# meyer-lab/cmtf-pls

Hardware: AMD Instinct MI355X
Metric: nipals_iters_per_sec (higher is better)
Workload: dtype f32

## Files before the change

cmtf_pls_amd/_lib.py:

```python
from __future__ import annotations

import ctypes
import os
from ctypes import c_char_p, c_double, c_int, c_int64, c_size_t, c_uint32, c_uint64, c_void_p

_HERE = os.path.dirname(os.path.abspath(__file__))
LIB_PATH = os.environ.get("CMTFPLS_LIB") or os.path.join(_HERE, "lib", "libcmtfpls.so")

_P = c_void_p

class XcovBlock(ctypes.Structure):
    _fields_ = [("S", _P), ("S2", _P), ("colcnt", _P), ("n_samples", c_double), ("order", c_int), ("A", c_int), ("B", c_int),
                ("n_squarings", c_int), ("Z", _P), ("wA", _P), ("wB", _P), ("info", _P)]


class KfoldState(ctypes.Structure):
    _fields_ = [("I", c_int), ("A", c_int), ("B", c_int), ("M", c_int), ("K", c_int), ("R", c_int)] + [
        (name, _P) for name in ("fold_of", "S", "mean", "Yk", "Gy", "WA", "WB", "Q", "Wa", "Wb", "T", "Gt", "coef", "Rm", "tm",
                                "Tout", "vec", "n_iter", "status", "part")]


class CvCoupledBlock(ctypes.Structure):
    _fields_ = [("X", _P), ("order", c_int), ("A", c_int), ("B", c_int)]


class LooCoupledBlock(ctypes.Structure):
    _fields_ = [("X", _P), ("colsum", _P), ("order", c_int), ("A", c_int), ("B", c_int)]


SIGNATURES = {
    "cmtfpls_xcov_iterate_blocks_f64": (c_int, [ctypes.POINTER(XcovBlock), c_int, c_int, _P, _P, _P, _P, _P, c_int, _P, c_size_t, _P]),
    "cmtfpls_abi_version": (c_int, []),
    "cmtfpls_last_error": (c_char_p, []),
    "cmtfpls_clear_error": (c_int, []),
    "cmtfpls_status_to_host": (c_int, [_P, _P, c_size_t, _P, _P]),
    "cmtfpls_colstats_workspace_bytes": (c_size_t, [c_int64, c_int64]),
    "cmtfpls_colstats_f32": (c_int, [_P, c_int64, c_int64, _P, _P, _P, c_size_t, _P]),
    "cmtfpls_colstats_f64": (c_int, [_P, c_int64, c_int64, _P, _P, _P, c_size_t, _P]),
    "cmtfpls_sweep_partials": (c_int, []),
    "cmtfpls_center_f32": (c_int, [_P, c_int64, c_int64, _P, _P, _P, _P]),
    "cmtfpls_center_f64": (c_int, [_P, c_int64, c_int64, _P, _P, _P, _P]),
    "cmtfpls_mode0_contract_workspace_bytes": (c_size_t, [c_int64, c_int64]),
    "cmtfpls_mode0_contract_f32": (c_int, [_P, c_int64, c_int64, _P, _P, c_int, _P, c_size_t, _P]),
    "cmtfpls_mode0_contract_f64": (c_int, [_P, c_int64, c_int64, _P, _P, c_int, _P, c_size_t, _P]),
    "cmtfpls_mode0_contract_yq_f32": (c_int, [_P, c_int64, c_int64, _P, c_int, c_int, _P, _P, c_int, _P, c_size_t, _P]),
    "cmtfpls_mode0_contract_yq_f64": (c_int, [_P, c_int64, c_int64, _P, c_int, c_int, _P, _P, c_int, _P, c_size_t, _P]),
    "cmtfpls_colscale_f64": (c_int, [_P, c_int64, _P, c_double, _P]),
    "cmtfpls_rank1_workspace_bytes": (c_size_t, [c_int, c_int]),
    "cmtfpls_rank1_score_f64": (c_int, [_P, c_int, c_int, _P, _P, _P, c_int, _P, c_int, _P, _P, c_size_t, _P]),
    "cmtfpls_rank1_f64": (c_int, [_P, c_int, c_int, _P, _P, _P, _P, c_int, _P, c_size_t, _P]),
    "cmtfpls_rank1_launches_f64": (c_int, [_P, c_int, c_int, _P, _P, _P, _P, c_int, _P, c_size_t, _P]),
    "cmtfpls_rank1_chain_enable": (None, [c_int]),
    "cmtfpls_rank1_chain_enabled": (c_int, []),
    "cmtfpls_normalize_f64": (c_int, [_P, c_int64, _P, _P]),
    "cmtfpls_rank1_tensor_workspace_bytes": (c_size_t, [_P, c_int]),
    "cmtfpls_rank1_tensor_f64": (c_int, [_P, _P, c_int, c_double, _P, c_int, _P, c_int, _P, c_size_t, _P]),
    "cmtfpls_kron_f64": (c_int, [_P, c_int, _P, c_int, _P, _P]),
    "cmtfpls_xcov_workspace_bytes": (c_size_t, [c_int64, c_int64, c_int]),
    "cmtfpls_xcov_f32": (c_int, [_P, c_int64, c_int64, _P, c_int, c_int, _P, c_int, _P, c_size_t, _P]),
    "cmtfpls_xcov_f64": (c_int, [_P, c_int64, c_int64, _P, c_int, c_int, _P, c_int, _P, c_size_t, _P]),
    "cmtfpls_xcov_bf16": (c_int, [_P, c_int64, c_int64, _P, c_int, c_int, _P, c_int, _P, c_size_t, _P]),
    "cmtfpls_xcov_f16": (c_int, [_P, c_int64, c_int64, _P, c_int, c_int, _P, c_int, _P, c_size_t, _P]),
    "cmtfpls_quadform_f64": (c_int, [_P, c_int, _P, _P, _P, _P]),
    "cmtfpls_xcov_iterate_f64": (c_int, [_P, c_int, c_int, c_int, _P, _P, _P, _P, _P, c_int, _P, _P, _P, c_int, _P, c_size_t, _P, c_size_t, _P]),
    "cmtfpls_s_downdate_f64": (c_int, [_P, c_int, c_int, c_int, _P, _P, _P, _P, _P, _P]),
    "cmtfpls_project_rows_f32": (c_int, [_P, c_int64, c_int, c_int, c_int, _P, _P, _P, _P, c_int, _P]),
    "cmtfpls_project_rows_f64": (c_int, [_P, c_int64, c_int, c_int, c_int, _P, _P, _P, _P, c_int, _P]),
    "cmtfpls_project_rows2_f32": (c_int, [_P, c_int, c_int, _P, _P, _P, _P, c_int, c_int, _P, _P, _P, c_int64, c_int, _P, c_int, _P]),
    "cmtfpls_project_rows2_f64": (c_int, [_P, c_int, c_int, _P, _P, _P, _P, c_int, c_int, _P, _P, _P, c_int64, c_int, _P, c_int, _P]),
    "cmtfpls_project_rows_idx_f32": (c_int, [_P, _P, c_int64, c_int, c_int, c_int, _P, _P, _P, _P, c_int, _P]),
    "cmtfpls_project_rows_idx_f64": (c_int, [_P, _P, c_int64, c_int, c_int, c_int, _P, _P, _P, _P, c_int, _P]),
    "cmtfpls_project_rows2_idx_f32": (c_int, [_P, c_int, c_int, _P, _P, _P, _P, c_int, c_int, _P, _P, _P, _P, c_int64, c_int, _P, c_int, _P]),
    "cmtfpls_project_rows2_idx_f64": (c_int, [_P, c_int, c_int, _P, _P, _P, _P, c_int, c_int, _P, _P, _P, _P, c_int64, c_int, _P, c_int, _P]),
    "cmtfpls_allreduce_sum_f64": (c_int, [_P, _P, c_size_t, _P]),
    "cmtfpls_allreduce_sum_f32": (c_int, [_P, _P, c_size_t, _P]),
    "cmtfpls_axpy_scalar_f64": (c_int, [_P, c_int64, _P, _P, _P]),
    "cmtfpls_xcov_deflate_f32": (c_int, [_P, c_int64, c_int, c_int, _P, c_int, c_int, _P, _P, _P, _P, _P, _P, c_size_t, _P]),
    "cmtfpls_xcov_deflate_f64": (c_int, [_P, c_int64, c_int, c_int, _P, c_int, c_int, _P, _P, _P, _P, _P, _P, c_size_t, _P]),
    "cmtfpls_xcov_stats_workspace_bytes": (c_size_t, [c_int64, c_int64, c_int]),
    "cmtfpls_xcov_stats_f32": (c_int, [_P, c_int64, c_int64, _P, c_int, c_int, _P, _P, _P, c_size_t, _P]),
    "cmtfpls_xcov_stats_f64": (c_int, [_P, c_int64, c_int64, _P, c_int, c_int, _P, _P, _P, c_size_t, _P]),
    "cmtfpls_xcov_stats_bf16": (c_int, [_P, c_int64, c_int64, _P, c_int, c_int, _P, _P, _P, c_size_t, _P]),
    "cmtfpls_xcov_stats_f16": (c_int, [_P, c_int64, c_int64, _P, c_int, c_int, _P, _P, _P, c_size_t, _P]),
    "cmtfpls_xcov_ssq_workspace_bytes": (c_size_t, [c_int64, c_int64, c_int]),
    "cmtfpls_xcov_ssq_f32": (c_int, [_P, c_int64, c_int64, _P, c_int, c_int, _P, _P, _P, _P, c_size_t, _P]),
    "cmtfpls_xcov_ssq_f64": (c_int, [_P, c_int64, c_int64, _P, c_int, c_int, _P, _P, _P, _P, c_size_t, _P]),
    "cmtfpls_score_contract_workspace_bytes": (c_size_t, [c_int64, c_int64]),
    "cmtfpls_score_contract_f32": (c_int, [_P, c_int64, c_int, c_int, _P, _P, _P, _P, _P, c_double, _P, _P, _P, _P, c_size_t, _P]),
    "cmtfpls_score_contract_f64": (c_int, [_P, c_int64, c_int, c_int, _P, _P, _P, _P, _P, c_double, _P, _P, _P, _P, c_size_t, _P]),
    "cmtfpls_score_contract_bf16": (c_int, [_P, c_int64, c_int, c_int, _P, _P, _P, _P, _P, c_double, _P, _P, _P, _P, c_size_t, _P]),
    "cmtfpls_score_contract_f16": (c_int, [_P, c_int64, c_int, c_int, _P, _P, _P, _P, _P, c_double, _P, _P, _P, _P, c_size_t, _P]),
    "cmtfpls_kr_axpy_f64": (c_int, [_P, c_int, c_int, _P, _P, c_int, c_int, _P, _P]),
    "cmtfpls_xcov_f32_mixed": (c_int, [_P, c_int64, c_int64, _P, c_int, c_int, _P, c_int, _P, c_size_t, _P]),
    "cmtfpls_mttkrp_f32_mixed": (c_int, [_P, c_int64, c_int, c_int, _P, _P, c_int, _P, c_int, _P]),
    "cmtfpls_mttkrp_f32": (c_int, [_P, c_int64, c_int, c_int, _P, _P, c_int, _P, c_int, _P]),
    "cmtfpls_mttkrp_f64": (c_int, [_P, c_int64, c_int, c_int, _P, _P, c_int, _P, c_int, _P]),
    "cmtfpls_mttkrp_bf16": (c_int, [_P, c_int64, c_int, c_int, _P, _P, c_int, _P, c_int, _P]),
    "cmtfpls_mttkrp_f16": (c_int, [_P, c_int64, c_int, c_int, _P, _P, c_int, _P, c_int, _P]),
    "cmtfpls_score_f32": (c_int, [_P, c_int64, c_int, c_int, _P, _P, _P, _P, _P]),
    "cmtfpls_score_f64": (c_int, [_P, c_int64, c_int, c_int, _P, _P, _P, _P, _P]),
    "cmtfpls_score_s_f64": (c_int, [_P, c_int, c_int, c_int, _P, _P, _P, _P]),
    "cmtfpls_deflate_contract_workspace_bytes": (c_size_t, [c_int64, c_int64]),
    "cmtfpls_deflate_contract_yq_f32": (c_int, [_P, c_int64, c_int, c_int, _P, _P, _P, _P, c_int, c_int, _P, _P, c_int, _P, _P, c_size_t, _P]),
    "cmtfpls_deflate_contract_yq_f64": (c_int, [_P, c_int64, c_int, c_int, _P, _P, _P, _P, c_int, c_int, _P, _P, c_int, _P, _P, c_size_t, _P]),
    "cmtfpls_score_gram_f32": (c_int, [_P, c_int64, c_int, c_int, _P, _P, _P, _P, _P, c_int, c_int, _P, _P]),
    "cmtfpls_score_gram_f64": (c_int, [_P, c_int64, c_int, c_int, _P, _P, _P, _P, _P, c_int, c_int, _P, _P]),
    "cmtfpls_q_update_f64": (c_int, [_P, c_int, c_int, _P, c_int, _P, _P, _P, _P]),
    "cmtfpls_deflate_f32": (c_int, [_P, c_int64, c_int, c_int, _P, _P, _P, _P, _P]),
    "cmtfpls_deflate_f64": (c_int, [_P, c_int64, c_int, c_int, _P, _P, _P, _P, _P]),
    "cmtfpls_score_deflate_f32": (c_int, [_P, c_int64, c_int, c_int, _P, _P, _P, _P, _P, _P]),
    "cmtfpls_score_deflate_f64": (c_int, [_P, c_int64, c_int, c_int, _P, _P, _P, _P, _P, _P]),
    "cmtfpls_sweep_form": (c_int, [c_char_p, c_int, c_int64, c_int, c_int, c_int, c_int, c_int, c_char_p, c_size_t]),
    "cmtfpls_sweep_form_list": (c_int, [c_char_p, c_int, c_char_p, c_size_t]),
    "cmtfpls_small_workspace_bytes": (c_size_t, []),
    "cmtfpls_gram_tn_f64": (c_int, [_P, c_int, c_int, _P, c_int, c_int, c_int64, _P, _P, c_size_t, _P]),
    "cmtfpls_rowdot_f64": (c_int, [_P, c_int, c_int, c_int64, _P, _P, _P, _P, _P, c_size_t, _P]),
    "cmtfpls_scores_mean_f64": (c_int, [_P, c_int, c_int64, _P, _P]),
    "cmtfpls_y_deflate_f64": (c_int, [_P, c_int, c_int, c_int64, _P, c_int, c_int, _P, _P, _P, _P, c_size_t, _P]),
# ... 159 lines not shown
```

cmtf_pls_amd/backend.py:

```python
from __future__ import annotations

import ctypes
from typing import Optional, Tuple

import torch

from . import _lib
from .storage import HALF_DTYPES, HALF_ENTRIES, SUFFIX, entry_name

_HALF_ENTRIES = tuple(dict.fromkeys(e for group in HALF_ENTRIES.values() for e in group))


def _ptr(t: Optional[torch.Tensor]):
    return None if t is None else t.data_ptr()


def _int_pairs(pairs):
    flat = [int(v) for p in pairs for v in p]
    return (ctypes.c_int * len(flat))(*flat)


def _scratch(nbytes: int, device) -> torch.Tensor:
    return torch.empty(max(int(nbytes), 256), dtype=torch.uint8, device=device)


def chunk_size(n: int, per: int, budget: int, cap: Optional[int] = None) -> int:
    chunk = max(1, min(int(n), int(budget) // max(int(per), 1)))
    return chunk if cap is None else min(chunk, int(cap))


class HipBackend:
    name = "hip"

    def __init__(self, device: Optional[torch.device] = None):
        self.lib = _lib.load()
        if not torch.cuda.is_available():
            raise _lib.CmtfplsError("cmtf_pls_amd needs a ROCm GPU (torch.cuda.is_available() is False); there is no CPU fallback")
        self.device = torch.device(device) if device is not None else torch.device("cuda", torch.cuda.current_device())
        self.n_partials = int(self.lib.cmtfpls_sweep_partials())
        self._ws = {}
        self._status_slots = {}
        self.rank1_squarings = 30
        self.rank1_chain_side = 256 if self.lib.cmtfpls_rank1_chain_enabled() else 0

    def _stream(self):
        return torch.cuda.current_stream(self.device).cuda_stream

    def _workspace(self, key: str, nbytes: int) -> torch.Tensor:
        buf = self._ws.get(key)
        if buf is None or buf.numel() < nbytes:
            buf = self._ws[key] = _scratch(nbytes, self.device)
        return buf

    @staticmethod
    def _form(rc: int, name: str, value=True):
        if rc == 4:
            return None
        _lib.check(rc, name)
        return value

    def _chunked_launch(self, name: str, call, n: int, per_fn, budget: int, cap: Optional[int] = None, extra: int = 0,
                        ws_key: Optional[str] = None) -> Optional[int]:
        if call(0, 1, None, 0) == 4:
            return None
        per = int(per_fn())
        chunk = chunk_size(n, per + extra, budget, cap)
        ws = self._workspace(ws_key, per * chunk) if ws_key else _scratch(per * chunk, self.device)
        launches = 0
        for i0 in range(0, n, chunk):
            if self._form(call(i0, min(chunk, n - i0), _ptr(ws), ws.numel()), name) is None:
                return None
            launches += 1
        return launches

    def _ws_budget(self, max_ws_bytes: Optional[int], third_of_free: bool = False) -> int:
        if max_ws_bytes is not None:
            return int(max_ws_bytes)
        return max(4 << 30, torch.cuda.mem_get_info(self.device)[0] // 3) if third_of_free else 4 << 30

    def clear_error(self) -> bool:
        return bool(self.lib.cmtfpls_clear_error())

    def empty(self, *shape, dtype=torch.float64) -> torch.Tensor:
        return torch.empty(*shape, dtype=dtype, device=self.device)

    def zeros(self, *shape, dtype=torch.float64) -> torch.Tensor:
        return torch.zeros(*shape, dtype=dtype, device=self.device)

    def has_half(self, base: str) -> bool:
        return base in _HALF_ENTRIES and all(hasattr(self.lib, entry_name(base, d)) for d in HALF_DTYPES)

    def _read_fn(self, base: str, X: torch.Tensor, mixed: bool = False):
        if X.dtype not in SUFFIX:
            raise TypeError(f"X must be float32 or float64 on device, got {X.dtype}")
        if X.dtype in HALF_DTYPES and (mixed or not self.has_half(base)):
            return None
        if mixed and X.dtype == torch.float32:
            return getattr(self.lib, f"cmtfpls_{base}_f32_mixed")
        assert X.is_contiguous() and X.device == self.device
        return getattr(self.lib, entry_name(base, X.dtype))

    def _fn(self, base: str, X: torch.Tensor):
        fn = self._read_fn(base, X)
        if fn is None:
            raise TypeError(f"{base} has no form for {X.dtype} storage (16-bit X is only read by {', '.join(_HALF_ENTRIES)}); "
                            "use a float32 copy")
        return fn

    def _close_partials(self, part: torch.Tensor) -> torch.Tensor:
        out = self.empty(1)
        _lib.check(self.lib.cmtfpls_sum_f64(_ptr(part), part.numel(), _ptr(out), self._stream()), "sum")
        return out

    @staticmethod
    def sweep_form(op: str, dtype, I: int, A: int, B: int, masked: bool = False, M: int = 0, aligned16: bool = True) -> str:
        buf = ctypes.create_string_buffer(256)
        elem = 4 if dtype in (torch.float32, "f32", "float32") else 8
        _lib.check(_lib.load().cmtfpls_sweep_form(op.encode(), elem, int(I), int(A), int(B), int(bool(masked)), int(M), int(bool(aligned16)),
                                                  buf, len(buf)), "sweep_form")
        return buf.value.decode()

    @staticmethod
    def sweep_form_list(op: str, dtype) -> list:
        buf = ctypes.create_string_buffer(1 << 14)
# ... 65 lines not shown
        ws = self._workspace("rank1t", self.lib.cmtfpls_rank1_tensor_workspace_bytes(arr, len(dims)))
        _lib.check(self.lib.cmtfpls_rank1_tensor_f64(_ptr(Z), arr, len(dims), float(tol), _ptr(factors), factors.stride(0), _ptr(info),
                                                     int(n_squarings or self.rank1_squarings), _ptr(ws), ws.numel(), self._stream()),
                   "rank1_tensor")

    def kron(self, a: torch.Tensor, b: torch.Tensor, out: torch.Tensor) -> torch.Tensor:
        _lib.check(self.lib.cmtfpls_kron_f64(_ptr(a), a.numel(), _ptr(b), b.numel(), _ptr(out), self._stream()), "kron")
        return out

    def normalize(self, v: torch.Tensor) -> None:
        _lib.check(self.lib.cmtfpls_normalize_f64(_ptr(v), v.numel(), None, self._stream()), "normalize")

    def xcov(self, X2: torch.Tensor, Y: torch.Tensor, masked: bool, out: Optional[torch.Tensor] = None,
             mixed: bool = False) -> Optional[torch.Tensor]:
        I, P = X2.shape
        M = Y.shape[1]
        fn = self._read_fn("xcov", X2, mixed)
        if fn is None:
            return None
        ws = self._workspace("contract", self.lib.cmtfpls_xcov_workspace_bytes(I, P, M))
        S = out if out is not None else self.empty(M, P)
        _lib.check(fn(_ptr(X2), I, P, _ptr(Y), Y.stride(0), M, _ptr(S), int(masked), _ptr(ws), ws.numel(), self._stream()), "xcov")
        return S

    def xcov_deflate(self, X2: torch.Tensor, A: int, B: int, Y: torch.Tensor, t: torch.Tensor, wA: torch.Tensor, wB: torch.Tensor,
                     out: torch.Tensor) -> Optional[torch.Tensor]:
        I, P = X2.shape
        M = Y.shape[1]
        if M > 64 or P % 4 != 0 or P != A * B:
            return None
        ws = self._workspace("contract", self.lib.cmtfpls_xcov_ssq_workspace_bytes(I, P, M))
        ssq = self.empty(1)
        rc = self._fn("xcov_deflate", X2)(_ptr(X2), I, A, B, _ptr(Y), Y.stride(0), M, _ptr(t), _ptr(wA), _ptr(wB), _ptr(out), _ptr(ssq),
                                          _ptr(ws), ws.numel(), self._stream())
        return self._form(rc, "xcov_deflate", ssq)

    def rank1_score(self, Z: torch.Tensor, A: int, B: int, wA: torch.Tensor, wB: torch.Tensor, S: torch.Tensor, tq: torch.Tensor,
                    info: Optional[torch.Tensor] = None, n_squarings: Optional[int] = None) -> torch.Tensor:
        M = S.shape[0]
        assert S.is_contiguous() and S.shape[1] == A * B and tq.numel() >= M
        ws = self._workspace("rank1", self.lib.cmtfpls_rank1_workspace_bytes(A, B))
        _lib.check(self.lib.cmtfpls_rank1_score_f64(_ptr(Z), A, B, _ptr(wA), _ptr(wB), _ptr(info),
                                                    int(n_squarings if n_squarings is not None else self.rank1_squarings),
                                                    _ptr(S), M, _ptr(tq), _ptr(ws), ws.numel(), self._stream()), "rank1_score")
        return tq

    def xcov_ssq(self, X2: torch.Tensor, Y: torch.Tensor, mean: torch.Tensor, out: torch.Tensor):
        I, P = X2.shape
        M = Y.shape[1]
        ws = self._workspace("contract", self.lib.cmtfpls_xcov_ssq_workspace_bytes(I, P, M))
        ssq = self.empty(1)
        assert mean.is_contiguous() and mean.numel() == P and mean.dtype == torch.float64
        _lib.check(self._fn("xcov_ssq", X2)(_ptr(X2), I, P, _ptr(Y), Y.stride(0), M, _ptr(out), _ptr(mean), _ptr(ssq), _ptr(ws), ws.numel(),
                                            self._stream()), "xcov_ssq")
        return out, ssq

    def xcov_stats(self, X2: torch.Tensor, Y: torch.Tensor, out: torch.Tensor):
        I, P = X2.shape
        M = Y.shape[1]
        fn = self._read_fn("xcov_stats", X2) if M <= 64 and X2.is_contiguous() else None
        if fn is None:
            return None
        ws = self._workspace("contract", self.lib.cmtfpls_xcov_stats_workspace_bytes(I, P, M))
        stats = self.empty(2 * P)
        rc = fn(_ptr(X2), I, P, _ptr(Y), Y.stride(0), M, _ptr(out), _ptr(stats), _ptr(ws), ws.numel(), self._stream())
        return self._form(rc, "xcov_stats", (out, stats))

    def status_snapshot(self, status: torch.Tensor, slot: int, slots: Optional[dict] = None):
        slots = self._status_slots if slots is None else slots
        ent = slots.get((slot, status.numel()))
        if ent is None:
            host, ev = torch.empty(status.numel(), dtype=torch.float64, pin_memory=True), torch.cuda.Event()
            ev.record(torch.cuda.current_stream(self.device))
            ent = slots[(slot, status.numel())] = (host, ev, host.numpy(), host.data_ptr(), ev.cuda_event, status.numel() * 8)
        rc = self.lib.cmtfpls_status_to_host(status.data_ptr(), ent[3], ent[5], ent[4], self._stream())
        if rc:
            _lib.check(rc, "status_to_host")
        return ent

    def status_wait(self, token) -> "np.ndarray":
        token[1].synchronize()
        return token[2]

    def xcov_iterate_plan(self, S: torch.Tensor, A: int, B: int, q_cur: torch.Tensor, Z: torch.Tensor, wA: torch.Tensor,
                          wB: torch.Tensor, status: torch.Tensor, q_new: torch.Tensor, G: torch.Tensor):
        M, P = S.shape
        wc = self._workspace("contract", self.lib.cmtfpls_mode0_contract_workspace_bytes(M, P))
        wr = self._workspace("rank1", self.lib.cmtfpls_rank1_workspace_bytes(A, B))
        keep = (S, q_cur, Z, wA, wB, status, q_new, G, wc, wr)
        fn = self.lib.cmtfpls_xcov_iterate_f64
        head = (_ptr(S), M, A, B, _ptr(q_cur), _ptr(Z), _ptr(wA), _ptr(wB), status[1:3].data_ptr())
        tail = (_ptr(wc), wc.numel(), _ptr(wr), wr.numel())
        qn, Gp, du2 = _ptr(q_new), _ptr(G), status[0:1].data_ptr()
        stream = self._stream

        def enqueue(n_squarings: int, first: bool, _keep=keep) -> None:
            rc = fn(*head, n_squarings, qn, Gp, du2, 1 if first else 0, *tail, stream())
            if rc:
                _lib.check(rc, "xcov_iterate")
        return enqueue

    def xcov_iterate(self, S: torch.Tensor, A: int, B: int, q_cur: torch.Tensor, Z: torch.Tensor, wA: torch.Tensor,
                     wB: torch.Tensor, info: torch.Tensor, n_squarings: int, q_new: torch.Tensor, G: torch.Tensor,
                     du2: torch.Tensor, first: bool) -> None:
        M, P = S.shape
        wc = self._workspace("contract", self.lib.cmtfpls_mode0_contract_workspace_bytes(M, P))
        wr = self._workspace("rank1", self.lib.cmtfpls_rank1_workspace_bytes(A, B))
        _lib.check(self.lib.cmtfpls_xcov_iterate_f64(_ptr(S), M, A, B, _ptr(q_cur), _ptr(Z), _ptr(wA), _ptr(wB), _ptr(info),
                                                     int(n_squarings), _ptr(q_new), _ptr(G), _ptr(du2), int(first),
                                                     _ptr(wc), wc.numel(), _ptr(wr), wr.numel(), self._stream()), "xcov_iterate")

    def xcov_blocks_plan(self, blocks, M: int, q_cur: torch.Tensor, tq: torch.Tensor, q_new: torch.Tensor, G: torch.Tensor,
                         status: torch.Tensor):
        nb = len(blocks)
        if M > 64 or any(b["order"] not in (2, 3) for b in blocks) or tq.numel() != nb * M or not tq.is_contiguous():
            return None
        arr = (_lib.XcovBlock * nb)()
        need = 256
        for i, b in enumerate(blocks):
            for name in ("S", "S2", "colcnt", "Z", "wA", "wB"):
                t = b.get(name)
                assert t is None or (t.is_contiguous() and t.dtype == torch.float64 and t.device == self.device), name
                setattr(arr[i], name, _ptr(t))
            arr[i].n_samples, arr[i].order, arr[i].A, arr[i].B = float(b["n_samples"]), int(b["order"]), int(b["A"]), int(b["B"])
            arr[i].info = status[1 + 2 * i: 3 + 2 * i].data_ptr()
            if b["order"] == 3:
                need = max(need, self.lib.cmtfpls_rank1_workspace_bytes(b["A"], b["B"]))
        wr = self._workspace("rank1", need)
        keep = (blocks, q_cur, tq, q_new, G, status, wr, arr)
        fn, stream = self.lib.cmtfpls_xcov_iterate_blocks_f64, self._stream
        args = (nb, M, _ptr(q_cur), _ptr(tq), _ptr(q_new), _ptr(G), status[0:1].data_ptr())
        tail = (_ptr(wr), wr.numel())

        def enqueue(n_squarings, first: bool, _keep=keep) -> None:
            for i in range(nb):
                arr[i].n_squarings = int(n_squarings[i])
            rc = fn(arr, *args, 1 if first else 0, *tail, stream())
            if rc:
                _lib.check(rc, "xcov_iterate_blocks")
        return enqueue

    def s_downdate(self, S: torch.Tensor, A: int, B: int, ya: torch.Tensor, wA: torch.Tensor, wB: torch.Tensor,
                   q: torch.Tensor, v: torch.Tensor) -> None:
        assert S.is_contiguous() and S.shape[1] == A * B
        _lib.check(self.lib.cmtfpls_s_downdate_f64(_ptr(S), S.shape[0], A, B, _ptr(ya), _ptr(wA), _ptr(wB), _ptr(q), _ptr(v),
                                                   self._stream()), "s_downdate")

    def kr_axpy(self, v: torch.Tensor, A: int, B: int, WA: torch.Tensor, WB: torch.Tensor, k: int, coef: torch.Tensor) -> torch.Tensor:
        assert WA.is_contiguous() and WB.is_contiguous() and WA.shape[1] == WB.shape[1] and coef.numel() >= k
        _lib.check(self.lib.cmtfpls_kr_axpy_f64(_ptr(v), A, B, _ptr(WA), _ptr(WB), WA.shape[1], int(k), _ptr(coef), self._stream()), "kr_axpy")
        return v

    def axpy_scalar(self, y: torch.Tensor, a: torch.Tensor, x: Optional[torch.Tensor] = None) -> torch.Tensor:
        assert y.is_contiguous() and y.dtype == torch.float64 and a.numel() >= 1 and (x is None or (x.is_contiguous() and x.numel() == y.numel()))
        _lib.check(self.lib.cmtfpls_axpy_scalar_f64(_ptr(y), y.numel(), _ptr(a), _ptr(x), self._stream()), "axpy_scalar")
        return y

    def total(self, v: torch.Tensor) -> torch.Tensor:
        assert v.is_contiguous() and v.dtype == torch.float64
        return self._close_partials(v)

    def quadform(self, G: torch.Tensor, q: torch.Tensor, q_old: torch.Tensor, out: torch.Tensor) -> torch.Tensor:
        _lib.check(self.lib.cmtfpls_quadform_f64(_ptr(G), G.shape[0], _ptr(q), _ptr(q_old), _ptr(out), self._stream()), "quadform")
        return out

    def mttkrp(self, X2: torch.Tensor, A: int, B: int, WA: torch.Tensor, WB: torch.Tensor, out: torch.Tensor,
               mixed: bool = False) -> Optional[torch.Tensor]:
        R = WA.shape[1]
        assert WA.is_contiguous() and WB.is_contiguous() and out.stride(1) == 1
        fn = self._read_fn("mttkrp", X2, mixed)
        if fn is None:
            return None
        rc = fn(_ptr(X2), X2.shape[0], A, B, _ptr(WA), _ptr(WB), R, _ptr(out), out.stride(0), self._stream())
        return self._form(rc, "mttkrp", out)

    def score(self, X2, A, B, wA, wB, rowcnt, out) -> torch.Tensor:
        _lib.check(self._fn("score", X2)(_ptr(X2), X2.shape[0], A, B, _ptr(wA), _ptr(wB), _ptr(rowcnt), _ptr(out), self._stream()), "score")
        return out

    def score_s(self, S, A, B, wA, wB, out) -> torch.Tensor:
        assert S.dtype == torch.float64 and S.is_contiguous()
        _lib.check(self.lib.cmtfpls_score_s_f64(_ptr(S), S.shape[0], A, B, _ptr(wA), _ptr(wB), _ptr(out), self._stream()), "score_s")
        return out

    def score_contract(self, X2, A, B, wA, wB, shift, t, Z, sub_own=None, add_other=None, alpha: float = 1.0,
                       csum: Optional[torch.Tensor] = None) -> Optional[torch.Tensor]:
        I, P = X2.shape
        fn = self._read_fn("score_contract", X2) if X2.is_contiguous() and P == A * B else None
        if fn is None:
            return None
        for v in (sub_own, add_other):
            assert v is None or (v.is_contiguous() and v.numel() == I and v.dtype == torch.float64)
        nbytes = self.lib.cmtfpls_score_contract_workspace_bytes(I, P)
        ws = self._workspace("score_contract", max(nbytes, 256))
        rc = fn(_ptr(X2), I, A, B, _ptr(wA), _ptr(wB), _ptr(shift), _ptr(sub_own), _ptr(add_other), float(alpha),
                                            _ptr(t), _ptr(Z), _ptr(csum), _ptr(ws), ws.numel(), self._stream())
        return self._form(rc, "score_contract", Z)

    def score_gram(self, X2, A, B, wA, wB, rowcnt, out, Y: torch.Tensor, qpart: torch.Tensor) -> Optional[torch.Tensor]:
        assert qpart.numel() >= self.n_partials * Y.shape[1] and qpart.is_contiguous()
        rc = self._fn("score_gram", X2)(_ptr(X2), X2.shape[0], A, B, _ptr(wA), _ptr(wB), _ptr(rowcnt), _ptr(out),
                                        _ptr(Y), Y.stride(0), Y.shape[1], _ptr(qpart), self._stream())
        return self._form(rc, "score_gram", out)

    def q_update(self, q: torch.Tensor, qpart: Optional[torch.Tensor] = None, normalize: bool = True,
                 G: Optional[torch.Tensor] = None, q_prev: Optional[torch.Tensor] = None,
                 du2: Optional[torch.Tensor] = None, nparts: Optional[int] = None) -> None:
        M = q.numel()
        nrows = (nparts or self.n_partials) if qpart is not None else 0
        assert qpart is None or (qpart.is_contiguous() and qpart.numel() >= nrows * M)
        _lib.check(self.lib.cmtfpls_q_update_f64(_ptr(qpart), nrows, M, _ptr(q), int(normalize),
                                                 _ptr(G), _ptr(q_prev), _ptr(du2), self._stream()), "q_update")

    def deflate(self, X2, A, B, t, wA, wB) -> torch.Tensor:
        part = self.empty(self.n_partials)
        _lib.check(self._fn("deflate", X2)(_ptr(X2), X2.shape[0], A, B, _ptr(t), _ptr(wA), _ptr(wB), _ptr(part), self._stream()), "deflate")
        return self._close_partials(part)

    def deflate_contract_yq(self, X2, A, B, t, wA, wB, Y: torch.Tensor, q: torch.Tensor, masked: bool,
                            out: torch.Tensor) -> Optional[torch.Tensor]:
        I, P = X2.shape
        ws = self._workspace("deflate_contract", self.lib.cmtfpls_deflate_contract_workspace_bytes(I, P))
        ssq = self.empty(1)
        rc = self._fn("deflate_contract_yq", X2)(_ptr(X2), I, A, B, _ptr(t), _ptr(wA), _ptr(wB), _ptr(Y), Y.stride(0), Y.shape[1],
                                                 _ptr(q), _ptr(out), int(masked), _ptr(ssq), _ptr(ws), ws.numel(), self._stream())
        return self._form(rc, "deflate_contract_yq", ssq)

    def score_deflate(self, X2, A, B, wA, wB, rowcnt, out) -> Optional[torch.Tensor]:
        part = self.empty(self.n_partials)
        rc = self._fn("score_deflate", X2)(_ptr(X2), X2.shape[0], A, B, _ptr(wA), _ptr(wB), _ptr(rowcnt), _ptr(out), _ptr(part), self._stream())
        if self._form(rc, "score_deflate") is None:
            return None
        return self._close_partials(part)

    def gram_tn(self, A: torch.Tensor, B: torch.Tensor, out: Optional[torch.Tensor] = None) -> torch.Tensor:
        if A.dim() == 1:
            A = A.unsqueeze(1)
        if B.dim() == 1:
            B = B.unsqueeze(1)
        assert A.stride(1) == 1 and B.stride(1) == 1 and A.shape[0] == B.shape[0]
        a, b = A.shape[1], B.shape[1]
        ws = self._workspace("small", self.lib.cmtfpls_small_workspace_bytes())
        C = out if out is not None else self.empty(a, b)
        assert C.numel() == a * b and C.is_contiguous()
        _lib.check(self.lib.cmtfpls_gram_tn_f64(_ptr(A), A.stride(0), a, _ptr(B), B.stride(0), b, A.shape[0], _ptr(C),
                                                _ptr(ws), ws.numel(), self._stream()), "gram_tn")
        return C

    def rowdot(self, Y: torch.Tensor, q: torch.Tensor, u_out: torch.Tensor, u_old: Optional[torch.Tensor],
               du2: Optional[torch.Tensor] = None) -> Optional[torch.Tensor]:
        ws = self._workspace("small", self.lib.cmtfpls_small_workspace_bytes())
        if u_old is not None and du2 is None:
            du2 = self.empty(1)
        _lib.check(self.lib.cmtfpls_rowdot_f64(_ptr(Y), Y.stride(0), Y.shape[1], Y.shape[0], _ptr(q), _ptr(u_out), _ptr(u_old),
                                               _ptr(du2) if u_old is not None else None,
                                               _ptr(ws), ws.numel(), self._stream()), "rowdot")
        return du2 if u_old is not None else None

    def normal_solve(self, G: torch.Tensor, g: torch.Tensor, out: Optional[torch.Tensor] = None) -> torch.Tensor:
        k = G.shape[0]
        assert G.is_contiguous() and G.shape == (k, k) and g.numel() == k
        b = out if out is not None else self.empty(k)
        if k <= 64:
            _lib.check(self.lib.cmtfpls_normal_solve_f64(_ptr(G), _ptr(g), k, _ptr(b), 1, self._stream()), "normal_solve")
        else:
            ws = self._workspace("normal_solve", self.lib.cmtfpls_normal_solve_workspace_bytes(k))
            _lib.check(self.lib.cmtfpls_normal_solve_ws_f64(_ptr(G), _ptr(g), k, _ptr(b), 1, _ptr(ws), ws.numel(), self._stream()),
                       "normal_solve")
        return b

    def unit_upper_solve_rows(self, M: torch.Tensor, U: torch.Tensor, shift: Optional[torch.Tensor] = None,
                              nan_flag: Optional[torch.Tensor] = None) -> torch.Tensor:
        I, R = M.shape
        assert M.stride(1) == 1 and U.is_contiguous() and U.shape == (R, R)
        assert shift is None or (shift.is_contiguous() and shift.numel() == R and shift.dtype == torch.float64)
        assert nan_flag is None or nan_flag.dtype == torch.int32
        _lib.check(self.lib.cmtfpls_unit_upper_solve_rows_f64(_ptr(M), I, M.stride(0), R, _ptr(U), _ptr(shift), _ptr(nan_flag),
                                                              self._stream()), "unit_upper_solve_rows")
        return M

    def kr_gram_row(self, L: torch.Tensor, a: int, g: torch.Tensor, first: bool) -> torch.Tensor:
        assert L.is_contiguous() and g.is_contiguous() and g.numel() >= a
        _lib.check(self.lib.cmtfpls_kr_gram_row_f64(_ptr(L), L.shape[0], L.shape[1], int(a), _ptr(g), int(first), self._stream()), "kr_gram_row")
        return g

    def kr_gram(self, L: torch.Tensor, G: torch.Tensor, first: bool) -> torch.Tensor:
        n, R = L.shape
        assert L.is_contiguous() and G.is_contiguous() and G.numel() == R * R
        _lib.check(self.lib.cmtfpls_kr_gram_f64(_ptr(L), n, R, _ptr(G), int(first), 1.0, self._stream()), "kr_gram")
        return G

    def khatri_rao(self, Am: torch.Tensor, Bm: torch.Tensor) -> torch.Tensor:
        na, R = Am.shape
# ... 489 lines not shown
```

cmtf_pls_amd/csrc/common.hpp:

```cpp
#pragma once
#include <hip/hip_runtime.h>
#include <stdint.h>
#include <stdio.h>

#include "../../include/cmtfpls.h"

namespace cmtfpls {

constexpr int kWave = 64;
#ifndef CMTFPLS_SWEEP_BLOCKS
#define CMTFPLS_SWEEP_BLOCKS 512
#endif
#ifndef CMTFPLS_UNROLL
#define CMTFPLS_UNROLL 4
#endif
#ifndef CMTFPLS_ROW_UNROLL
#define CMTFPLS_ROW_UNROLL 8
#endif
#ifndef CMTFPLS_CONTRACT_BLOCKS
#define CMTFPLS_CONTRACT_BLOCKS 1024
#endif
#ifndef CMTFPLS_NT_LOAD
#define CMTFPLS_NT_LOAD 1
#endif
// ... 57 lines not shown
__device__ __forceinline__ VT ld_stream(const VT* p) {
#if CMTFPLS_NT_LOAD
  using R = typename NtRaw<sizeof(VT)>::type;
  const R r = __builtin_nontemporal_load(reinterpret_cast<const R*>(p));
  VT v;
  __builtin_memcpy(&v, &r, sizeof(VT));
  return v;
#else
  return *p;
#endif
}
template <typename VT>
__device__ __forceinline__ void st_stream(VT* p, const VT& v) {
#if CMTFPLS_NT_STORE
  using R = typename NtRaw<sizeof(VT)>::type;
  R r;
  __builtin_memcpy(&r, &v, sizeof(VT));
  __builtin_nontemporal_store(r, reinterpret_cast<R*>(p));
#else
  *p = v;
#endif
}

__device__ __forceinline__ double wave_sum(double v) {
#pragma unroll
  for (int m = 32; m > 0; m >>= 1) v += __shfl_xor(v, m, kWave);
  return v;
}

__device__ __forceinline__ double block_sum(double v, double* slot) {
  const int lane = threadIdx.x & 63, wv = threadIdx.x >> 6, nw = (blockDim.x + 63) >> 6;
  v = wave_sum(v);
  if (lane == 0) slot[wv] = v;
  __syncthreads();
  double s = 0.0;
  for (int w = 0; w < nw; ++w) s += slot[w];
  return s;
}

struct KronWalk {
  int j, k, dj, dk, B;
  __device__ __forceinline__ KronWalk(int64_t c0, int64_t stride, int B_) : B(B_) {
    j = (int)(c0 / B_);
    k = (int)(c0 % B_);
    dj = (int)(stride / B_);
    dk = (int)(stride % B_);
  }
  __device__ __forceinline__ void next() {
    k += dk;
    j += dj;
    if (k >= B) { k -= B; ++j; }
  }
};


struct TileId { int ct, rb; };
__device__ __forceinline__ TileId xcd_tile() {
  const unsigned CT = gridDim.x, RB = gridDim.y;
  const unsigned lin = blockIdx.x + CT * blockIdx.y;
  const unsigned G = CT * 8u, groups = RB / 8u;
  const unsigned grp = lin / G;
  TileId id;
  if (grp < groups) {
    const unsigned within = lin - grp * G;
    id.ct = (int)(within >> 3);
    id.rb = (int)(grp * 8u + (within & 7u));
  } else {
    const unsigned rest = lin - groups * G;
    id.ct = (int)(rest % CT);
    id.rb = (int)(groups * 8u + rest / CT);
  }
  return id;
}

struct XcovPlan {
  int col_tiles, row_blocks, rows_per_block;
};
XcovPlan plan_xcov(int64_t I, int64_t P);
constexpr int kXcovMaxResponses = 64;

void set_error(const char* msg);
int check_launch(const char* what);

}
```

cmtf_pls_amd/csrc/rank1.hip:

```cpp
#include "common.hpp"
#include <atomic>

namespace cmtfpls {

constexpr int kTile = 16;
constexpr int kMaxTiles = 256;
constexpr int kMaxSteps = 48;

struct Rank1Ctl {
  int done;
  int final_buf;
  int steps_used;
  int last_step;
  double pad[6];
};
__host__ __device__ __forceinline__ size_t rank1_ctl_bytes(int nt) {
  return sizeof(Rank1Ctl) + ((size_t)(kMaxSteps + 2) * nt + 2 * (size_t)nt * nt) * sizeof(double);
}
__device__ __forceinline__ double* ctl_trace(Rank1Ctl* c, int nt, int step) { return reinterpret_cast<double*>(c + 1) + (size_t)step * nt; }
__device__ __forceinline__ double* ctl_fro(Rank1Ctl* c, int nt, int which) {
  return reinterpret_cast<double*>(c + 1) + (size_t)(kMaxSteps + 2) * nt + (size_t)which * nt * nt;
}

__device__ __forceinline__ double pow2_scale_from_trace(const double* parts, int nt, double* tr_out) {
// ... 49 lines not shown
    if (tid >= nt * nt) f = 0.0;
    for (int i = tid + kTile * kTile; i < nt * nt; i += kTile * kTile) f += fp[i];
    f = wave_sum(f);
    if ((tid & 63) == 0) fsum[tid >> 6] = f;
    if (tid == 0) s_done = done_in;
    __syncthreads();
    fro_in = ((fsum[0] + fsum[1]) + fsum[2]) + fsum[3];
  }
  if (tid == 0) {
    int done = 0;
    double scale = 1.0;
    if (step == 0) {
      if (blockIdx.x == 0 && blockIdx.y == 0) { ctl->done = 0; ctl->final_buf = -1; ctl->steps_used = 0; ctl->last_step = -1; }
    } else {
      done = s_done;
      if (!done) {
        double tr1;
        scale = pow2_scale_from_trace(tr_s, nt, &tr1);
        const double rho = fro_in / (tr1 * tr1);
        const bool rank_one_in = !(tr1 > 0.0) || rho >= 1.0 - 1e-13;
        const bool rank_one_out = rho >= 1.0 - 1e-7;
        if (blockIdx.x == 0 && blockIdx.y == 0) {
          if (rank_one_in) { ctl->done = 1; ctl->final_buf = out_buf ^ 1; }
          else {
            ctl->steps_used = step;
            if (rank_one_out) { ctl->last_step = step; ctl->final_buf = out_buf; }
          }
        }
        if (rank_one_in) done = 1;
      }
    }
    s_scale = scale;
    s_done = done;
  }
  __syncthreads();
  if (s_done) return;
  const double scale = s_scale;

  d4r_t acc = d4r_t{0.0, 0.0, 0.0, 0.0};
  for (int kk = 0; kk < k; kk += KC) {
    if (kk > 0) {
#pragma unroll
      for (int s2 = 0; s2 < KW; ++s2) {
        const int c = kk + cl + s2;
        const int cc = (c < k) ? c : 0;
        a[s2] = rowa[cc];
        b[s2] = rowb[cc];
      }
    }
#pragma unroll
    for (int s2 = 0; s2 < KW; ++s2) {
      const bool cok = (kk + cl + s2) < k;
      const double av = (ra && cok) ? a[s2] : 0.0;
      const double bv = (rb && cok) ? b[s2] : 0.0;
      acc = __builtin_amdgcn_mfma_f64_16x16x4f64(av, bv, acc, 0, 0, 0);
    }
  }
#pragma unroll
  for (int e = 0; e < 4; ++e) red[wv][(kq + 4 * e) * kTile + ri] = acc[e];
  __syncthreads();
  double cacc = ((red[0][tid] + red[1][tid]) + red[2][tid]) + red[3][tid];
  cacc *= scale * scale;
  const bool inside = (i0 + ty < n && j0 + tx < n);
  if (inside) C[(int64_t)(i0 + ty) * n + (j0 + tx)] = cacc;
  if (inside && C_keep) C_keep[(int64_t)(i0 + ty) * n + (j0 + tx)] = cacc;
  {
    double sq = inside ? cacc * cacc : 0.0;
    sq = wave_sum(sq);
    if ((tid & 63) == 0) fsum[tid >> 6] = sq;
    __syncthreads();
    if (tid == 0) ctl_fro(ctl, nt, step & 1)[blockIdx.y * nt + blockIdx.x] = ((fsum[0] + fsum[1]) + fsum[2]) + fsum[3];
  }
  if (blockIdx.x == blockIdx.y) {
    if (tx == ty) diag[tx] = (i0 + ty < n) ? cacc : 0.0;
    __syncthreads();
    if (tid == 0) {
      double t = 0.0;
      for (int l = 0; l < kTile; ++l) t += diag[l];
      ctl_trace(ctl, nt, step)[blockIdx.x] = t;
    }
  }
}

constexpr unsigned long long kChainEmpty = ~0ull;
constexpr int kChainMaxSteps = 31;
constexpr int kChainSpin = 1 << 15;

__device__ __forceinline__ double chain_ld(const double* p) {
  return __longlong_as_double((long long)__hip_atomic_load(reinterpret_cast<const unsigned long long*>(p), __ATOMIC_RELAXED, __HIP_MEMORY_SCOPE_AGENT));
}
__device__ __forceinline__ void chain_st(double* p, double v) {
  unsigned long long b = (unsigned long long)__double_as_longlong(v);
  if (b == kChainEmpty) b = 0x7FF8000000000000ull;
  __hip_atomic_store(reinterpret_cast<unsigned long long*>(p), b, __ATOMIC_RELAXED, __HIP_MEMORY_SCOPE_AGENT);
}
__device__ __forceinline__ bool chain_empty(double v) { return (unsigned long long)__double_as_longlong(v) == kChainEmpty; }

__global__ __launch_bounds__(256) void chain_preset_kernel(unsigned long long* __restrict__ p, int64_t n) {
  for (int64_t i = (int64_t)blockIdx.x * 256 + threadIdx.x; i < n; i += (int64_t)gridDim.x * 256) p[i] = kChainEmpty;
}

#ifdef CMTFPLS_CHAIN_PROFILE
__device__ unsigned long long g_chain_prof[1024];
#define CHAIN_STAMP(slot) do { if (first_wg && tid == 0 && step < 32) g_chain_prof[step * 8 + (slot)] = __builtin_amdgcn_s_memrealtime(); } while (0)
#define CHAIN_COUNT(slot, v) do { if (first_wg && tid == 0 && step < 32) g_chain_prof[step * 8 + (slot)] = (unsigned long long)(v); } while (0)
#else
#define CHAIN_STAMP(slot) do { } while (0)
#define CHAIN_COUNT(slot, v) do { } while (0)
#endif

__global__ __launch_bounds__(kTile* kTile) void syrk_chain_kernel(const double* __restrict__ M0, int n, int k0,
                                                                 double* gbufs, double* trs, double* fros, double* gave_up,
                                                                 Rank1Ctl* __restrict__ ctl, int n_squarings) {
  constexpr int KC = 128, KW = 8, LDP = KC + 2;
  __shared__ __attribute__((aligned(16))) double pan[2][kTile][LDP];
  __shared__ double red[2][4][kTile * kTile];
  __shared__ double diag[2][kTile];
  __shared__ double fsum[2][4];
  __shared__ double cfro[2][4];
  __shared__ double ctr[2][kTile];
  __shared__ int cdead[2];
  const int tx = threadIdx.x, ty = threadIdx.y, tid = ty * kTile + tx;
  const int lane = tid & 63, wv = tid >> 6, ri = lane & 15, kq = lane >> 4;
  const int nt = (n + kTile - 1) / kTile, nt2 = nt * nt;
  const int i0 = blockIdx.y * kTile, j0 = blockIdx.x * kTile;
  const bool first_wg = blockIdx.x == 0 && blockIdx.y == 0;
  const bool ra = (i0 + ri) < n, rb = (j0 + ri) < n;
  const int cl = 32 * wv + KW * kq;
  const int64_t nn = (int64_t)n * n;
  const double qnan = __longlong_as_double(0x7FF8000000000000ll);
  bool dead = false;
  if (first_wg && tid == 0) { ctl->done = 0; ctl->final_buf = -1; ctl->steps_used = 0; ctl->last_step = -1; }
  if (tid < 2) cdead[tid] = 0;
  int last_step = -1;
  for (int step = 0; step <= n_squarings; ++step) {
    if (last_step >= 0) break;
    const int par = step & 1;
    const double* __restrict__ M = step == 0 ? M0 : gbufs + (int64_t)(step - 1) * nn;
    const int k = step == 0 ? k0 : n, ld = k;
    double* C = gbufs + (int64_t)step * nn;
    double a[KW], b[KW];
    double scale = 1.0;
    bool input_is_result = false;
    d4r_t acc = d4r_t{0.0, 0.0, 0.0, 0.0};
    CHAIN_STAMP(0);
    for (int kk = 0; kk < k; kk += KC) {
      if (step == 0) {
        const double* __restrict__ rowa = M + (int64_t)(ra ? i0 + ri : 0) * ld;
        const double* __restrict__ rowb = M + (int64_t)(rb ? j0 + ri : 0) * ld;
#pragma unroll
        for (int s2 = 0; s2 < KW; ++s2) {
          const int c = kk + cl + s2;
          const int cc = (c < k) ? c : 0;
          a[s2] = rowa[cc];
          b[s2] = rowb[cc];
        }
      } else {
        double va[8], vb[8], trv = 0.0, f = 0.0;
        const bool first_chunk = kk == 0;
        const double* tp = trs + (int64_t)(step - 1) * nt;
        const double* fp = fros + (int64_t)(step - 1) * nt2;
        unsigned offa[8], offb[8];
#pragma unroll
        for (int i = 0; i < 8; ++i) {
          const int e = tid + 256 * i, r = e >> 7, c = kk + (e & 127);
          const int cc = (c < k) ? c : 0;
          const int rra = (i0 + r < n) ? i0 + r : 0, rrb = (j0 + r < n) ? j0 + r : 0;
// ... 275 lines not shown
    if (bestv[w] > bv || (bestv[w] == bv && besti[w] < bi)) { bv = bestv[w]; bi = besti[w]; }
  const bool gv = gave && !chain_empty(chain_ld(gave));
  const double sgn = gv ? __longlong_as_double(0x7FF8000000000000ll) : ((vb[bi] < 0.0) ? -1.0 : 1.0);
  double* lx = x_is_A ? sA : sB;
  double* ly = x_is_A ? sB : sA;
  double* ox = x_is_A ? wA : wB;
  double* oy = x_is_A ? wB : wA;
  const bool store = blockIdx.x == 0;
  for (int i = threadIdx.x; i < n; i += 1024) {
    const double v = sgn * (x[i] / nx);
    lx[i] = v;
    if (store) ox[i] = v;
  }
  for (int i = threadIdx.x; i < k; i += 1024) {
    const double v = sgn * (y[i] / ny);
    ly[i] = v;
    if (store) oy[i] = v;
  }
  if (store && threadIdx.x == 0) rank1_write_info(info, ctl, gave);
  __syncthreads();
  using VT = Pack<double, 2>;
  const int64_t P = (int64_t)A * B;
  const int64_t step = (int64_t)1024 * 2;
  const double* __restrict__ xr = S + (int64_t)blockIdx.x * P;
  KronWalk w((int64_t)threadIdx.x * 2, step, B);
  double acc = 0.0;
  int64_t c = (int64_t)threadIdx.x * 2;
  constexpr int UN = 4;
  for (; c + (UN - 1) * step < P; c += UN * step) {
    VT xs[UN];
#pragma unroll
    for (int u = 0; u < UN; ++u) xs[u] = ld_stream(reinterpret_cast<const VT*>(xr + c + u * step));
#pragma unroll
    for (int u = 0; u < UN; ++u) {
      double d = 0.0;
      d = fma(xs[u].e[0], sB[w.k], d);
      d = fma(xs[u].e[1], sB[w.k + 1], d);
      acc = fma(sA[w.j], d, acc);
      w.next();
    }
  }
  for (; c < P; c += step) {
    const VT xv = ld_stream(reinterpret_cast<const VT*>(xr + c));
    double d = 0.0;
    d = fma(xv.e[0], sB[w.k], d);
    d = fma(xv.e[1], sB[w.k + 1], d);
    acc = fma(sA[w.j], d, acc);
    w.next();
  }
  acc = block_sum(acc, red[0]);
  if (threadIdx.x == 0) t[blockIdx.x] = acc;
}

static inline size_t align_up(size_t x, size_t a) { return (x + a - 1) / a * a; }

static std::atomic<int> g_chain_on{1};

static int chain_slots() {
  static int slots = 0;
  if (slots == 0) {
    int dev = 0, cus = 0;
    if (hipGetDevice(&dev) != hipSuccess || hipDeviceGetAttribute(&cus, hipDeviceAttributeMultiprocessorCount, dev) != hipSuccess || cus <= 0) cus = 256;
    slots = 2 * cus;
  }
  return slots;
}

}

using namespace cmtfpls;

extern "C" {

size_t cmtfpls_rank1_workspace_bytes(int A, int B) {
  if (A <= 0 || B <= 0) return 0;
  const size_t n = (size_t)(A < B ? A : B), k = (size_t)(A < B ? B : A);
  const size_t nt = (n + kTile - 1) / kTile;
  const size_t chain = nt * nt <= 256 ? align_up(((size_t)(kChainMaxSteps + 1) * (n * n + nt + nt * nt) + 1) * sizeof(double), 256) : 0;
  return align_up(rank1_ctl_bytes((int)nt), 256) + 3 * align_up(n * n * sizeof(double), 256) +
         align_up((size_t)A * B * sizeof(double), 256) + align_up(n * sizeof(double), 256) + align_up(k * sizeof(double), 256) + chain;
}

static int rank1_run(const double* Z, int A, int B, double* wA, double* wB, double* sigma, double* info,
                     int n_squarings, void* ws, size_t ws_bytes, void* stream, const double* S, int M, double* tq, bool allow_chain = true);

int cmtfpls_rank1_f64(const double* Z, int A, int B, double* wA, double* wB, double* sigma, double* info,
                      int n_squarings, void* ws, size_t ws_bytes, void* stream) {
  return rank1_run(Z, A, B, wA, wB, sigma, info, n_squarings, ws, ws_bytes, stream, nullptr, 0, nullptr);
}

#ifdef CMTFPLS_CHAIN_PROFILE
int cmtfpls_debug_chain_prof(unsigned long long* out) { return (int)hipMemcpyFromSymbol(out, HIP_SYMBOL(g_chain_prof), sizeof(unsigned long long) * 1024); }
#endif
void cmtfpls_rank1_chain_enable(int on) { g_chain_on.store((on == 1 || on == 2) ? on : 0, std::memory_order_relaxed); }
int cmtfpls_rank1_chain_enabled(void) { return g_chain_on.load(std::memory_order_relaxed); }

int cmtfpls_rank1_launches_f64(const double* Z, int A, int B, double* wA, double* wB, double* sigma, double* info,
                               int n_squarings, void* ws, size_t ws_bytes, void* stream) {
  return rank1_run(Z, A, B, wA, wB, sigma, info, n_squarings, ws, ws_bytes, stream, nullptr, 0, nullptr, false);
}

int cmtfpls_rank1_score_f64(const double* Z, int A, int B, double* wA, double* wB, double* info, int n_squarings,
                            const double* S, int M, double* tq, void* ws, size_t ws_bytes, void* stream) {
  if (!S || !tq || M <= 0) { set_error("rank1_score: bad argument"); return CMTFPLS_EINVAL; }
  const int64_t P = (int64_t)A * B;
  if (M > 64 || P < 8192 || (B % 2) != 0 || ((size_t)(((A + 1) & ~1) + B) * sizeof(double)) > 60 * 1024 ||
      (reinterpret_cast<uintptr_t>(S) & 15) != 0) {
    int rc = cmtfpls_rank1_f64(Z, A, B, wA, wB, nullptr, info, n_squarings, ws, ws_bytes, stream);
    if (rc == CMTFPLS_OK) rc = cmtfpls_score_s_f64(S, M, A, B, wA, wB, tq, stream);
    return rc;
  }
  return rank1_run(Z, A, B, wA, wB, nullptr, info, n_squarings, ws, ws_bytes, stream, S, M, tq);
}

static int rank1_run(const double* Z, int A, int B, double* wA, double* wB, double* sigma, double* info,
                     int n_squarings, void* ws, size_t ws_bytes, void* stream, const double* S, int M, double* tq, bool allow_chain) {
  if (!Z || !wA || !wB || A <= 0 || B <= 0) { set_error("rank1: bad argument"); return CMTFPLS_EINVAL; }
  const int n = A < B ? A : B, k = A < B ? B : A;
  if (n > kTile * kMaxTiles) { set_error("rank1: min(A, B) > 4096 unsupported"); return CMTFPLS_EUNSUPPORTED; }
  if ((size_t)n * sizeof(double) > 64 * 1024) { set_error("rank1: seed exceeds the LDS"); return CMTFPLS_EUNSUPPORTED; }
  if (n_squarings < 1) n_squarings = 1;
  if (n_squarings > kMaxSteps) n_squarings = kMaxSteps;
  if (!ws || ws_bytes < cmtfpls_rank1_workspace_bytes(A, B)) { set_error("rank1: workspace too small"); return CMTFPLS_EWORKSPACE; }
  hipStream_t st = (hipStream_t)stream;
  char* p = static_cast<char*>(ws);
  Rank1Ctl* ctl = reinterpret_cast<Rank1Ctl*>(p);
  p += align_up(rank1_ctl_bytes((n + kTile - 1) / kTile), 256);
  double* buf0 = reinterpret_cast<double*>(p);
  p += align_up((size_t)n * n * sizeof(double), 256);
  double* buf1 = reinterpret_cast<double*>(p);
  p += align_up((size_t)n * n * sizeof(double), 256);
  double* g0keep = reinterpret_cast<double*>(p);
  p += align_up((size_t)n * n * sizeof(double), 256);
  double* Zt = reinterpret_cast<double*>(p);
  p += align_up((size_t)A * B * sizeof(double), 256);
  double* xv = reinterpret_cast<double*>(p);
  p += align_up((size_t)n * sizeof(double), 256);
  double* yv = reinterpret_cast<double*>(p);
  p += align_up((size_t)k * sizeof(double), 256);
  double* chain_region = reinterpret_cast<double*>(p);

  const double* M0 = Z;
  if (A > B) {
    const int64_t tot = (int64_t)A * B;
    hipLaunchKernelGGL(transpose_kernel, dim3((unsigned)((tot + 255) / 256)), dim3(256), 0, st, Z, A, B, Zt);
    M0 = Zt;
  }
  const int nt = (n + kTile - 1) / kTile;
  const dim3 grid(nt, nt), block(kTile, kTile);
  const int ny_blocks = (k + 31) / 32;
  const double* gave = nullptr;
  if (allow_chain && g_chain_on.load(std::memory_order_relaxed) && nt * nt <= 256 && nt * nt <= chain_slots() && n_squarings <= kChainMaxSteps) {
    const size_t nn = (size_t)n * n, steps = (size_t)n_squarings + 1;
    double* gbufs = chain_region;
    double* trs = gbufs + steps * nn;
    double* fros = trs + steps * nt;
    double* gave_up = fros + steps * (size_t)nt * nt;
    gave = gave_up;
    const int64_t words = (int64_t)(steps * (nn + nt + (size_t)nt * nt) + 1);
    hipLaunchKernelGGL(chain_preset_kernel, dim3((unsigned)((words + 2047) / 2048)), dim3(256), 0, st, reinterpret_cast<unsigned long long*>(chain_region), words);
    const dim3 cgrid(nt, (g_chain_on.load(std::memory_order_relaxed) == 2 && nt > 1) ? nt - 1 : nt);
    hipLaunchKernelGGL(syrk_chain_kernel, cgrid, block, 0, st, M0, n, k, gbufs, trs, fros, gave_up, ctl, n_squarings);
    hipLaunchKernelGGL(rank1_seed_xy_kernel, dim3(ny_blocks + (n + 3) / 4), dim3(256), (size_t)n * sizeof(double), st,
                       M0, n, k, gbufs, (int64_t)nn, gbufs, ctl, n_squarings, ny_blocks, yv, xv);
  } else {
    hipLaunchKernelGGL(syrk_step_kernel, grid, block, 0, st, M0, n, k, k, buf0, ctl, 0, 0, g0keep);
    for (int s = 1; s <= n_squarings; ++s) {
      const double* in = (s & 1) ? buf0 : buf1;
      double* out = (s & 1) ? buf1 : buf0;
      hipLaunchKernelGGL(syrk_step_kernel, grid, block, 0, st, in, n, n, n, out, ctl, s, s & 1, (double*)nullptr);
    }
    hipLaunchKernelGGL(rank1_seed_xy_kernel, dim3(ny_blocks + (n + 3) / 4), dim3(256), (size_t)n * sizeof(double), st,
                       M0, n, k, buf0, (int64_t)(buf1 - buf0), g0keep, ctl, n_squarings & 1, ny_blocks, yv, xv);
  }
  if (S) {
    const size_t lds = (size_t)(((A + 1) & ~1) + B) * sizeof(double);
    hipLaunchKernelGGL(rank1_final_score_kernel, dim3((unsigned)M), dim3(1024), lds, st, xv, yv, n, k, (A <= B) ? 1 : 0, ctl, wA, wB, info,
                       S, A, B, tq, gave);
    return check_launch("rank1_score");
  }
  hipLaunchKernelGGL(rank1_final_kernel, dim3(1), dim3(1024), 0, st, xv, yv, n, k, (A <= B) ? 1 : 0, ctl, wA, wB, sigma, info, gave);
  return check_launch("rank1");
}

}
```

cmtf_pls_amd/csrc/runtime.hip:

```cpp
#include <string.h>

#include "common.hpp"

namespace cmtfpls {

static thread_local char g_err[256] = "";

void set_error(const char* msg) {
  strncpy(g_err, msg, sizeof(g_err) - 1);
  g_err[sizeof(g_err) - 1] = 0;
}

int check_launch(const char* what) {
  const hipError_t e = hipGetLastError();
  if (e == hipSuccess) return CMTFPLS_OK;
  snprintf(g_err, sizeof(g_err), "%s: %s", what, hipGetErrorString(e));
  return CMTFPLS_EHIP;
}

}

extern "C" {
int cmtfpls_abi_version(void) { return 1; }
const char* cmtfpls_last_error(void) { return cmtfpls::g_err; }
int cmtfpls_clear_error(void) {
  const hipError_t e = hipGetLastError();
  cmtfpls::g_err[0] = 0;
  return e == hipSuccess ? 0 : 1;
}

int cmtfpls_status_to_host(const void* src, void* dst_host, size_t bytes, void* event, void* stream) {
  if (!src || !dst_host || bytes == 0) { cmtfpls::set_error("status_to_host: bad argument"); return CMTFPLS_EINVAL; }
  hipStream_t st = (hipStream_t)stream;
  hipError_t e = hipMemcpyAsync(dst_host, src, bytes, hipMemcpyDeviceToHost, st);
  if (e == hipSuccess && event) e = hipEventRecord((hipEvent_t)event, st);
  if (e != hipSuccess) { cmtfpls::set_error(hipGetErrorString(e)); return CMTFPLS_EHIP; }
  return CMTFPLS_OK;
}
}
```

cmtf_pls_amd/csrc/small.hip:

```cpp
#include "common.hpp"

namespace cmtfpls {

void launch_reduce_rows(const double* part, int nrows, int64_t P, double* out, hipStream_t st);

constexpr int kSmallBlocks = 128;
constexpr int kMaxGramDim = 64;
constexpr size_t kSmallWsBytes = (size_t)kSmallBlocks * kMaxGramDim * kMaxGramDim * sizeof(double);

__global__ __launch_bounds__(256) void gram_tn_kernel(const double* __restrict__ A, int lda, int a,
                                                     const double* __restrict__ B, int ldb, int b,
                                                     int64_t I, double* __restrict__ part, int TR) {
  extern __shared__ double lds[];
  double* As = lds;
  double* Bs = lds + TR * a;
  const int ab = a * b;
  const int64_t rows_per = (I + gridDim.x - 1) / gridDim.x;
  const int64_t r0 = (int64_t)blockIdx.x * rows_per;
  const int64_t r1 = (r0 + rows_per < I) ? r0 + rows_per : I;
  double acc[16];
#pragma unroll
  for (int s = 0; s < 16; ++s) acc[s] = 0.0;
  for (int64_t rb = r0; rb < r1; rb += TR) {
    const int nr = (int)((r1 - rb < TR) ? r1 - rb : TR);
    if (lda == a) {
      for (int idx = threadIdx.x; idx < nr * a; idx += 256) As[idx] = A[rb * a + idx];
    } else {
      for (int idx = threadIdx.x; idx < nr * a; idx += 256) As[idx] = A[(rb + idx / a) * lda + idx % a];
    }
    if (ldb == b) {
      for (int idx = threadIdx.x; idx < nr * b; idx += 256) Bs[idx] = B[rb * b + idx];
    } else {
      for (int idx = threadIdx.x; idx < nr * b; idx += 256) Bs[idx] = B[(rb + idx / b) * ldb + idx % b];
    }
    __syncthreads();
#pragma unroll
    for (int s = 0; s < 16; ++s) {
      const int o = threadIdx.x + s * 256;
      if (o < ab) {
        const int p = o / b, q = o % b;
        double v = acc[s];
        for (int r = 0; r < nr; ++r) v = fma(As[r * a + p], Bs[r * b + q], v);
        acc[s] = v;
      }
    }
    __syncthreads();
  }
#pragma unroll
  for (int s = 0; s < 16; ++s) {
    const int o = threadIdx.x + s * 256;
    if (o < ab) part[(int64_t)blockIdx.x * ab + o] = acc[s];
  }
}

__global__ __launch_bounds__(256) void reduce_block_kernel(const double* __restrict__ part, int nblk, int ac, int bc,
                                                          double* __restrict__ C, int ldc) {
  const int o = blockIdx.x * 4 + (threadIdx.x >> 6);
  const int lane = threadIdx.x & 63;
  if (o >= ac * bc) return;
  double s = 0.0;
  for (int r = lane; r < nblk; r += 64) s += part[(int64_t)r * ac * bc + o];
  s = wave_sum(s);
  if (lane == 0) C[(int64_t)(o / bc) * ldc + (o % bc)] = s;
}

__global__ __launch_bounds__(256) void gemv_t_kernel(const double* __restrict__ A, int lda, int a0, int ac,
                                                    const double* __restrict__ v, int ldv, int64_t I,
                                                    double* __restrict__ part, int a_total) {
  __shared__ double red[4][16];
  double acc[16];
#pragma unroll
  for (int e = 0; e < 16; ++e) acc[e] = 0.0;
  for (int64_t i = (int64_t)blockIdx.x * 256 + threadIdx.x; i < I; i += (int64_t)gridDim.x * 256) {
    const double vi = v[i * ldv];
    const double* ar = A + i * lda + a0;
#pragma unroll
    for (int e = 0; e < 16; ++e)
      if (e < ac) acc[e] = fma(ar[e], vi, acc[e]);
  }
  const int lane = threadIdx.x & 63, wv = threadIdx.x >> 6;
#pragma unroll
  for (int e = 0; e < 16; ++e) {
// ... 25 lines not shown
  }
}

__global__ __launch_bounds__(256) void y_deflate_kernel(double* __restrict__ Y, int ldy, int M, int64_t I,
                                                       const double* __restrict__ T, int ldt, int R,
                                                       const double* __restrict__ b, const double* __restrict__ q,
                                                       double* __restrict__ part) {
  __shared__ double red[16];
  double ssq = 0.0;
  for (int64_t i = (int64_t)blockIdx.x * 256 + threadIdx.x; i < I; i += (int64_t)gridDim.x * 256) {
    double s = 0.0;
    for (int r = 0; r < R; ++r) s = fma(T[i * ldt + r], b[r], s);
    double* yr = Y + i * ldy;
    for (int m = 0; m < M; ++m) {
      const double v = yr[m] - s * q[m];
      yr[m] = v;
      ssq = fma(v, v, ssq);
    }
  }
  const double s = block_sum(ssq, red);
  if (threadIdx.x == 0) part[blockIdx.x] = s;
}

__global__ __launch_bounds__(1024) void sum_kernel(const double* __restrict__ in, int64_t n, double* __restrict__ out) {
  __shared__ double red[16];
  double s = 0.0;
  for (int64_t i = threadIdx.x; i < n; i += 1024) s += in[i];
  s = block_sum(s, red);
  if (threadIdx.x == 0) out[0] = s;
}

__global__ __launch_bounds__(1024) void normalize_kernel(double* __restrict__ v, int64_t n, double* __restrict__ nrm) {
  __shared__ double red[16];
  double s = 0.0;
  for (int64_t i = threadIdx.x; i < n; i += 1024) s = fma(v[i], v[i], s);
  s = sqrt(block_sum(s, red));
  for (int64_t i = threadIdx.x; i < n; i += 1024) v[i] = v[i] / s;
  if (nrm && threadIdx.x == 0) nrm[0] = s;
}

__global__ __launch_bounds__(1024) void normalize_to_kernel(const double* __restrict__ in, double* __restrict__ out, int64_t n) {
  __shared__ double red[16];
  double s = 0.0;
  for (int64_t i = threadIdx.x; i < n; i += 1024) s = fma(in[i], in[i], s);
  s = sqrt(block_sum(s, red));
  for (int64_t i = threadIdx.x; i < n; i += 1024) out[i] = in[i] / s;
}

__global__ __launch_bounds__(1024) void s_vector_block_kernel(const double* __restrict__ S, const double* __restrict__ S2,
                                                            const double* __restrict__ colcnt, double n_samples, int M, int P,
                                                            const double* __restrict__ q, double* __restrict__ Z,
                                                            double* __restrict__ wB, double* __restrict__ tq) {
  extern __shared__ double wl[];
  __shared__ double red[16];
  const int lane = threadIdx.x & 63, wv = threadIdx.x >> 6;
  double ssq = 0.0;
  for (int c = threadIdx.x; c < P; c += 1024) {
    double z = 0.0;
#pragma unroll 8
    for (int m = 0; m < M; ++m) z = fma(q[m], S[(int64_t)m * P + c], z);
    if (colcnt) z = (colcnt[c] > 0.0) ? z / colcnt[c] * n_samples : 0.0;
    Z[c] = z;
    wl[c] = z;
    ssq = fma(z, z, ssq);
  }
  const double nrm = sqrt(block_sum(ssq, red));
  for (int c = threadIdx.x; c < P; c += 1024) {
    const double w = wl[c] / nrm;
    wl[c] = w;
    wB[c] = w;
  }
  __syncthreads();
  for (int m = wv; m < M; m += 16) {
    double acc = 0.0;
    for (int c = lane; c < P; c += 64) acc = fma(S2[(int64_t)m * P + c], wl[c], acc);
    acc = wave_sum(acc);
    if (lane == 0) tq[m] = acc;
  }
}

__global__ __launch_bounds__(1024) void q_update_kernel(const double* __restrict__ qpart, int nblk, int M,
                                                       double* __restrict__ q, int normalize,
                                                       const double* __restrict__ G, const double* __restrict__ q_prev,
                                                       double* __restrict__ du2) {
  __shared__ double part[64][17];
  __shared__ double qs[64];
  __shared__ double dq[64];
  __shared__ double red[16];
  const int tid = threadIdx.x, lane = tid & 63;
  const int Mp = (M <= 16) ? 16 : (M <= 32) ? 32 : 64;
  const int ngrp = 1024 / Mp;
  const int m = tid & (Mp - 1), grp = tid / Mp;
  double* pflat = &part[0][0];
  if (qpart) {
    double sacc = 0.0;
    const int msafe = (m < M) ? m : 0;
    for (int b0 = grp; b0 < nblk; b0 += 16 * ngrp) {
      double v[16];
#pragma unroll
      for (int k = 0; k < 16; ++k) {
        const int b = b0 + k * ngrp;
        v[k] = qpart[(int64_t)((b < nblk) ? b : nblk - 1) * M + msafe];
      }
#pragma unroll
      for (int k = 0; k < 16; ++k) sacc += (b0 + k * ngrp < nblk) ? v[k] : 0.0;
    }
    if (m >= M) sacc = 0.0;
    pflat[grp * (Mp + 1) + m] = sacc;
    __syncthreads();
    if (tid < M) {
      double tot = 0.0;
      for (int g = 0; g < ngrp; ++g) tot += pflat[g * (Mp + 1) + tid];
      qs[tid] = tot;
    }
  } else if (tid < M) {
    qs[tid] = q[tid];
  }
  __syncthreads();
  if (tid < 64) {
    double v = (lane < M) ? qs[lane] : 0.0;
    if (normalize) {
      const double nrm = sqrt(wave_sum(v * v));
      v = v / nrm;
    }
    if (lane < M) {
      q[lane] = v;
      if (G) dq[lane] = v - q_prev[lane];
    }
  }
  if (G) {
    __syncthreads();
    double sacc = 0.0;
    for (int idx = tid; idx < M * M; idx += 1024) {
      const int i = idx / M, j = idx - i * M;
      sacc = fma(dq[i] * G[idx], dq[j], sacc);
    }
    sacc = block_sum(sacc, red);
    if (tid == 0) du2[0] = sacc;
  }
}

__global__ __launch_bounds__(256) void s_downdate_kernel(double* __restrict__ S, int M, int64_t P, int B,
                                                        const double* __restrict__ ya, const double* __restrict__ wA,
                                                        const double* __restrict__ wB, const double* __restrict__ q,
                                                        const double* __restrict__ v) {
  const int64_t c = (int64_t)blockIdx.x * 256 + threadIdx.x;
  if (c >= P) return;
  const double w = wA[c / B] * wB[c % B];
  const double vc = v[c];
  for (int m = 0; m < M; ++m) {
    double sv = S[(int64_t)m * P + c];
    sv = fma(-ya[m], w, sv);
    sv = fma(-q[m], vc, sv);
    S[(int64_t)m * P + c] = sv;
  }
}

__global__ __launch_bounds__(256) void s_contract_kernel(const double* __restrict__ S, int M, int64_t P, const double* __restrict__ q,
                                                        double* __restrict__ Z) {
  const int64_t c = (int64_t)blockIdx.x * 256 + threadIdx.x;
  if (c >= P) return;
  double acc = 0.0;
#pragma unroll 8
  for (int m = 0; m < M; ++m) acc = fma(q[m], S[(int64_t)m * P + c], acc);
  Z[c] = acc;
}

__global__ __launch_bounds__(256) void axpy_scalar_kernel(double* __restrict__ y, int64_t n, const double* __restrict__ a,
                                                         const double* __restrict__ x) {
  const double av = a[0];
  for (int64_t i = (int64_t)blockIdx.x * 256 + threadIdx.x; i < n; i += (int64_t)gridDim.x * 256) y[i] = fma(-av, x ? x[i] : 1.0, y[i]);
}

__global__ __launch_bounds__(256) void kr_axpy_kernel(double* __restrict__ v, int64_t P, int B, const double* __restrict__ WA,
                                                     const double* __restrict__ WB, int ld, int k, const double* __restrict__ coef) {
  __shared__ double cs[64];
  for (int j = threadIdx.x; j < k; j += 256) cs[j] = coef[j];
  __syncthreads();
  const int64_t c = (int64_t)blockIdx.x * 256 + threadIdx.x;
  if (c >= P) return;
  const double* __restrict__ wa = WA + (c / B) * ld;
  const double* __restrict__ wb = WB + (c % B) * ld;
  double s = 0.0;
  for (int j = 0; j < k; ++j) s = fma(cs[j] * wa[j], wb[j], s);
  v[c] -= s;
}

__global__ __launch_bounds__(256) void colscale_kernel(double* __restrict__ Z, int64_t P, const double* __restrict__ cnt, double n_samples) {
  const int64_t c = (int64_t)blockIdx.x * 256 + threadIdx.x;
  if (c < P) Z[c] = (cnt[c] > 0.0) ? Z[c] / cnt[c] * n_samples : 0.0;
}

__global__ __launch_bounds__(256) void scores_mean_kernel(const double* __restrict__ Ts, int nb, int64_t I, double* __restrict__ out) {
  const int64_t i = (int64_t)blockIdx.x * 256 + threadIdx.x;
  if (i >= I) return;
  double s = Ts[i];
  for (int b = 1; b < nb; ++b) s += Ts[(int64_t)b * I + i];
  out[i] = s / (double)nb;
}

}

using namespace cmtfpls;

extern "C" {

size_t cmtfpls_small_workspace_bytes(void) { return kSmallWsBytes; }

int cmtfpls_gram_tn_f64(const double* A, int lda, int a, const double* B, int ldb, int b, int64_t I,
                        double* C, void* ws, size_t ws_bytes, void* stream) {
  if (!A || !B || !C || a <= 0 || b <= 0 || lda < a || ldb < b || I <= 0) {
    set_error("gram_tn: bad argument");
    return CMTFPLS_EINVAL;
  }
  if (!ws || ws_bytes < kSmallWsBytes) { set_error("gram_tn: workspace too small"); return CMTFPLS_EWORKSPACE; }
  hipStream_t st = (hipStream_t)stream;
  double* part = static_cast<double*>(ws);
  if (b == 1 && (size_t)kSmallBlocks * a * sizeof(double) <= kSmallWsBytes) {
    for (int a0 = 0; a0 < a; a0 += 16) {
      const int ac = (a - a0 < 16) ? a - a0 : 16;
      hipLaunchKernelGGL(gemv_t_kernel, dim3(kSmallBlocks), dim3(256), 0, st, A, lda, a0, ac, B, ldb, I, part, a);
    }
    hipLaunchKernelGGL(reduce_block_kernel, dim3((a + 3) / 4), dim3(256), 0, st, part, kSmallBlocks, a, 1, C, 1);
    return check_launch("gram_tn");
  }
  for (int a0 = 0; a0 < a; a0 += kMaxGramDim)
    for (int b0 = 0; b0 < b; b0 += kMaxGramDim) {
      const int ac = (a - a0 < kMaxGramDim) ? a - a0 : kMaxGramDim;
      const int bc = (b - b0 < kMaxGramDim) ? b - b0 : kMaxGramDim;
      const int tr = (ac + bc <= 32) ? 128 : (ac + bc <= 64) ? 64 : 32;
      const size_t lds = (size_t)tr * (ac + bc) * sizeof(double);
      hipLaunchKernelGGL(gram_tn_kernel, dim3(kSmallBlocks), dim3(256), lds, st, A + a0, lda, ac, B + b0, ldb, bc, I, part, tr);
      hipLaunchKernelGGL(reduce_block_kernel, dim3((ac * bc + 3) / 4), dim3(256), 0, st, part, kSmallBlocks, ac, bc,
                         C + (size_t)a0 * b + b0, b);
    }
  return check_launch("gram_tn");
}

int cmtfpls_rowdot_f64(const double* Y, int ldy, int M, int64_t I, const double* q, double* u,
                       const double* u_old, double* du2, void* ws, size_t ws_bytes, void* stream) {
  if (!Y || !q || !u || M <= 0 || ldy < M || I <= 0 || (u_old && !du2)) { set_error("rowdot: bad argument"); return CMTFPLS_EINVAL; }
  if (u_old && (!ws || ws_bytes < kSmallBlocks * sizeof(double))) { set_error("rowdot: workspace too small"); return CMTFPLS_EWORKSPACE; }
  hipStream_t st = (hipStream_t)stream;
  double* part = u_old ? static_cast<double*>(ws) : nullptr;
  hipLaunchKernelGGL(rowdot_kernel, dim3(kSmallBlocks), dim3(256), 0, st, Y, ldy, M, I, q, u, u_old, part);
  if (u_old) hipLaunchKernelGGL(sum_kernel, dim3(1), dim3(1024), 0, st, part, (int64_t)kSmallBlocks, du2);
  return check_launch("rowdot");
}

int cmtfpls_y_deflate_f64(double* Y, int ldy, int M, int64_t I, const double* T, int ldt, int R,
                          const double* b, const double* q, double* ssq, void* ws, size_t ws_bytes, void* stream) {
  if (!Y || !T || !b || !q || !ssq || M <= 0 || ldy < M || R <= 0 || ldt < R || I <= 0) { set_error("y_deflate: bad argument"); return CMTFPLS_EINVAL; }
  if (!ws || ws_bytes < kSmallBlocks * sizeof(double)) { set_error("y_deflate: workspace too small"); return CMTFPLS_EWORKSPACE; }
  hipStream_t st = (hipStream_t)stream;
  double* part = static_cast<double*>(ws);
  hipLaunchKernelGGL(y_deflate_kernel, dim3(kSmallBlocks), dim3(256), 0, st, Y, ldy, M, I, T, ldt, R, b, q, part);
  hipLaunchKernelGGL(sum_kernel, dim3(1), dim3(1024), 0, st, part, (int64_t)kSmallBlocks, ssq);
  return check_launch("y_deflate");
}

int cmtfpls_sum_f64(const double* in, int64_t n, double* out, void* stream) {
  if (!in || !out || n <= 0) { set_error("sum: bad argument"); return CMTFPLS_EINVAL; }
  hipLaunchKernelGGL(sum_kernel, dim3(1), dim3(1024), 0, (hipStream_t)stream, in, n, out);
  return check_launch("sum");
}

int cmtfpls_normalize_f64(double* v, int64_t n, double* nrm, void* stream) {
  if (!v || n <= 0) { set_error("normalize: bad argument"); return CMTFPLS_EINVAL; }
  hipLaunchKernelGGL(normalize_kernel, dim3(1), dim3(1024), 0, (hipStream_t)stream, v, n, nrm);
  return check_launch("normalize");
}

int cmtfpls_q_update_f64(const double* qpart, int nblk, int M, double* q, int normalize, const double* G, const double* q_prev,
                         double* du2, void* stream) {
  if (!q || M <= 0 || (qpart && nblk <= 0) || (G && (!q_prev || !du2))) { set_error("q_update: bad argument"); return CMTFPLS_EINVAL; }
  if (M > 64) { set_error("q_update: more than 64 responses; use gram_tn + normalize + rowdot"); return CMTFPLS_EUNSUPPORTED; }
  hipLaunchKernelGGL(q_update_kernel, dim3(1), dim3(1024), 0, (hipStream_t)stream, qpart, nblk, M, q, normalize, G, q_prev, du2);
  return check_launch("q_update");
}

int cmtfpls_s_downdate_f64(double* S, int M, int A, int B, const double* ya, const double* wA, const double* wB,
                           const double* q, const double* v, void* stream) {
  if (!S || !ya || !wA || !wB || !q || !v || M <= 0 || A <= 0 || B <= 0) { set_error("s_downdate: bad argument"); return CMTFPLS_EINVAL; }
  const int64_t P = (int64_t)A * B;
  hipLaunchKernelGGL(s_downdate_kernel, dim3((unsigned)((P + 255) / 256)), dim3(256), 0, (hipStream_t)stream, S, M, P, B, ya, wA, wB, q, v);
  return check_launch("s_downdate");
}

int cmtfpls_axpy_scalar_f64(double* y, int64_t n, const double* a, const double* x, void* stream) {
  if (!y || !a || n <= 0) { set_error("axpy_scalar: bad argument"); return CMTFPLS_EINVAL; }
  int64_t blocks = (n + 255) / 256;
  if (blocks > 1024) blocks = 1024;
  hipLaunchKernelGGL(axpy_scalar_kernel, dim3((unsigned)blocks), dim3(256), 0, (hipStream_t)stream, y, n, a, x);
  return check_launch("axpy_scalar");
}

int cmtfpls_kr_axpy_f64(double* v, int A, int B, const double* WA, const double* WB, int ld, int k, const double* coef, void* stream) {
  if (!v || !WA || !WB || !coef || A <= 0 || B <= 0 || k < 0 || ld < k) { set_error("kr_axpy: bad argument"); return CMTFPLS_EINVAL; }
  if (k > 64) { set_error("kr_axpy: more than 64 terms"); return CMTFPLS_EUNSUPPORTED; }
  if (k == 0) return CMTFPLS_OK;
  const int64_t P = (int64_t)A * B;
  hipLaunchKernelGGL(kr_axpy_kernel, dim3((unsigned)((P + 255) / 256)), dim3(256), 0, (hipStream_t)stream, v, P, B, WA, WB, ld, k, coef);
  return check_launch("kr_axpy");
}

int cmtfpls_xcov_iterate_f64(const double* S, int M, int A, int B, const double* q_cur, double* Z, double* wA, double* wB,
                             double* info, int n_squarings, double* q_new, const double* G, double* du2, int first,
                             void* ws_contract, size_t ws_contract_bytes, void* ws_rank1, size_t ws_rank1_bytes, void* stream) {
  if (!S || !q_cur || !Z || !wA || !wB || !q_new || !G || !du2 || M <= 0 || A <= 0 || B <= 0) {
    set_error("xcov_iterate: bad argument");
    return CMTFPLS_EINVAL;
  }
  if (M > 64) { set_error("xcov_iterate: more than 64 responses"); return CMTFPLS_EUNSUPPORTED; }
  const int64_t P = (int64_t)A * B;
  int rc = CMTFPLS_OK;
  if (first) {
    hipLaunchKernelGGL(s_contract_kernel, dim3((unsigned)((P + 255) / 256)), dim3(256), 0, (hipStream_t)stream, S, M, P, q_cur, Z);
    rc = check_launch("xcov_iterate: s_contract");
  }
  if (rc == CMTFPLS_OK) rc = cmtfpls_rank1_score_f64(Z, A, B, wA, wB, info, n_squarings, S, M, q_new, ws_rank1, ws_rank1_bytes, stream);
  if (rc == CMTFPLS_OK) rc = cmtfpls_q_update_f64(nullptr, 0, M, q_new, 1, G, q_cur, du2, stream);
  return rc;
}

int cmtfpls_xcov_iterate_blocks_f64(const cmtfpls_xcov_block* blocks, int nb, int M, const double* q_cur, double* tq, double* q_new,
                                    const double* G, double* du2, int first, void* ws_rank1, size_t ws_rank1_bytes, void* stream) {
  if (!blocks || nb <= 0 || !q_cur || !tq || !q_new || !G || !du2 || M <= 0) { set_error("xcov_iterate_blocks: bad argument"); return CMTFPLS_EINVAL; }
  if (M > 64) { set_error("xcov_iterate_blocks: more than 64 responses"); return CMTFPLS_EUNSUPPORTED; }
  hipStream_t st = (hipStream_t)stream;
  int rc = CMTFPLS_OK;
  for (int b = 0; b < nb && rc == CMTFPLS_OK; ++b) {
    const cmtfpls_xcov_block& k = blocks[b];
    if (!k.S || !k.Z || !k.wA || !k.wB || k.A <= 0 || k.B <= 0 || (k.order != 2 && k.order != 3) || (k.order == 2 && k.A != 1) ||
        (k.order == 3 && !k.info)) {
      set_error("xcov_iterate_blocks: bad block");
      return CMTFPLS_EINVAL;
    }
    const int64_t P = (int64_t)k.A * k.B;
    if (k.order == 2 && P <= 8192) {
      hipLaunchKernelGGL(s_vector_block_kernel, dim3(1), dim3(1024), (size_t)P * sizeof(double), st, k.S, k.S2 ? k.S2 : k.S, k.colcnt,
                         k.n_samples, M, (int)P, q_cur, k.Z, k.wB, tq + (int64_t)b * M);
      rc = check_launch("xcov_iterate_blocks: s_vector_block");
      continue;
    }
    if (first) {
      hipLaunchKernelGGL(s_contract_kernel, dim3((unsigned)((P + 255) / 256)), dim3(256), 0, st, k.S, M, P, q_cur, k.Z);
      rc = check_launch("xcov_iterate_blocks: s_contract");
      if (rc == CMTFPLS_OK && k.colcnt) rc = cmtfpls_colscale_f64(k.Z, P, k.colcnt, k.n_samples, stream);
    }
    if (rc != CMTFPLS_OK) break;
    if (k.order == 3) {
      rc = cmtfpls_rank1_score_f64(k.Z, k.A, k.B, k.wA, k.wB, k.info, k.n_squarings, k.S2 ? k.S2 : k.S, M, tq + (int64_t)b * M, ws_rank1,
                                   ws_rank1_bytes, stream);
      continue;
    } else {
      hipLaunchKernelGGL(normalize_to_kernel, dim3(1), dim3(1024), 0, st, k.Z, k.wB, P);
      rc = check_launch("xcov_iterate_blocks: normalize_to");
    }
    if (rc == CMTFPLS_OK) rc = cmtfpls_score_s_f64(k.S2 ? k.S2 : k.S, M, k.A, k.B, k.wA, k.wB, tq + (int64_t)b * M, stream);
  }
  if (rc == CMTFPLS_OK) rc = cmtfpls_q_update_f64(tq, nb, M, q_new, 1, G, q_cur, du2, stream);
  return rc;
}

int cmtfpls_colscale_f64(double* Z, int64_t P, const double* colcnt, double n_samples, void* stream) {
  if (!Z || !colcnt || P <= 0) { set_error("colscale: bad argument"); return CMTFPLS_EINVAL; }
  hipLaunchKernelGGL(colscale_kernel, dim3((unsigned)((P + 255) / 256)), dim3(256), 0, (hipStream_t)stream, Z, P, colcnt, n_samples);
  return check_launch("colscale");
}

int cmtfpls_scores_mean_f64(const double* Ts, int nb, int64_t I, double* out, void* stream) {
  if (!Ts || !out || nb <= 0 || I <= 0) { set_error("scores_mean: bad argument"); return CMTFPLS_EINVAL; }
  hipLaunchKernelGGL(scores_mean_kernel, dim3((unsigned)((I + 255) / 256)), dim3(256), 0, (hipStream_t)stream, Ts, nb, I, out);
  return check_launch("scores_mean");
}

}
```

cmtf_pls_amd/fitrun.py:

```python
from __future__ import annotations

import math
from typing import Dict, List, Optional

import numpy as np
import torch

from .fitrun_xcov import XcovMixin
from .state import BlockState, FitState, split_trailing, validate_limits
from .storage import HALF_DTYPES, HALF_ENTRIES, dtype_name, fallback_text, half_route


class FitRun(XcovMixin):

    def __init__(self, eng: NipalsEngine, Xs: List[torch.Tensor], Y: torch.Tensor, n_components: int, coupled: bool,
                 algorithm: str = "direct", owned: Optional[List[bool]] = None, allow_raw: bool = True):
        be, comm = eng.be, eng.comm
        Xs = list(Xs)
        owned = [True] * len(Xs) if owned is None else list(owned)
        if algorithm not in ("direct", "xcov"):
            raise ValueError("algorithm must be 'direct' or 'xcov'")
        self.algorithm_requested = self.algorithm = algorithm
        self.notes: List[str] = []
        validate_limits([tuple(X.shape) for X in Xs], n_components)
# ... 19 lines not shown
            self.half_fallback = fallback_text([dtype_name(d) for d in self.half_storage if d is not None], why)
            self.notes.append(self.half_fallback)

        if any(d is not None for d in self.half_storage):
            why = self._half_declined(want_raw, allow_raw, [tuple(X.shape) for X in Xs], M)
            if why is not None:
                upcast(why)
        if not want_raw:
            for b in range(len(Xs)):
                if not owned[b]:
                    Xs[b] = Xs[b].clone()
        ysum, ycnt = be.colstats(Y)
        comm.allreduce(ysum)
        comm.allreduce(ycnt)
        self.y_mean = ysum / ycnt
        _, ssqy0 = be.center(Y, self.y_mean, False)
        comm.allreduce(ssqy0)
        self.ssqy0 = float(ssqy0.item())
        self._ssq_with_s = (want_raw and hasattr(be, "xcov_ssq") and eng.opt.xcov_ssq_with_s)
        self._ssq0_dev = {}
        self._s_prebuilt = {}
        self.blocks = None
        self._stats_with_s = False
        if (want_raw and self._ssq_with_s and eng.opt.xcov_stats_with_s and hasattr(be, "xcov_stats") and M <= 64
                and eng._probe_plain(Xs)):
            self.blocks = self._blocks_from_one_read(Xs)
            self._stats_with_s = self.blocks is not None
            if self.blocks is None:
                self._s_prebuilt, self._ssq0_dev = {}, {}
                self.notes.append("column statistics from the read that builds S declined: a column sum came out non-finite")
        if self.blocks is None and any(X.dtype in HALF_DTYPES for X in Xs):
            upcast("missing or non-finite values in X (the statistics read shows them; the masked forms write X)")
        if self.blocks is None:
            self.blocks = [eng._prepare_block(X, self.n_total, defer_centring=want_raw) for X in Xs]
        self.raw = want_raw and not any(blk.has_miss for blk in self.blocks)
        raw_declined = None
        if self.raw:
            ratio = eng._offset_ratio(self.blocks, Xs)
            if not ratio <= eng.opt.xcov_raw_max_offset:
                self.raw = False
                raw_declined = f"uncentred xcov form declined: max|column mean| / spread = {ratio:.3g} > {eng.opt.xcov_raw_max_offset:g}"
                self.notes.append(raw_declined)
        if self.raw and not self._ssq_with_s:
            self.raw = all(eng._ssq_uncentred(blk, X) for blk, X in zip(self.blocks, Xs))
        if not self.raw and any(X.dtype in HALF_DTYPES for X in Xs):
            upcast(raw_declined or "the uncentred cross-covariance form declined: no read-only norm of the block")
        for blk, d in zip(self.blocks, self.half_storage):
            if d is not None:
                blk.dtype = d
        if want_raw and not self.raw:
            for b, blk in enumerate(self.blocks):
                if not owned[b]:
                    Xs[b] = Xs[b].clone()
                eng._centre_block(blk, Xs[b])
        if want_raw and not self.raw:
            self._s_prebuilt, self._ssq0_dev, self._stats_with_s = {}, {}, False
        self.X2 = [X.view(I, -1) for X in Xs]
        self.T = be.zeros(I, R)
        self.U = be.zeros(I, R)
        self.Q = be.zeros(M, R)
        self.coef = np.zeros((R, R))
        self.coef_dev = be.zeros(R, R)
        self.b_dev = be.empty(R)
        self.ssq_log = be.zeros(R, len(self.blocks) + 1)
        self.r2y = np.zeros(R)
        for blk in self.blocks:
            blk.loadings = [be.zeros(d, R) for d in blk.shape[1:]]
            blk.r2x = np.zeros(R)
        self.wA = [be.empty(blk.A) for blk in self.blocks]
        for b, blk in enumerate(self.blocks):
            if len(blk.shape) == 2:
                self.wA[b].fill_(1.0)
        self.wB = [be.empty(blk.B) for blk in self.blocks]
        self.Zs = [be.empty(blk.A * blk.B) for blk in self.blocks]
        self.fac = [be.zeros(len(blk.shape) - 1, max(blk.shape[1:])) if len(blk.shape) > 3 else None for blk in self.blocks]
        self.tol = 1e-8
        self.Ts = be.empty(len(self.blocks), I)
        self.t = self.Ts[0] if (len(self.blocks) == 1 and not coupled) else be.empty(I)
        self.status = be.zeros(1 + 2 * len(self.blocks))
        self.status[1::2] = 1.0
        self.status_host = None
        if self.status.is_cuda:
            self.status_host = torch.empty(self.status.shape, dtype=torch.float64, pin_memory=True)
        self.sq_max = int(getattr(be, "rank1_squarings", 30))
        self.sq_budget = [self.sq_max] * len(self.blocks)
        side = int(getattr(be, "rank1_chain_side", 0))
        self.sq_spare = [3 if (len(blk.shape) == 3 and min(blk.A, blk.B) <= side) else 1 for blk in self.blocks]
        self.u = be.empty(I)
        self.u_new = be.empty(I)
        self.q = be.empty(M)
        self.n_iter: List[int] = []
        self.pipeline_stats = {"iterations": 0, "ahead": 0, "unused": 0, "waited": 0, "redone": 0}
        self._executed = 0
        self._parity = 0
        self.mixed = False
        self.use_graphs = False
        self._graphs = {}
        self._graph_error = None
        self._collectives_captured = None
        self._z_ready = False
        self._fused = (algorithm == "direct" and M <= 64
                       and all(hasattr(be, f) for f in ("mode0_contract_yq", "score_gram", "q_update")))
        if self._fused:
            self.Gy = be.empty(M, M)
            self.qbuf = [be.zeros(M), be.zeros(M)]
            self.qpart = be.empty(len(self.blocks), int(be.n_partials) * M)
        elif algorithm == "direct" and comm.sharded:
            self.Gy = be.empty(M, M)
            self.q_prev = be.zeros(M)
        if algorithm == "xcov":
            nb = len(self.blocks)
            self._s_pair = 2 * M <= 64 and eng.opt.xcov_pair_build
            self.S, self.S2, self.S12 = [], [], []
            for blk in self.blocks:
                if blk.has_miss and self._s_pair:
                    both = be.empty(2 * M, blk.A * blk.B)
                    self.S12.append(both)
                    self.S.append(both[:M])
                    self.S2.append(both[M:])
                else:
                    self.S12.append(None)
                    pre = self._s_prebuilt.get(len(self.S))
                    self.S.append(pre if pre is not None else be.empty(M, blk.A * blk.B))
                    self.S2.append(be.empty(M, blk.A * blk.B) if blk.has_miss else None)
            self.rowscale = [(float(blk.A * blk.B) / blk.rowcnt) if blk.has_miss else None for blk in self.blocks]
            any_miss = any(blk.has_miss for blk in self.blocks)
            self.Yw = be.empty(I, 2 * M if self._s_pair else M) if any_miss else None
            self.Gy = be.empty(M, M)
            self.Tq = be.empty(nb, M)
            self.qx = [be.zeros(M), be.zeros(M)]
            self.qc = self.qx[0]
            self.qn = self.Tq[0] if (nb == 1 and not coupled) else be.empty(M)
            self._s_carry = (not any(blk.has_miss for blk in self.blocks)
                             and all(hasattr(be, f) for f in ("s_downdate", "deflate_contract_yq")))
            self._s_ready = False
            self._nowrite = False
            if self.raw:
                self.zM = be.zeros(M)
                self.zA = [be.zeros(blk.A) for blk in self.blocks]
                self.zB = [be.zeros(blk.B) for blk in self.blocks]
            if self._s_carry:
                self.yhat = be.empty(I, 1)
                self.one = be.empty(1)
                self.one.fill_(1.0)
                self.vs = [be.empty(blk.A * blk.B) for blk in self.blocks]
                self._nowrite = eng.opt.xcov_nowrite and hasattr(be, "kr_axpy") and R <= 64
                if self._nowrite:
                    self.dot_log = be.zeros(R, 1 + len(self.blocks))
                    self.Gw = be.empty(R * R)
                    self._G_last = None
                    self._one_read = R > 1 and eng.opt.xcov_one_read and hasattr(be, "score_contract")
                    if self._one_read:
                        self._fused_b = max(range(len(self.blocks)), key=lambda b: self.blocks[b].A * self.blocks[b].B)
                        P0 = self.blocks[self._fused_b].A * self.blocks[self._fused_b].B
                        self.ps = be.empty(P0)
                        self.Rm = be.zeros(P0, R)
                        self.corr = be.empty(I)
                        self.csum = be.empty(1)
            assert self._nowrite or not self.raw, "an uncentred X needs the form of the loop that never writes it"

    def _half_declined(self, want_raw: bool, allow_raw: bool, shapes, M: int) -> Optional[str]:
        eng, be = self.eng, self.eng.be
        if self.algorithm != "xcov":
            return 'algorithm="direct" centres and deflates X in place'
        if not half_route(eng, None, HALF_ENTRIES["fit"])[0]:
            return "the backend has no 16-bit entries"
# ... 58 lines not shown
                comm.allreduce(self.Gy)
            return
        for b, blk in enumerate(self.blocks):
            if self._s_ready:
                break
            if self.S12[b] is not None:
                self.Yw[:, :self.M].copy_(self.Y)
                torch.mul(self.Y, self.rowscale[b][:, None], out=self.Yw[:, self.M:])
                be.xcov(self.X2[b], self.Yw, True, out=self.S12[b], mixed=self.mixed)
                comm.allreduce(self.S12[b])
                continue
            if b in self._s_prebuilt:
                del self._s_prebuilt[b]
            elif self.raw and self._ssq_with_s and b not in self._ssq0_dev:
                _, ssq = be.xcov_ssq(self.X2[b], self.Y, blk.mean, out=self.S[b])
                self._ssq0_dev[b] = comm.allreduce(ssq)
            else:
                be.xcov(self.X2[b], self.Y, blk.has_miss, out=self.S[b], mixed=self.mixed)
            comm.allreduce(self.S[b])
            if self.raw:
                ysum, _ = be.colstats(self.Y)
                comm.allreduce(ysum)
                be.s_downdate(self.S[b], blk.A, blk.B, self.zM, self.zA[b], self.zB[b], ysum, blk.mean)
            if blk.has_miss:
                torch.mul(self.Y, self.rowscale[b][:, None], out=self.Yw)
                be.xcov(self.X2[b], self.Yw, True, out=self.S2[b], mixed=self.mixed)
                comm.allreduce(self.S2[b])
        self._s_ready = False
        be.gram_tn(self.Y, self.Y, out=self.Gy)
        comm.allreduce(self.Gy)
        self._parity = 0
        self.qc = self.qx[0]
        self.qc.zero_()
        self.qc[0] = 1.0

    def inner_loop(self, a: int, max_iter: int, tol: float, verbose: int = 0) -> None:
        if max_iter > 0 and self._pipeline_ok():
            self._pipelined = True
            self._inner_loop_xcov_pipelined(a, max_iter, tol, verbose)
            return
        for it in range(max_iter):
            du = self.iterate(it)
            if du is not None and du < tol:
                if verbose:
                    print("Comp {}: converged after {} iterations".format(a, it))
                break

    def _update_budgets(self, host) -> bool:
        retry = False
        for b in range(len(self.blocks)):
            conv, used = host[1 + 2 * b] > 0.5, int(host[2 + 2 * b])
            if used < 0:
                self._chain_gave_up()
                retry = True
                continue
            if not conv and self.sq_budget[b] < self.sq_max:
                self.sq_budget[b] = self.sq_max
                retry = True
            elif conv and len(self.blocks[b].shape) == 3:
                if not self.use_graphs or used + 1 > self.sq_budget[b] or used + 3 < self.sq_budget[b]:
                    self.sq_budget[b] = min(self.sq_max, used + (1 if self.use_graphs else self.sq_spare[b]))
        return retry

    def _peer_failed(self, host, first_attempt: bool) -> bool:
        if not self.eng.comm.sharded:
            return False
        if first_attempt:
            self._nan_tails = 0
        if np.isfinite(float(host[0])) or self._nan_tails > int(getattr(self.eng.comm, "world", 1)):
            return False
        self._nan_tails += 1
        return True

    def _chain_gave_up(self) -> None:
        be = self.eng.be
        if hasattr(be, "rank1_chain_gave_up"):
            be.rank1_chain_gave_up()
        self._graphs.clear()
        self.sq_spare = [1] * len(self.blocks)
        note = "rank-1 chain of squarings in one launch switched off: a workgroup never became resident (GPU shared with another process)"
        if note not in self.notes:
            self.notes.append(note)

    def _read_status(self) -> np.ndarray:
        if self.status_host is None:
            return self.status.cpu().numpy()
        self.status_host.copy_(self.status, non_blocking=True)
        torch.cuda.current_stream(self.status.device).synchronize()
        return self.status_host.numpy()

    def _run(self, key, fn) -> None:
        if not self.use_graphs:
            fn()
            return
        g = self._graphs.get(key)
        if g is not None:
            g.replay()
            return
        fn()
        try:
            g = torch.cuda.CUDAGraph()
            with torch.cuda.graph(g, capture_error_mode="thread_local"):
                fn()
            self._graphs[key] = g
        except Exception as e:
            self.use_graphs = False
            self._graph_error = repr(e)
            self._after_failed_capture()

    def _run_with_collectives(self, key, fn) -> bool:
        if not (self.use_graphs and self.eng.opt.capture_collectives and self._collectives_captured is not False):
            return False
        if not getattr(self.eng.comm, "capturable", False):
            self._collectives_captured = False
            self.notes.append(f"all-reduces not captured into the iteration's graph: the {getattr(self.eng.comm, 'backend', None)} "
                              "backend stages through the host (only RCCL collectives are stream-ordered kernels)")
            return False
        g = self._graphs.get(key)
        if g is not None:
            g.replay()
            return True
        fn()
        try:
            torch.cuda.current_stream().synchronize()
            g = torch.cuda.CUDAGraph()
            with torch.cuda.graph(g, capture_error_mode="thread_local"):
                fn()
            self._graphs[key] = g
            self._collectives_captured = True
        except Exception as e:
            self._collectives_captured = False
            self.notes.append("all-reduces not captured into the iteration's graph: " + repr(e)[:200])
            self._after_failed_capture()
        return True

    def _after_failed_capture(self) -> None:
        try:
            torch.cuda.synchronize()
        except Exception:
            pass
        if hasattr(self.eng.be, "clear_error"):
            self.eng.be.clear_error()

    def iterate(self, it: int) -> Optional[float]:
        if self.algorithm == "xcov":
            return self._iterate_xcov(it)
        be, comm = self.eng.be, self.eng.comm
        if self._fused:
            return self._iterate_fused(it)
        self._executed += 1
        sharded = comm.sharded
        par = self._parity
        u, u_new = (self.u, self.u_new) if par == 0 else (self.u_new, self.u)

        def seg_contract():
            for b, blk in enumerate(self.blocks):
                be.mode0_contract(self.X2[b], u, blk.has_miss, out=self.Zs[b])

        def seg_colscale():
            for b, blk in enumerate(self.blocks):
                if blk.has_miss:
                    be.colscale(self.Zs[b], blk.colcnt, self.n_total)

        def seg_loadings_scores():
            for b, blk in enumerate(self.blocks):
                self.eng._rank1(blk, self.Zs[b], self.wA[b], self.wB[b], info=self.status[1 + 2 * b: 3 + 2 * b],
                                n_squarings=self.sq_budget[b], fac=self.fac[b], tol=self.tol)
                be.score(self.X2[b], blk.A, blk.B, self.wA[b], self.wB[b],
                         blk.rowcnt if blk.has_miss else None, self.Ts[b])
            if self.t.data_ptr() != self.Ts.data_ptr():
                be.scores_mean(self.Ts, self.t)
            be.gram_tn(self.Y, self.t, out=self.q)

        def seg_y_update():
            be.normalize(self.q)
            if sharded:
                be.rowdot(self.Y, self.q, u_new, None)
                be.quadform(self.Gy, self.q, self.q_prev if it > 0 else self.q, self.status[0:1])
            else:
                be.rowdot(self.Y, self.q, u_new, u if it > 0 else None, du2=self.status[0:1])

        first = True
        while True:
            budgets = tuple(self.sq_budget)
            if not sharded:
                def whole():
                    if first:
                        seg_contract()
                        seg_colscale()
                    seg_loadings_scores()
                    seg_y_update()
                self._run(("iter", it > 0, par, budgets, first), whole)
            else:
                if first:
                    self._run(("contract", par), seg_contract)
                    for b in range(len(self.blocks)):
                        comm.allreduce(self.Zs[b])
                    seg_colscale()
                self._run(("loadings", budgets), seg_loadings_scores)
                comm.allreduce(self.q)
                self._run(("yupdate", it > 0, par), seg_y_update)
            host = self._read_status()
            local, peer = self._update_budgets(host), self._peer_failed(host, first)
            if not (local or peer):
                break
            first = False
        if sharded:
            self.q_prev.copy_(self.q)
        self._parity ^= 1
        return None if it == 0 else math.sqrt(max(float(host[0]), 0.0))

    def _iterate_fused(self, it: int) -> Optional[float]:
        be, comm = self.eng.be, self.eng.comm
        self._executed += 1
        sharded = comm.sharded
        par = self._parity
        q_cur, q_new = self.qbuf[par], self.qbuf[par ^ 1]
        nparts = len(self.blocks) * int(be.n_partials)

        def seg_contract():
            for b, blk in enumerate(self.blocks):
                if be.mode0_contract_yq(self.X2[b], self.Y, q_cur, blk.has_miss, out=self.Zs[b]) is None:
                    be.rowdot(self.Y, q_cur, self.u, None)
                    be.mode0_contract(self.X2[b], self.u, blk.has_miss, out=self.Zs[b])

        def seg_colscale():
            for b, blk in enumerate(self.blocks):
                if blk.has_miss:
                    be.colscale(self.Zs[b], blk.colcnt, self.n_total)

        def seg_loadings_scores():
            for b, blk in enumerate(self.blocks):
                self.eng._rank1(blk, self.Zs[b], self.wA[b], self.wB[b], info=self.status[1 + 2 * b: 3 + 2 * b],
                                n_squarings=self.sq_budget[b], fac=self.fac[b], tol=self.tol)
                if be.score_gram(self.X2[b], blk.A, blk.B, self.wA[b], self.wB[b], blk.rowcnt if blk.has_miss else None,
                                 self.Ts[b], self.Y, self.qpart[b]) is None:
                    raise RuntimeError("score_gram refused a shape the fused iteration was planned for")
            if sharded:
                be.q_update(q_new, self.qpart, normalize=False, nparts=nparts)

        def seg_y_update():
            if sharded:
                be.q_update(q_new, None, normalize=True, G=self.Gy, q_prev=q_cur, du2=self.status[0:1])
            else:
                be.q_update(q_new, self.qpart, normalize=True, G=self.Gy, q_prev=q_cur, du2=self.status[0:1], nparts=nparts)

        have_z = self._z_ready and it == 0
        self._z_ready = False
        first = True
        while True:
            budgets = tuple(self.sq_budget)
            if not sharded:
                def whole():
                    if first:
                        if not have_z:
                            seg_contract()
                        seg_colscale()
                    seg_loadings_scores()
                    seg_y_update()
                self._run(("fiter", par, budgets, first, have_z), whole)
            else:
                def whole_sharded():
                    if first:
                        if not have_z:
                            seg_contract()
                        for b in range(len(self.blocks)):
                            comm.allreduce(self.Zs[b])
                        seg_colscale()
                    seg_loadings_scores()
                    comm.allreduce(q_new)
                    seg_y_update()
                if not self._run_with_collectives(("fiter+ar", par, budgets, first, have_z), whole_sharded):
                    if first:
                        if not have_z:
                            self._run(("fcontract", par), seg_contract)
                        for b in range(len(self.blocks)):
                            comm.allreduce(self.Zs[b])
                        seg_colscale()
                    self._run(("floadings", par, budgets), seg_loadings_scores)
                    comm.allreduce(q_new)
                    self._run(("fyupdate", par), seg_y_update)
            host = self._read_status()
            local, peer = self._update_budgets(host), self._peer_failed(host, first)
            if not (local or peer):
                break
            first = False
        self._parity ^= 1
        self.q = q_new
        return None if it == 0 else math.sqrt(max(float(host[0]), 0.0))

    def finish_component(self, a: int) -> None:
        be, comm = self.eng.be, self.eng.comm
        self.n_iter.append(self._executed)
        ssqs = []
        if self.algorithm == "xcov" and self._s_carry:
            if self._nowrite:
                self._finish_xcov_nowrite(a)
            else:
                self._finish_xcov_carry(a)
            return
        if (self.algorithm == "xcov" and len(self.blocks) == 1 and self.blocks[0].has_miss and self.S12[0] is not None
                and a + 1 < self.R and hasattr(be, "xcov_deflate") and self.eng.opt.xcov_deflate_build
                and getattr(self, "_deflate_build_ok", True)):
            if self._finish_xcov_masked_fused(a):
                return
        if self.algorithm == "xcov":
            self.q = self.qc
            if len(self.blocks) == 1:
                blk = self.blocks[0]
                rc = blk.rowcnt if blk.has_miss else None
                s0 = be.score_deflate(self.X2[0], blk.A, blk.B, self.wA[0], self.wB[0], rc, self.t)
                if s0 is None:
                    be.score(self.X2[0], blk.A, blk.B, self.wA[0], self.wB[0], rc, self.t)
                    s0 = be.deflate(self.X2[0], blk.A, blk.B, self.t, self.wA[0], self.wB[0])
                ssqs.append(s0)
            else:
                for b, blk in enumerate(self.blocks):
                    be.score(self.X2[b], blk.A, blk.B, self.wA[b], self.wB[b], blk.rowcnt if blk.has_miss else None, self.Ts[b])
                be.scores_mean(self.Ts, self.t)
                for b, blk in enumerate(self.blocks):
                    ssqs.append(be.deflate(self.X2[b], blk.A, blk.B, self.t, self.wA[b], self.wB[b]))
            be.rowdot(self.Y, self.q, self.u, None)
        if self.algorithm == "direct" and self._fused:
            be.rowdot(self.Y, self.q, self.u, None)
            if self.t.data_ptr() != self.Ts.data_ptr():
                be.scores_mean(self.Ts, self.t)
        elif self.algorithm == "direct" and self._parity == 1:
            self.u.copy_(self.u_new)
            self._parity = 0
        self.T[:, a].copy_(self.t)
        self.U[:, a].copy_(self.u)
        self.Q[:, a].copy_(self.q)
        for b, blk in enumerate(self.blocks):
            if len(blk.shape) == 2:
                blk.loadings[0][:, a].copy_(self.wB[b])
            elif len(blk.shape) == 3:
                blk.loadings[0][:, a].copy_(self.wA[b])
                blk.loadings[1][:, a].copy_(self.wB[b])
            else:
                for m, d in enumerate(blk.shape[1:]):
                    blk.loadings[m][:, a].copy_(self.fac[b][m, :d])
            if self.algorithm == "direct" and not self._fused:
                ssqs.append(be.deflate(self.X2[b], blk.A, blk.B, self.t, self.wA[b], self.wB[b]))
        if self.algorithm == "direct" and self._fused:
            self._finish_fused(a)
            return
        b_dev, _ = self._inner_regression(a)
        for b in range(len(self.blocks)):
            self.ssq_log[a, b].copy_(ssqs[b].reshape(()))
        ssqy = be.y_deflate(self.Y, self.T, a + 1, b_dev, self.q)
        self.ssq_log[a, len(self.blocks)].copy_(ssqy.reshape(()))

    def _inner_regression(self, a: int, extra: Optional[torch.Tensor] = None):
        be, comm = self.eng.be, self.eng.comm
        k = a + 1
        Ta = self.T[:, :k]
        G = be.gram_tn(Ta, Ta)
        g = be.gram_tn(Ta, self.u)
        if comm.sharded:
            packed = torch.cat([G.reshape(-1), g.reshape(-1)] + ([extra.reshape(-1)] if extra is not None else []))
            comm.allreduce(packed)
            G, g = packed[: k * k].view(k, k), packed[k * k: k * k + k]
            extra = packed[k * k + k:] if extra is not None else None
        b_dev = be.normal_solve(G, g.reshape(-1), out=self.b_dev[:k])
        self.coef_dev[:k, a].copy_(b_dev)
        self._G_last = G
        return b_dev, extra

    def _finish_fused(self, a: int) -> None:
        be, comm = self.eng.be, self.eng.comm
        k = a + 1
        b_dev, _ = self._inner_regression(a)
        ssqy = be.y_deflate(self.Y, self.T, k, b_dev, self.q)
        ssqs = []
        self._z_ready = False
        if k < self.R:
            q0 = self.qbuf[0]
            q0.zero_()
            q0[0] = 1.0
            ready = True
            for b, blk in enumerate(self.blocks):
                s_b = be.deflate_contract_yq(self.X2[b], blk.A, blk.B, self.t, self.wA[b], self.wB[b], self.Y, q0,
                                             blk.has_miss, out=self.Zs[b])
                if s_b is None:
                    s_b = be.deflate(self.X2[b], blk.A, blk.B, self.t, self.wA[b], self.wB[b])
                    ready = False
                ssqs.append(s_b)
            self._z_ready = ready
        else:
            for b, blk in enumerate(self.blocks):
                ssqs.append(be.deflate(self.X2[b], blk.A, blk.B, self.t, self.wA[b], self.wB[b]))
        self._log_ssq(a, ssqs, ssqy)

    def _log_ssq(self, a: int, ssqs, ssqy) -> None:
        for b in range(len(self.blocks)):
            self.ssq_log[a, b].copy_(ssqs[b].reshape(()))
        self.ssq_log[a, len(self.blocks)].copy_(ssqy.reshape(()))

    def _store_component(self, a: int) -> None:
        self.T[:, a].copy_(self.t)
        self.U[:, a].copy_(self.u)
        self.Q[:, a].copy_(self.q)
        self._store_loadings(a)

    def _store_loadings(self, a: int) -> None:
        for b, blk in enumerate(self.blocks):
            if len(blk.shape) == 2:
                blk.loadings[0][:, a].copy_(self.wB[b])
            elif len(blk.shape) == 3:
                blk.loadings[0][:, a].copy_(self.wA[b])
                blk.loadings[1][:, a].copy_(self.wB[b])
            else:
                for m, d in enumerate(blk.shape[1:]):
                    blk.loadings[m][:, a].copy_(self.fac[b][m, :d])

    def result(self) -> FitState:
        if getattr(self, "_state", None) is not None:
            return self._state
        nb = len(self.blocks)
        nowrite = self.algorithm == "xcov" and getattr(self, "_nowrite", False)
        for b, ssq in getattr(self, "_ssq0_dev", {}).items():
            self.blocks[b].ssq0 = float(ssq.item())
        self.eng.comm.allreduce(self.ssq_log)
        parts = [self.coef_dev.reshape(-1), self.ssq_log.reshape(-1)]
        if nowrite:
            self.eng.comm.allreduce(self.dot_log)
            parts.append(self.dot_log.reshape(-1))
        host = torch.cat(parts).cpu().numpy()
        R = self.R
        self.coef[...] = host[: R * R].reshape(R, R)
        ssq = host[R * R: R * R + R * (nb + 1)].reshape(R, nb + 1).copy()
        if nowrite:
            dots = host[R * R + R * (nb + 1):].reshape(R, 1 + nb)
            for b, blk in enumerate(self.blocks):
                run = blk.ssq0
                for a in range(len(self.n_iter)):
                    run = run - 2.0 * dots[a, 1 + b] + dots[a, 0]
                    ssq[a, b] = run
        for a in range(len(self.n_iter)):
            for b, blk in enumerate(self.blocks):
                blk.r2x[a] = 1.0 - ssq[a, b] / blk.ssq0
            self.r2y[a] = 1.0 - ssq[a, nb] / self.ssqy0
        self._state = FitState(coupled=self.coupled, n_components=self.R, blocks=self.blocks, T=self.T, U=self.U, Q=self.Q,
                               coef=self.coef, r2y=self.r2y, y_mean=self.y_mean, n_iter=self.n_iter,
                               n_samples_total=self.n_total, report=self.build_report())
        return self._state

    def build_report(self) -> Dict[str, object]:
        eng, comm, nb = self.eng, self.eng.comm, len(self.blocks)
        rep: Dict[str, object] = {
            "form": "regular", "algorithm_requested": self.algorithm_requested, "algorithm": self.algorithm,
            "shapes": [tuple(b.shape) for b in self.blocks], "storage": [dtype_name(b.dtype) for b in self.blocks],
            "missing": [bool(b.has_miss) for b in self.blocks], "responses": self.M,
            "sharded": bool(comm.sharded), "world": int(comm.world),
            "graphs": bool(self.use_graphs and self._graphs), "graph_error": self._graph_error,
            "collectives_in_graph": self._collectives_captured is True,
            "backend": getattr(eng.be, "name", type(eng.be).__name__),
        }
        if self.algorithm == "direct":
            rep["y_side"] = "fused into the sweeps" if self._fused else "separate launches"
            if not self._fused and self.M > 64:
                self.notes.append("Y side not fused into the sweeps: more than 64 responses")
            rep["x_passes_per_iteration"] = "2 reads"
            rep["x_passes_per_component"] = ("1 read + write (deflation fused with the next contraction)" if self._fused
                                             else "1 read + write (deflation)")
            rep["x_copy"] = "centred private copy"
        else:
            nowrite = bool(getattr(self, "_nowrite", False))
            one_read = nowrite and bool(getattr(self, "_one_read", False))
            any_miss = any(b.has_miss for b in self.blocks)
            rep["x_copy"] = "none: the caller's uncentred tensor is read in place" if self.raw else "centred private copy"
            rep["raw"] = bool(self.raw)
            rep["x_written"] = not nowrite
            rep["s_carried"] = bool(self._s_carry)
            rep["s_build"] = ("per component (missing values)" if any_miss else "first component only") + \
                             (f", {(self.M + 63) // 64} response tiles of <= 64" if self.M > 64 else "") + \
                             (", [Y, Y * rowscale] in one pass" if any(x is not None for x in self.S12) else "")
            rep["one_read"] = one_read
            rep["stats_with_s"] = bool(getattr(self, "_stats_with_s", False))
            if nowrite:
                rep["x_passes_per_component"] = ("1 read (largest block); 2 reads (other blocks)" if one_read and nb > 1 else
                                                 "1 read" if one_read else "2 reads")
            elif any_miss and nb == 1 and getattr(self, "_deflate_build_ok", True) and self.S12[0] is not None and eng.opt.xcov_deflate_build:
                rep["x_passes_per_component"] = "1 read + 1 read + write (deflation inside the rebuild of S)"
            elif any_miss:
                rep["x_passes_per_component"] = "1 read + write (score + deflation) + S rebuild reads"
            else:
                rep["x_passes_per_component"] = "1 read + 1 read + write"
            rep["pipelined"] = bool(getattr(self, "_pipelined", False))
            if rep["pipelined"]:
                rep["pipeline"] = dict(self.pipeline_stats)
            if not rep["pipelined"] and eng.opt.xcov_pipeline:
                why = ("graph replay requested" if self.use_graphs else "more than 64 responses" if self.M > 64 else
                       "a block of order > 3 or a backend without the single-call iteration")
                self.notes.append("inner loop on S not pipelined: " + why)
            if self.algorithm_requested == "xcov" and not self.raw and eng.opt.xcov_raw and not any_miss and not any("uncentred" in n for n in self.notes):
                self.notes.append("uncentred xcov form declined: " + ("more than 64 components" if self.R > 64 else
                                                                      "f32 matrix precision or a backend without its kernels"))
            if nowrite and eng.opt.xcov_one_read and self.R > 1 and not one_read:
                self.notes.append("one read per component declined: the row does not fit the registers of 1..16 workgroups "
                                  "(rows of 2048..131072 f32 -- 262144 when the last mode divides 4096 -- / 1024..131072 f64 elements, "
                                  "last mode a multiple of 4 / 2)")
        if any(d is not None for d in self.half_storage):
            rep["half_storage"] = {
                "in_place": self.half_fallback is None,
                "fallback": self.half_fallback,
                "reads": [None if d is None or self.half_fallback is not None else self._half_reads_form(b)
                          for b, d in enumerate(self.half_storage)],
            }
        rep["rank1_one_launch_chain"] = bool(getattr(eng.be, "rank1_chain_side", 0)) and any(
            len(blk.shape) == 3 and min(blk.A, blk.B) <= int(getattr(eng.be, "rank1_chain_side", 0)) for blk in self.blocks)
        rep["declined"] = list(self.notes)
        return rep
```

cmtf_pls_amd/fitrun_xcov.py:

```python
from __future__ import annotations

import math
from typing import Optional

import torch

from .storage import HALF_DTYPES


class XcovMixin:
    def _score_x0(self, b: int, out: torch.Tensor) -> None:
        be, blk, X2 = self.eng.be, self.blocks[b], self.X2[b]
        if X2.dtype in HALF_DTYPES:
            self.half_reads.setdefault(b, set()).add("mttkrp")
            if be.mttkrp(X2, blk.A, blk.B, self.wA[b].view(-1, 1), self.wB[b].view(-1, 1), out.view(-1, 1)) is None:
                raise RuntimeError("mttkrp refused a shape the 16-bit fit was planned for")
        else:
            be.score(X2, blk.A, blk.B, self.wA[b], self.wB[b], None, out)

    def _contract_x0(self, b: int, v: torch.Tensor, out: torch.Tensor) -> None:
        be, X2 = self.eng.be, self.X2[b]
        if X2.dtype in HALF_DTYPES:
            self.half_reads.setdefault(b, set()).add("xcov")
            if be.xcov(X2, v.view(-1, 1), False, out=out.view(1, -1)) is None:
                raise RuntimeError("xcov refused a block the 16-bit fit was planned for")
        else:
            be.mode0_contract(X2, v, False, out=out)

    def _iterate_xcov(self, it: int) -> Optional[float]:
        be = self.eng.be
        self._executed += 1

        blk0 = self.blocks[0]
        composite = (len(self.blocks) == 1 and len(blk0.shape) == 3 and not blk0.has_miss and self.M <= 64
                     and self.qn.data_ptr() == self.Tq.data_ptr() and hasattr(be, "xcov_iterate"))

        par = self._parity
        q_cur, q_new = self.qx[par], self.qx[par ^ 1]

        def seg(first: bool):
            if composite:
                be.xcov_iterate(self.S[0], blk0.A, blk0.B, q_cur, self.Zs[0], self.wA[0], self.wB[0], self.status[1:3],
                                self.sq_budget[0], q_new, self.Gy, self.status[0:1], first)
                return
            if first:
                for b, blk in enumerate(self.blocks):
                    be.mode0_contract(self.S[b], self.qc, False, out=self.Zs[b])
                    if blk.has_miss:
                        be.colscale(self.Zs[b], blk.colcnt, self.n_total)
            for b, blk in enumerate(self.blocks):
                self.eng._rank1(blk, self.Zs[b], self.wA[b], self.wB[b], info=self.status[1 + 2 * b: 3 + 2 * b],
                                n_squarings=self.sq_budget[b], fac=self.fac[b], tol=self.tol)
                be.score_s(self.S2[b] if blk.has_miss else self.S[b], blk.A, blk.B, self.wA[b], self.wB[b], self.Tq[b])
            if self.qn.data_ptr() != self.Tq.data_ptr():
                be.scores_mean(self.Tq, self.qn)
            be.normalize(self.qn)
            if it > 0:
                be.quadform(self.Gy, self.qn, self.qc, self.status[0:1])

        first = True
        while True:
            self._run(("xcov", it > 0, tuple(self.sq_budget), first, par if composite else -1), lambda: seg(first))
            host = self._read_status()
            if not self._update_budgets(host):
                break
            first = False
        if composite:
            self._parity ^= 1
            self.qc = q_new
        else:
            self.qc.copy_(self.qn)
        return None if it == 0 else math.sqrt(max(float(host[0]), 0.0))

    def _single_composite(self) -> bool:
        blk0 = self.blocks[0]
        return (len(self.blocks) == 1 and len(blk0.shape) == 3 and not blk0.has_miss and self.M <= 64
                and self.qn.data_ptr() == self.Tq.data_ptr() and hasattr(self.eng.be, "xcov_iterate"))

    def _pipeline_ok(self) -> bool:
        be = self.eng.be
        if self.algorithm != "xcov" or self.use_graphs or not self.eng.opt.xcov_pipeline:
            return False
        if self.M > 64 or not all(hasattr(be, f) for f in ("status_snapshot", "status_wait")):
            return False
        return self._single_composite() or (hasattr(be, "xcov_blocks_plan") and all(len(blk.shape) in (2, 3) for blk in self.blocks))

    def _inner_loop_xcov_pipelined(self, a: int, max_iter: int, tol: float, verbose: int) -> None:
        be = self.eng.be
        nb = len(self.blocks)
        single = self._single_composite()
        pp = getattr(self, "_pipe", None)
        if pp is None:
            M = self.M
            second = {"Z": [], "wA": [], "wB": []}
            for b, blk in enumerate(self.blocks):
                second["Z"].append(be.empty(blk.A * blk.B))
                second["wA"].append(self.wA[b].clone())
                second["wB"].append(be.empty(blk.B))
            pp = self._pipe = {
                "q": [self.qx[0], self.qx[1], be.zeros(M)],
                "Z": [list(self.Zs), second["Z"]], "wA": [list(self.wA), second["wA"]], "wB": [list(self.wB), second["wB"]],
                "status": [be.zeros(1 + 2 * nb), be.zeros(1 + 2 * nb)],
                "plans": {}, "slots": {},
            }
            for st in pp["status"]:
                st[1::2] = 1.0
        plans = pp["plans"]

        def make_plan(it: int):
            s = it & 1
            st, q_cur, q_new = pp["status"][s], pp["q"][it % 3], pp["q"][(it + 1) % 3]
            if single:
                blk0 = self.blocks[0]
                if hasattr(be, "xcov_iterate_plan"):
                    one = be.xcov_iterate_plan(self.S[0], blk0.A, blk0.B, q_cur, pp["Z"][s][0], pp["wA"][s][0], pp["wB"][s][0], st,
                                               q_new, self.Gy)
                    return lambda nsq, first: one(nsq[0], first)
                return lambda nsq, first: be.xcov_iterate(self.S[0], blk0.A, blk0.B, q_cur, pp["Z"][s][0], pp["wA"][s][0],
                                                          pp["wB"][s][0], st[1:3], nsq[0], q_new, self.Gy, st[0:1], first)
            descr = [dict(S=self.S[b], S2=self.S2[b] if blk.has_miss else None, colcnt=blk.colcnt if blk.has_miss else None,
                          n_samples=self.n_total, order=len(blk.shape), A=blk.A, B=blk.B,
                          Z=pp["Z"][s][b], wA=pp["wA"][s][b], wB=pp["wB"][s][b]) for b, blk in enumerate(self.blocks)]
            return be.xcov_blocks_plan(descr, self.M, q_cur, self.Tq, q_new, self.Gy, st)

        def enqueue(it: int, first: bool = True):
            plan = plans.get(it % 6)
            if plan is None:
                plan = plans[it % 6] = make_plan(it)
            plan([n if it > 0 else min(self.sq_max, n + 4) for n in self.sq_budget], first)
            return be.status_snapshot(pp["status"][it & 1], it & 1, slots=pp["slots"])

        stats = self.pipeline_stats
        it, tok = 0, enqueue(0)
        du_prev = du = None
        while True:
            ahead = None
            if it + 1 < max_iter:
                predicted = None if (du is None or du_prev is None or du_prev <= 0.0) else du * (du / du_prev)
                if it == 0 or predicted is None or predicted >= tol:
                    ahead = enqueue(it + 1)
                    stats["ahead"] += 1
            host = be.status_wait(tok)
            short = [b for b in range(nb) if not host[1 + 2 * b] > 0.5 and self.sq_budget[b] < self.sq_max]
            if any(host[2 + 2 * b] < 0 for b in range(nb)):
                self._chain_gave_up()
                pp["plans"].clear()
                tok = enqueue(it, first=False)
                stats["redone"] += 1
                continue
            if short:
                for b in short:
                    self.sq_budget[b] = self.sq_max
                tok = enqueue(it, first=False)
                stats["redone"] += 1
                continue
            for b, blk in enumerate(self.blocks):
                if len(blk.shape) == 3 and host[1 + 2 * b] > 0.5:
                    self.sq_budget[b] = min(self.sq_max, int(host[2 + 2 * b]) + self.sq_spare[b])
            self._executed += 1
            stats["iterations"] += 1
            du_prev, du = du, (None if it == 0 else math.sqrt(max(float(host[0]), 0.0)))
            if (du is not None and du < tol) or it + 1 >= max_iter:
                if verbose and du is not None and du < tol:
                    print("Comp {}: converged after {} iterations".format(a, it))
                stats["unused"] += ahead is not None
                break
            it += 1
            stats["waited"] += ahead is None
            tok = ahead if ahead is not None else enqueue(it)
        if it & 1:
            for b in range(nb):
                self.wA[b].copy_(pp["wA"][1][b])
                self.wB[b].copy_(pp["wB"][1][b])
        self.qc = pp["q"][(it + 1) % 3]
        self._parity = 0

    def _finish_xcov_masked_fused(self, a: int) -> bool:
        be, comm = self.eng.be, self.eng.comm
        blk, M = self.blocks[0], self.M
        if blk.A * blk.B % 4 != 0:
            self._deflate_build_ok = False
            return False
        self.q = self.qc
        be.score(self.X2[0], blk.A, blk.B, self.wA[0], self.wB[0], blk.rowcnt, self.t)
        be.rowdot(self.Y, self.q, self.u, None)
        self._store_component(a)
        b_dev, _ = self._inner_regression(a)
        ssqy = be.y_deflate(self.Y, self.T, a + 1, b_dev, self.q)
        self.Yw[:, :M].copy_(self.Y)
        torch.mul(self.Y, self.rowscale[0][:, None], out=self.Yw[:, M:])
        ssq = be.xcov_deflate(self.X2[0], blk.A, blk.B, self.Yw, self.t, self.wA[0], self.wB[0], out=self.S12[0])
        if ssq is None:
            self._deflate_build_ok = False
            ssq = be.deflate(self.X2[0], blk.A, blk.B, self.t, self.wA[0], self.wB[0])
        else:
            comm.allreduce(self.S12[0])
            self._s_ready = True
        self._log_ssq(a, [ssq], ssqy)
        return True

    def _finish_xcov_carry(self, a: int) -> None:
        be, comm = self.eng.be, self.eng.comm
        self.q = self.qc
        for b, blk in enumerate(self.blocks):
            be.score(self.X2[b], blk.A, blk.B, self.wA[b], self.wB[b], None, self.Ts[b])
        if self.t.data_ptr() != self.Ts.data_ptr():
            be.scores_mean(self.Ts, self.t)
        be.rowdot(self.Y, self.q, self.u, None)
        self._store_component(a)
        k = a + 1
        Ta = self.T[:, :k]
        ya = be.gram_tn(self.Y, self.t).reshape(-1)
        b_dev, ya_g = self._inner_regression(a, extra=ya)
        ssqs = []
        if k < self.R:
            be.rowdot(Ta, b_dev, self.yhat.view(-1), None)
        ssqy = be.y_deflate(self.Y, self.T, k, b_dev, self.q)
        if k < self.R:
            carried = True
            for b, blk in enumerate(self.blocks):
                s_b = be.deflate_contract_yq(self.X2[b], blk.A, blk.B, self.t, self.wA[b], self.wB[b], self.yhat, self.one,
                                             False, out=self.vs[b])
                if s_b is None:
                    s_b = be.deflate(self.X2[b], blk.A, blk.B, self.t, self.wA[b], self.wB[b])
                    carried = False
# ... 95 lines not shown
```

cmtf_pls_amd/options.py:

```python
from __future__ import annotations

from dataclasses import dataclass, replace
from typing import Optional


@dataclass(frozen=True)
class EngineOptions:
    small_fit: bool = True
    small_fit_elements: int = 1 << 15
    xcov_nowrite: bool = True
    xcov_raw: bool = True
    xcov_raw_max_offset: float = 1e4
    project_raw_max_offset: float = 1e4
    xcov_one_read: bool = True
    xcov_pair_build: bool = True
    xcov_ssq_with_s: bool = True
    xcov_stats_with_s: bool = True
    xcov_deflate_build: bool = True
    xcov_pipeline: bool = True
    capture_collectives: bool = False
    project_split_rows: bool = True
    masked_folds: bool = False
    masked_folds_coupled: bool = False
    coupled_permutations: bool = False
    tensor_folds: bool = False
    tensor_folds_coupled: bool = False
    masked_tensor_folds: bool = False
    tensor_resamples_coupled: bool = False
    masked_tensor_folds_coupled: bool = False
    half_folds: bool = False
    half_diagnostics: bool = False

    def but(self, **changes) -> "EngineOptions":
        return replace(self, **changes)


_DEFAULT_OPTIONS = EngineOptions()


def default_options() -> EngineOptions:
    return _DEFAULT_OPTIONS


def set_default_options(options: Optional[EngineOptions]) -> EngineOptions:
    global _DEFAULT_OPTIONS
    old, _DEFAULT_OPTIONS = _DEFAULT_OPTIONS, (options if options is not None else EngineOptions())
    return old
```

include/cmtfpls.h:

```cpp
#ifndef CMTFPLS_H
#define CMTFPLS_H

#include <stddef.h>
#include <stdint.h>

#ifdef __cplusplus
extern "C" {
#endif

#define CMTFPLS_OK 0
#define CMTFPLS_EINVAL 1
#define CMTFPLS_EWORKSPACE 2
#define CMTFPLS_EHIP 3
#define CMTFPLS_EUNSUPPORTED 4

int cmtfpls_abi_version(void);
const char* cmtfpls_last_error(void);
int cmtfpls_clear_error(void);
int cmtfpls_status_to_host(const void* src, void* dst_host, size_t bytes, void* event, void* stream);

size_t cmtfpls_colstats_workspace_bytes(int64_t I, int64_t P);
int cmtfpls_colstats_f32(const float* X, int64_t I, int64_t P, double* colsum, double* colcnt,
                         void* ws, size_t ws_bytes, void* stream);
int cmtfpls_colstats_f64(const double* X, int64_t I, int64_t P, double* colsum, double* colcnt,
                         void* ws, size_t ws_bytes, void* stream);
int cmtfpls_sweep_partials(void);
int cmtfpls_center_f32(float* X, int64_t I, int64_t P, const double* mean, double* rowcnt,
                       double* ssq_part, void* stream);
int cmtfpls_center_f64(double* X, int64_t I, int64_t P, const double* mean, double* rowcnt,
                       double* ssq_part, void* stream);

size_t cmtfpls_mode0_contract_workspace_bytes(int64_t I, int64_t P);
int cmtfpls_mode0_contract_f32(const float* X, int64_t I, int64_t P, const double* u, double* Z,
                               int masked, void* ws, size_t ws_bytes, void* stream);
int cmtfpls_mode0_contract_f64(const double* X, int64_t I, int64_t P, const double* u, double* Z,
                               int masked, void* ws, size_t ws_bytes, void* stream);
int cmtfpls_mode0_contract_yq_f32(const float* X, int64_t I, int64_t P, const double* Y, int ldy, int M,
                                  const double* q, double* Z, int masked, void* ws, size_t ws_bytes, void* stream);
int cmtfpls_mode0_contract_yq_f64(const double* X, int64_t I, int64_t P, const double* Y, int ldy, int M,
                                  const double* q, double* Z, int masked, void* ws, size_t ws_bytes, void* stream);
int cmtfpls_colscale_f64(double* Z, int64_t P, const double* colcnt, double n_samples, void* stream);

size_t cmtfpls_rank1_workspace_bytes(int A, int B);
int cmtfpls_rank1_f64(const double* Z, int A, int B, double* wA, double* wB, double* sigma, double* info,
                      int n_squarings, void* ws, size_t ws_bytes, void* stream);
int cmtfpls_rank1_launches_f64(const double* Z, int A, int B, double* wA, double* wB, double* sigma, double* info,
                               int n_squarings, void* ws, size_t ws_bytes, void* stream);
void cmtfpls_rank1_chain_enable(int on);
int cmtfpls_rank1_chain_enabled(void);
int cmtfpls_rank1_score_f64(const double* Z, int A, int B, double* wA, double* wB, double* info, int n_squarings,
                            const double* S, int M, double* tq, void* ws, size_t ws_bytes, void* stream);
int cmtfpls_normalize_f64(double* v, int64_t n, double* nrm, void* stream);
size_t cmtfpls_rank1_tensor_workspace_bytes(const int* dims, int n);
int cmtfpls_rank1_tensor_f64(const double* Z, const int* dims, int n, double tol, double* factors, int ld,
                             double* info, int n_squarings, void* ws, size_t ws_bytes, void* stream);
int cmtfpls_kron_f64(const double* a, int na, const double* b, int nb, double* out, void* stream);

size_t cmtfpls_xcov_workspace_bytes(int64_t I, int64_t P, int M);
int cmtfpls_xcov_f32(const float* X, int64_t I, int64_t P, const double* Y, int ldy, int M, double* S,
                     int masked, void* ws, size_t ws_bytes, void* stream);
int cmtfpls_xcov_f64(const double* X, int64_t I, int64_t P, const double* Y, int ldy, int M, double* S,
                     int masked, void* ws, size_t ws_bytes, void* stream);
int cmtfpls_quadform_f64(const double* G, int M, const double* q, const double* q_old, double* out, void* stream);
int cmtfpls_xcov_bf16(const uint16_t* X, int64_t I, int64_t P, const double* Y, int ldy, int M, double* S,
                      int masked, void* ws, size_t ws_bytes, void* stream);
int cmtfpls_xcov_f16(const uint16_t* X, int64_t I, int64_t P, const double* Y, int ldy, int M, double* S,
                     int masked, void* ws, size_t ws_bytes, void* stream);
int cmtfpls_xcov_deflate_f32(float* X, int64_t I, int A, int B, const double* Y, int ldy, int M, const double* t, const double* wA,
                             const double* wB, double* S, double* ssq, void* ws, size_t ws_bytes, void* stream);
int cmtfpls_xcov_deflate_f64(double* X, int64_t I, int A, int B, const double* Y, int ldy, int M, const double* t, const double* wA,
                             const double* wB, double* S, double* ssq, void* ws, size_t ws_bytes, void* stream);
size_t cmtfpls_xcov_ssq_workspace_bytes(int64_t I, int64_t P, int M);
size_t cmtfpls_xcov_stats_workspace_bytes(int64_t I, int64_t P, int M);
int cmtfpls_xcov_stats_f32(const float* X, int64_t I, int64_t P, const double* Y, int ldy, int M, double* S, double* stats,
                           void* ws, size_t ws_bytes, void* stream);
int cmtfpls_xcov_stats_f64(const double* X, int64_t I, int64_t P, const double* Y, int ldy, int M, double* S, double* stats,
                           void* ws, size_t ws_bytes, void* stream);
int cmtfpls_xcov_stats_bf16(const uint16_t* X, int64_t I, int64_t P, const double* Y, int ldy, int M, double* S, double* stats,
                            void* ws, size_t ws_bytes, void* stream);
int cmtfpls_xcov_stats_f16(const uint16_t* X, int64_t I, int64_t P, const double* Y, int ldy, int M, double* S, double* stats,
                           void* ws, size_t ws_bytes, void* stream);
int cmtfpls_xcov_ssq_f32(const float* X, int64_t I, int64_t P, const double* Y, int ldy, int M, double* S, const double* mean,
                         double* ssq, void* ws, size_t ws_bytes, void* stream);
int cmtfpls_xcov_ssq_f64(const double* X, int64_t I, int64_t P, const double* Y, int ldy, int M, double* S, const double* mean,
                         double* ssq, void* ws, size_t ws_bytes, void* stream);
int cmtfpls_xcov_iterate_f64(const double* S, int M, int A, int B, const double* q_cur, double* Z, double* wA,
                             double* wB, double* info, int n_squarings, double* q_new, const double* G, double* du2,
                             int first, void* ws_contract, size_t ws_contract_bytes, void* ws_rank1,
                             size_t ws_rank1_bytes, void* stream);
typedef struct {
  const double* S;
  const double* S2;
  const double* colcnt;
  double n_samples;
  int order;
  int A, B;
  int n_squarings;
  double* Z;
  double* wA;
  double* wB;
  double* info;
} cmtfpls_xcov_block;
int cmtfpls_xcov_iterate_blocks_f64(const cmtfpls_xcov_block* blocks, int nb, int M, const double* q_cur, double* tq, double* q_new,
                                    const double* G, double* du2, int first, void* ws_rank1, size_t ws_rank1_bytes, void* stream);
int cmtfpls_s_downdate_f64(double* S, int M, int A, int B, const double* ya, const double* wA, const double* wB,
                           const double* q, const double* v, void* stream);
int cmtfpls_kr_axpy_f64(double* v, int A, int B, const double* WA, const double* WB, int ld, int k, const double* coef, void* stream);
int cmtfpls_axpy_scalar_f64(double* y, int64_t n, const double* a, const double* x, void* stream);
size_t cmtfpls_score_contract_workspace_bytes(int64_t I, int64_t P);
int cmtfpls_score_contract_f32(const float* X, int64_t I, int A, int B, const double* wA, const double* wB, const double* shift,
                               const double* sub_own, const double* add_other, double alpha, double* t, double* Z, double* csum,
                               void* ws, size_t ws_bytes, void* stream);
int cmtfpls_score_contract_f64(const double* X, int64_t I, int A, int B, const double* wA, const double* wB, const double* shift,
                               const double* sub_own, const double* add_other, double alpha, double* t, double* Z, double* csum,
                               void* ws, size_t ws_bytes, void* stream);
int cmtfpls_score_contract_bf16(const uint16_t* X, int64_t I, int A, int B, const double* wA, const double* wB, const double* shift,
                                const double* sub_own, const double* add_other, double alpha, double* t, double* Z, double* csum,
                                void* ws, size_t ws_bytes, void* stream);
int cmtfpls_score_contract_f16(const uint16_t* X, int64_t I, int A, int B, const double* wA, const double* wB, const double* shift,
                               const double* sub_own, const double* add_other, double alpha, double* t, double* Z, double* csum,
                               void* ws, size_t ws_bytes, void* stream);
int cmtfpls_xcov_f32_mixed(const float* X, int64_t I, int64_t P, const double* Y, int ldy, int M, double* S,
                           int masked, void* ws, size_t ws_bytes, void* stream);
int cmtfpls_mttkrp_f32_mixed(const float* X, int64_t I, int A, int B, const double* WA, const double* WB, int R,
                             double* out, int ldo, void* stream);

int cmtfpls_mttkrp_f32(const float* X, int64_t I, int A, int B, const double* WA, const double* WB, int R,
                       double* out, int ldo, void* stream);
int cmtfpls_mttkrp_f64(const double* X, int64_t I, int A, int B, const double* WA, const double* WB, int R,
                       double* out, int ldo, void* stream);
int cmtfpls_mttkrp_bf16(const uint16_t* X, int64_t I, int A, int B, const double* WA, const double* WB, int R,
                        double* out, int ldo, void* stream);
int cmtfpls_mttkrp_f16(const uint16_t* X, int64_t I, int A, int B, const double* WA, const double* WB, int R,
                       double* out, int ldo, void* stream);

int cmtfpls_score_f32(const float* X, int64_t I, int A, int B, const double* wA, const double* wB,
                      const double* rowcnt, double* t, void* stream);
int cmtfpls_score_f64(const double* X, int64_t I, int A, int B, const double* wA, const double* wB,
                      const double* rowcnt, double* t, void* stream);
int cmtfpls_score_s_f64(const double* S, int M, int A, int B, const double* wA, const double* wB, double* tq, void* stream);

size_t cmtfpls_deflate_contract_workspace_bytes(int64_t I, int64_t P);
int cmtfpls_deflate_contract_yq_f32(float* X, int64_t I, int A, int B, const double* t, const double* wA,
                                    const double* wB, const double* Y, int ldy, int M, const double* q, double* Z,
                                    int masked, double* ssq, void* ws, size_t ws_bytes, void* stream);
int cmtfpls_deflate_contract_yq_f64(double* X, int64_t I, int A, int B, const double* t, const double* wA,
                                    const double* wB, const double* Y, int ldy, int M, const double* q, double* Z,
                                    int masked, double* ssq, void* ws, size_t ws_bytes, void* stream);
int cmtfpls_score_gram_f32(const float* X, int64_t I, int A, int B, const double* wA, const double* wB,
                           const double* rowcnt, double* t, const double* Y, int ldy, int M, double* qpart,
                           void* stream);
int cmtfpls_score_gram_f64(const double* X, int64_t I, int A, int B, const double* wA, const double* wB,
                           const double* rowcnt, double* t, const double* Y, int ldy, int M, double* qpart,
                           void* stream);
int cmtfpls_q_update_f64(const double* qpart, int nblk, int M, double* q, int normalize, const double* G,
                         const double* q_prev, double* du2, void* stream);

int cmtfpls_deflate_f32(float* X, int64_t I, int A, int B, const double* t, const double* wA,
                        const double* wB, double* ssq_part, void* stream);
int cmtfpls_deflate_f64(double* X, int64_t I, int A, int B, const double* t, const double* wA,
                        const double* wB, double* ssq_part, void* stream);

int cmtfpls_score_deflate_f32(float* X, int64_t I, int A, int B, const double* wA, const double* wB,
                              const double* rowcnt, double* t, double* ssq_part, void* stream);
int cmtfpls_score_deflate_f64(double* X, int64_t I, int A, int B, const double* wA, const double* wB,
                              const double* rowcnt, double* t, double* ssq_part, void* stream);

int cmtfpls_sweep_form(const char* op, int elem_bytes, int64_t I, int A, int B, int masked, int M,
                       int aligned16, char* out, size_t n);
int cmtfpls_sweep_form_list(const char* op, int elem_bytes, char* out, size_t n);

size_t cmtfpls_small_workspace_bytes(void);
int cmtfpls_gram_tn_f64(const double* A, int lda, int a, const double* B, int ldb, int b, int64_t I,
                        double* C, void* ws, size_t ws_bytes, void* stream);
int cmtfpls_rowdot_f64(const double* Y, int ldy, int M, int64_t I, const double* q, double* u,
                       const double* u_old, double* du2, void* ws, size_t ws_bytes, void* stream);
int cmtfpls_scores_mean_f64(const double* Ts, int nb, int64_t I, double* out, void* stream);
int cmtfpls_y_deflate_f64(double* Y, int ldy, int M, int64_t I, const double* T, int ldt, int R,
                          const double* b, const double* q, double* ssq, void* ws, size_t ws_bytes,
                          void* stream);
int cmtfpls_sum_f64(const double* in, int64_t n, double* out, void* stream);

int cmtfpls_project_rows_f32(const float* X, int64_t I, int A, int B, int R, const double* WA, const double* WB,
                             const double* mean, double* scores, int ld, void* stream);
int cmtfpls_project_rows_f64(const double* X, int64_t I, int A, int B, int R, const double* WA, const double* WB,
                             const double* mean, double* scores, int ld, void* stream);
int cmtfpls_project_rows2_f32(const float* X0, int A0, int B0, const double* WA0, const double* WB0, const double* mean0,
                              const float* X1, int A1, int B1, const double* WA1, const double* WB1, const double* mean1,
                              int64_t I, int R, double* scores, int ld, void* stream);
int cmtfpls_project_rows2_f64(const double* X0, int A0, int B0, const double* WA0, const double* WB0, const double* mean0,
                              const double* X1, int A1, int B1, const double* WA1, const double* WB1, const double* mean1,
                              int64_t I, int R, double* scores, int ld, void* stream);
int cmtfpls_project_rows_idx_f32(const float* X, const int64_t* rows, int64_t n_rows, int A, int B, int R, const double* WA,
                                 const double* WB, const double* mean, double* scores, int ld, void* stream);
int cmtfpls_project_rows_idx_f64(const double* X, const int64_t* rows, int64_t n_rows, int A, int B, int R, const double* WA,
                                 const double* WB, const double* mean, double* scores, int ld, void* stream);
int cmtfpls_project_rows2_idx_f32(const float* X0, int A0, int B0, const double* WA0, const double* WB0, const double* mean0,
                                  const float* X1, int A1, int B1, const double* WA1, const double* WB1, const double* mean1,
                                  const int64_t* rows, int64_t n_rows, int R, double* scores, int ld, void* stream);
int cmtfpls_project_rows2_idx_f64(const double* X0, int A0, int B0, const double* WA0, const double* WB0, const double* mean0,
                                  const double* X1, int A1, int B1, const double* WA1, const double* WB1, const double* mean1,
                                  const int64_t* rows, int64_t n_rows, int R, double* scores, int ld, void* stream);

int cmtfpls_allreduce_sum_f64(void* comm, double* buf, size_t count, void* stream);
int cmtfpls_allreduce_sum_f32(void* comm, float* buf, size_t count, void* stream);

int cmtfpls_normal_solve_f64(const double* G, const double* g, int k, double* b, int incb, void* stream);
size_t cmtfpls_normal_solve_workspace_bytes(int k);
int cmtfpls_normal_solve_ws_f64(const double* G, const double* g, int k, double* b, int incb, void* ws, size_t ws_bytes,
                                void* stream);
int cmtfpls_unit_upper_solve_rows_f64(double* M, int64_t I, int ld, int R, const double* U, const double* shift, int* nan_flag,
                                      void* stream);
int cmtfpls_kr_gram_f64(const double* L, int n, int R, double* G, int first, double scale, void* stream);
int cmtfpls_kr_gram_row_f64(const double* L, int n, int R, int a, double* g, int first, void* stream);
int cmtfpls_khatri_rao_f64(const double* Am, int na, const double* Bm, int nb, int R, double* out, void* stream);
int cmtfpls_predict_rows_f64(const double* S, int64_t I, int lds, int R, const double* Bm, int M, const double* mean,
                             double* out, int ldo, void* stream);
int cmtfpls_recon_f32(const double* T, int64_t I, int ldt, int R, const double* WA, const double* WB, int A, int B,
                      const double* mean, float* out, void* stream);
int cmtfpls_recon_f64(const double* T, int64_t I, int ldt, int R, const double* WA, const double* WB, int A, int B,
                      const double* mean, double* out, void* stream);
size_t cmtfpls_recon_r2_workspace_bytes(int64_t I, int64_t P);
int cmtfpls_recon_r2_f32(const float* X, const double* T, int64_t I, int ldt, int R, const double* WA, const double* WB,
                         int A, int B, const double* mean, double* out, void* ws, size_t ws_bytes, void* stream);
int cmtfpls_recon_r2_f64(const double* X, const double* T, int64_t I, int ldt, int R, const double* WA, const double* WB,
                         int A, int B, const double* mean, double* out, void* ws, size_t ws_bytes, void* stream);
int cmtfpls_recon_r2_bf16(const uint16_t* X, const double* T, int64_t I, int ldt, int R, const double* WA, const double* WB,
                          int A, int B, const double* mean, double* out, void* ws, size_t ws_bytes, void* stream);
int cmtfpls_recon_r2_f16(const uint16_t* X, const double* T, int64_t I, int ldt, int R, const double* WA, const double* WB,
                         int A, int B, const double* mean, double* out, void* ws, size_t ws_bytes, void* stream);

size_t cmtfpls_resid_rows_workspace_bytes(int64_t I, int64_t P);
int cmtfpls_resid_rows_f32(const float* X, const double* T, int64_t I, int ldt, int R, const double* WA, const double* WB,
                           int A, int B, const double* mean, double* rows, double* cols, void* ws, size_t ws_bytes, void* stream);
int cmtfpls_resid_rows_f64(const double* X, const double* T, int64_t I, int ldt, int R, const double* WA, const double* WB,
                           int A, int B, const double* mean, double* rows, double* cols, void* ws, size_t ws_bytes, void* stream);
int cmtfpls_resid_rows_bf16(const uint16_t* X, const double* T, int64_t I, int ldt, int R, const double* WA, const double* WB,
                            int A, int B, const double* mean, double* rows, double* cols, void* ws, size_t ws_bytes, void* stream);
int cmtfpls_resid_rows_f16(const uint16_t* X, const double* T, int64_t I, int ldt, int R, const double* WA, const double* WB,
// ... 215 lines not shown
```

Measured before the change: 760.0.

## Deliver per-iteration NIPALS status through a mapped host mailbox instead of copy+event

Adds a pinned, host-mapped coherent mailbox that GPU kernels write status words and a sequence counter into. The host polls that memory instead of enqueuing a device-to-host copy and synchronizing on an event each iteration. It also lets the chain-region preset be skipped when it is already armed, which drops one kernel launch per iteration. In exchange it adds a host spin-wait with a timeout and depends on the coherence and ordering of mapped memory on the GPU.

```diff
diff --git a/cmtf_pls_amd/_lib.py b/cmtf_pls_amd/_lib.py
--- a/cmtf_pls_amd/_lib.py
+++ b/cmtf_pls_amd/_lib.py
@@ -34,6 +34,15 @@
     "cmtfpls_last_error": (c_char_p, []),
     "cmtfpls_clear_error": (c_int, []),
     "cmtfpls_status_to_host": (c_int, [_P, _P, c_size_t, _P, _P]),
+    "cmtfpls_mailbox_create": (c_int, [c_int, ctypes.POINTER(_P)]),
+    "cmtfpls_mailbox_destroy": (c_int, [_P]),
+    "cmtfpls_mailbox_host": (_P, [_P]),
+    "cmtfpls_host_wait": (c_int, [_P, c_uint64, _P, c_int, c_double, _P, c_int]),
+    "cmtfpls_q_update_mailbox_f64": (c_int, [_P, c_int, c_int, _P, c_int, _P, _P, _P, c_int, _P, _P]),
+    "cmtfpls_xcov_iterate_mailbox_f64": (c_int, [_P, c_int, c_int, c_int, _P, _P, _P, _P, _P, c_int, _P, _P, _P, c_int, _P, c_size_t, c_int, _P, _P]),
+    "cmtfpls_xcov_iterate_blocks_mailbox_f64": (c_int, [ctypes.POINTER(XcovBlock), c_int, c_int, _P, _P, _P, _P, _P, c_int, _P, c_size_t, c_int, _P, _P]),
+    "cmtfpls_xcov_preset_merge_enable": (None, [c_int]),
+    "cmtfpls_xcov_preset_merge_enabled": (c_int, []),
     "cmtfpls_colstats_workspace_bytes": (c_size_t, [c_int64, c_int64]),
     "cmtfpls_colstats_f32": (c_int, [_P, c_int64, c_int64, _P, _P, _P, c_size_t, _P]),
     "cmtfpls_colstats_f64": (c_int, [_P, c_int64, c_int64, _P, _P, _P, c_size_t, _P]),
diff --git a/cmtf_pls_amd/backend.py b/cmtf_pls_amd/backend.py
--- a/cmtf_pls_amd/backend.py
+++ b/cmtf_pls_amd/backend.py
@@ -3,6 +3,7 @@
 import ctypes
 from typing import Optional, Tuple
 
+import numpy as np
 import torch
 
 from . import _lib
@@ -27,6 +28,37 @@
 def chunk_size(n: int, per: int, budget: int, cap: Optional[int] = None) -> int:
     chunk = max(1, min(int(n), int(budget) // max(int(per), 1)))
     return chunk if cap is None else min(chunk, int(cap))
+
+
+class Mailbox:
+
+    def __init__(self, lib, n_words: int):
+        handle = ctypes.c_void_p()
+        _lib.check(lib.cmtfpls_mailbox_create(int(n_words), ctypes.byref(handle)), "mailbox_create")
+        self.lib, self.handle, self.n = lib, handle, int(n_words)
+        self.host = lib.cmtfpls_mailbox_host(handle)
+        self._words = (ctypes.c_uint64 * (1 + self.n)).from_address(self.host)
+        self.out = np.zeros(self.n)
+        self._out_ptr = self.out.ctypes.data
+        self.count = 0
+
+    def sequence(self) -> int:
+        return int(self._words[0])
+
+    def payload(self) -> "np.ndarray":
+        return np.frombuffer(self._words, dtype=np.float64, count=self.n, offset=8).copy()
+
+    def wait(self, want: int, stream, timeout: float = 120.0) -> "np.ndarray":
+        rc = self.lib.cmtfpls_host_wait(self.host, int(want), self._out_ptr, self.n, float(timeout), stream, 1)
+        if rc:
+            _lib.check(rc, "host_wait")
+        return self.out
+
+    def close(self) -> None:
+        if self.handle is not None:
+            self._words = None
+            self.lib.cmtfpls_mailbox_destroy(self.handle)
+            self.handle = None
 
 
 class HipBackend:
@@ -40,6 +72,7 @@
         self.n_partials = int(self.lib.cmtfpls_sweep_partials())
         self._ws = {}
         self._status_slots = {}
+        self._mailboxes_free = []
         self.rank1_squarings = 30
         self.rank1_chain_side = 256 if self.lib.cmtfpls_rank1_chain_enabled() else 0
 
@@ -271,8 +304,34 @@
         token[1].synchronize()
         return token[2]
 
+    def mailbox_acquire(self, n_words: int) -> Optional[Mailbox]:
+        for i, mb in enumerate(self._mailboxes_free):
+            if mb.n == n_words:
+                del self._mailboxes_free[i]
+                mb.count = mb.sequence()
+                return mb
+        try:
+            with torch.cuda.device(self.device):
+                return Mailbox(self.lib, n_words)
+        except _lib.CmtfplsError:
+            self.clear_error()
+            return None
+
+    def mailbox_release(self, mb: Optional[Mailbox]) -> None:
+        if mb is not None and mb.handle is not None:
+            self._mailboxes_free.append(mb)
+
+    def mailbox_wait(self, mb: Mailbox, want: int, timeout: float = 120.0) -> "np.ndarray":
+        return mb.wait(want, self._stream(), timeout)
+
+    def xcov_preset_merge(self, on: Optional[bool] = None) -> bool:
+        if on is not None:
+            self.lib.cmtfpls_xcov_preset_merge_enable(int(bool(on)))
+        return bool(self.lib.cmtfpls_xcov_preset_merge_enabled())
+
     def xcov_iterate_plan(self, S: torch.Tensor, A: int, B: int, q_cur: torch.Tensor, Z: torch.Tensor, wA: torch.Tensor,
-                          wB: torch.Tensor, status: torch.Tensor, q_new: torch.Tensor, G: torch.Tensor):
+                          wB: torch.Tensor, status: torch.Tensor, q_new: torch.Tensor, G: torch.Tensor,
+                          mailbox: Optional[Mailbox] = None):
         M, P = S.shape
         wc = self._workspace("contract", self.lib.cmtfpls_mode0_contract_workspace_bytes(M, P))
         wr = self._workspace("rank1", self.lib.cmtfpls_rank1_workspace_bytes(A, B))
@@ -282,6 +341,15 @@
         tail = (_ptr(wc), wc.numel(), _ptr(wr), wr.numel())
         qn, Gp, du2 = _ptr(q_new), _ptr(G), status[0:1].data_ptr()
         stream = self._stream
+        if mailbox is not None:
+            assert status.is_contiguous() and status.numel() <= mailbox.n
+            fnm, tailm = self.lib.cmtfpls_xcov_iterate_mailbox_f64, (_ptr(wr), wr.numel(), status.numel() - 1, mailbox.handle)
+
+            def enqueue_mailbox(n_squarings: int, first: bool, _keep=keep + (mailbox,)) -> None:
+                rc = fnm(*head, n_squarings, qn, Gp, du2, 1 if first else 0, *tailm, stream())
+                if rc:
+                    _lib.check(rc, "xcov_iterate_mailbox")
+            return enqueue_mailbox
 
         def enqueue(n_squarings: int, first: bool, _keep=keep) -> None:
             rc = fn(*head, n_squarings, qn, Gp, du2, 1 if first else 0, *tail, stream())
@@ -291,16 +359,22 @@
 
     def xcov_iterate(self, S: torch.Tensor, A: int, B: int, q_cur: torch.Tensor, Z: torch.Tensor, wA: torch.Tensor,
                      wB: torch.Tensor, info: torch.Tensor, n_squarings: int, q_new: torch.Tensor, G: torch.Tensor,
-                     du2: torch.Tensor, first: bool) -> None:
+                     du2: torch.Tensor, first: bool, mailbox: Optional[Mailbox] = None, n_status: int = 0) -> None:
         M, P = S.shape
         wc = self._workspace("contract", self.lib.cmtfpls_mode0_contract_workspace_bytes(M, P))
         wr = self._workspace("rank1", self.lib.cmtfpls_rank1_workspace_bytes(A, B))
+        if mailbox is not None:
+            _lib.check(self.lib.cmtfpls_xcov_iterate_mailbox_f64(_ptr(S), M, A, B, _ptr(q_cur), _ptr(Z), _ptr(wA), _ptr(wB), _ptr(info),
+                                                                 int(n_squarings), _ptr(q_new), _ptr(G), _ptr(du2), int(first),
+                                                                 _ptr(wr), wr.numel(), int(n_status), mailbox.handle, self._stream()),
+                       "xcov_iterate_mailbox")
+            return
         _lib.check(self.lib.cmtfpls_xcov_iterate_f64(_ptr(S), M, A, B, _ptr(q_cur), _ptr(Z), _ptr(wA), _ptr(wB), _ptr(info),
                                                      int(n_squarings), _ptr(q_new), _ptr(G), _ptr(du2), int(first),
                                                      _ptr(wc), wc.numel(), _ptr(wr), wr.numel(), self._stream()), "xcov_iterate")
 
     def xcov_blocks_plan(self, blocks, M: int, q_cur: torch.Tensor, tq: torch.Tensor, q_new: torch.Tensor, G: torch.Tensor,
-                         status: torch.Tensor):
+                         status: torch.Tensor, mailbox: Optional[Mailbox] = None):
         nb = len(blocks)
         if M > 64 or any(b["order"] not in (2, 3) for b in blocks) or tq.numel() != nb * M or not tq.is_contiguous():
             return None
@@ -320,6 +394,9 @@
         fn, stream = self.lib.cmtfpls_xcov_iterate_blocks_f64, self._stream
         args = (nb, M, _ptr(q_cur), _ptr(tq), _ptr(q_new), _ptr(G), status[0:1].data_ptr())
         tail = (_ptr(wr), wr.numel())
+        if mailbox is not None:
+            assert status.is_contiguous() and status.numel() <= mailbox.n
+            fn, tail, keep = self.lib.cmtfpls_xcov_iterate_blocks_mailbox_f64, tail + (status.numel() - 1, mailbox.handle), keep + (mailbox,)
 
         def enqueue(n_squarings, first: bool, _keep=keep) -> None:
             for i in range(nb):
@@ -394,10 +471,15 @@
 
     def q_update(self, q: torch.Tensor, qpart: Optional[torch.Tensor] = None, normalize: bool = True,
                  G: Optional[torch.Tensor] = None, q_prev: Optional[torch.Tensor] = None,
-                 du2: Optional[torch.Tensor] = None, nparts: Optional[int] = None) -> None:
+                 du2: Optional[torch.Tensor] = None, nparts: Optional[int] = None, mailbox: Optional[Mailbox] = None,
+                 n_status: int = 0) -> None:
         M = q.numel()
         nrows = (nparts or self.n_partials) if qpart is not None else 0
         assert qpart is None or (qpart.is_contiguous() and qpart.numel() >= nrows * M)
+        if mailbox is not None:
+            _lib.check(self.lib.cmtfpls_q_update_mailbox_f64(_ptr(qpart), nrows, M, _ptr(q), int(normalize), _ptr(G), _ptr(q_prev),
+                                                             _ptr(du2), int(n_status), mailbox.handle, self._stream()), "q_update_mailbox")
+            return
         _lib.check(self.lib.cmtfpls_q_update_f64(_ptr(qpart), nrows, M, _ptr(q), int(normalize),
                                                  _ptr(G), _ptr(q_prev), _ptr(du2), self._stream()), "q_update")
 
diff --git a/cmtf_pls_amd/csrc/common.hpp b/cmtf_pls_amd/csrc/common.hpp
--- a/cmtf_pls_amd/csrc/common.hpp
+++ b/cmtf_pls_amd/csrc/common.hpp
@@ -163,4 +163,16 @@
 void set_error(const char* msg);
 int check_launch(const char* what);
 
+struct Mailbox {
+  unsigned long long* host;
+  unsigned long long* dev;
+  unsigned long long* counter;
+  int n_words;
+};
+
+constexpr unsigned long long kChainEmpty = ~0ull;
+int64_t rank1_chain_region(int A, int B, int n_squarings, void* ws, size_t ws_bytes, unsigned long long** region);
+int rank1_score_armed(const double* Z, int A, int B, double* wA, double* wB, double* info, int n_squarings, const double* S, int M,
+                      double* tq, void* ws, size_t ws_bytes, void* stream, int64_t armed_words);
+
 }
diff --git a/cmtf_pls_amd/csrc/rank1.hip b/cmtf_pls_amd/csrc/rank1.hip
--- a/cmtf_pls_amd/csrc/rank1.hip
+++ b/cmtf_pls_amd/csrc/rank1.hip
@@ -155,7 +155,6 @@
   }
 }
 
-constexpr unsigned long long kChainEmpty = ~0ull;
 constexpr int kChainMaxSteps = 31;
 constexpr int kChainSpin = 1 << 15;
 
@@ -597,7 +596,8 @@
 }
 
 static int rank1_run(const double* Z, int A, int B, double* wA, double* wB, double* sigma, double* info,
-                     int n_squarings, void* ws, size_t ws_bytes, void* stream, const double* S, int M, double* tq, bool allow_chain = true);
+                     int n_squarings, void* ws, size_t ws_bytes, void* stream, const double* S, int M, double* tq, bool allow_chain = true,
+                     int64_t armed_words = 0);
 
 int cmtfpls_rank1_f64(const double* Z, int A, int B, double* wA, double* wB, double* sigma, double* info,
                       int n_squarings, void* ws, size_t ws_bytes, void* stream) {
@@ -617,19 +617,12 @@
 
 int cmtfpls_rank1_score_f64(const double* Z, int A, int B, double* wA, double* wB, double* info, int n_squarings,
                             const double* S, int M, double* tq, void* ws, size_t ws_bytes, void* stream) {
-  if (!S || !tq || M <= 0) { set_error("rank1_score: bad argument"); return CMTFPLS_EINVAL; }
-  const int64_t P = (int64_t)A * B;
-  if (M > 64 || P < 8192 || (B % 2) != 0 || ((size_t)(((A + 1) & ~1) + B) * sizeof(double)) > 60 * 1024 ||
-      (reinterpret_cast<uintptr_t>(S) & 15) != 0) {
-    int rc = cmtfpls_rank1_f64(Z, A, B, wA, wB, nullptr, info, n_squarings, ws, ws_bytes, stream);
-    if (rc == CMTFPLS_OK) rc = cmtfpls_score_s_f64(S, M, A, B, wA, wB, tq, stream);
-    return rc;
-  }
-  return rank1_run(Z, A, B, wA, wB, nullptr, info, n_squarings, ws, ws_bytes, stream, S, M, tq);
+  return rank1_score_armed(Z, A, B, wA, wB, info, n_squarings, S, M, tq, ws, ws_bytes, stream, 0);
 }
 
 static int rank1_run(const double* Z, int A, int B, double* wA, double* wB, double* sigma, double* info,
-                     int n_squarings, void* ws, size_t ws_bytes, void* stream, const double* S, int M, double* tq, bool allow_chain) {
+                     int n_squarings, void* ws, size_t ws_bytes, void* stream, const double* S, int M, double* tq, bool allow_chain,
+                     int64_t armed_words) {
   if (!Z || !wA || !wB || A <= 0 || B <= 0) { set_error("rank1: bad argument"); return CMTFPLS_EINVAL; }
   const int n = A < B ? A : B, k = A < B ? B : A;
   if (n > kTile * kMaxTiles) { set_error("rank1: min(A, B) > 4096 unsupported"); return CMTFPLS_EUNSUPPORTED; }
@@ -673,7 +666,8 @@
     double* gave_up = fros + steps * (size_t)nt * nt;
     gave = gave_up;
     const int64_t words = (int64_t)(steps * (nn + nt + (size_t)nt * nt) + 1);
-    hipLaunchKernelGGL(chain_preset_kernel, dim3((unsigned)((words + 2047) / 2048)), dim3(256), 0, st, reinterpret_cast<unsigned long long*>(chain_region), words);
+    if (armed_words != words)
+      hipLaunchKernelGGL(chain_preset_kernel, dim3((unsigned)((words + 2047) / 2048)), dim3(256), 0, st, reinterpret_cast<unsigned long long*>(chain_region), words);
     const dim3 cgrid(nt, (g_chain_on.load(std::memory_order_relaxed) == 2 && nt > 1) ? nt - 1 : nt);
     hipLaunchKernelGGL(syrk_chain_kernel, cgrid, block, 0, st, M0, n, k, gbufs, trs, fros, gave_up, ctl, n_squarings);
     hipLaunchKernelGGL(rank1_seed_xy_kernel, dim3(ny_blocks + (n + 3) / 4), dim3(256), (size_t)n * sizeof(double), st,
@@ -699,3 +693,36 @@
 }
 
 }
+
+namespace cmtfpls {
+
+int64_t rank1_chain_region(int A, int B, int n_squarings, void* ws, size_t ws_bytes, unsigned long long** region) {
+  if (A <= 0 || B <= 0 || !ws || !region) return 0;
+  const int n = A < B ? A : B, k = A < B ? B : A;
+  if (n > kTile * kMaxTiles || (size_t)n * sizeof(double) > 64 * 1024 || ws_bytes < cmtfpls_rank1_workspace_bytes(A, B)) return 0;
+  if (n_squarings < 1) n_squarings = 1;
+  if (n_squarings > kMaxSteps) n_squarings = kMaxSteps;
+  const int nt = (n + kTile - 1) / kTile;
+  if (!g_chain_on.load(std::memory_order_relaxed) || nt * nt > 256 || nt * nt > chain_slots() || n_squarings > kChainMaxSteps) return 0;
+  const size_t off = align_up(rank1_ctl_bytes(nt), 256) + 3 * align_up((size_t)n * n * sizeof(double), 256) +
+                     align_up((size_t)A * B * sizeof(double), 256) + align_up((size_t)n * sizeof(double), 256) +
+                     align_up((size_t)k * sizeof(double), 256);
+  const size_t nn = (size_t)n * n, steps = (size_t)n_squarings + 1;
+  *region = reinterpret_cast<unsigned long long*>(static_cast<char*>(ws) + off);
+  return (int64_t)(steps * (nn + nt + (size_t)nt * nt) + 1);
+}
+
+int rank1_score_armed(const double* Z, int A, int B, double* wA, double* wB, double* info, int n_squarings, const double* S, int M,
+                      double* tq, void* ws, size_t ws_bytes, void* stream, int64_t armed_words) {
+  if (!S || !tq || M <= 0) { set_error("rank1_score: bad argument"); return CMTFPLS_EINVAL; }
+  const int64_t P = (int64_t)A * B;
+  if (M > 64 || P < 8192 || (B % 2) != 0 || ((size_t)(((A + 1) & ~1) + B) * sizeof(double)) > 60 * 1024 ||
+      (reinterpret_cast<uintptr_t>(S) & 15) != 0) {
+    int rc = rank1_run(Z, A, B, wA, wB, nullptr, info, n_squarings, ws, ws_bytes, stream, nullptr, 0, nullptr, true, armed_words);
+    if (rc == CMTFPLS_OK) rc = cmtfpls_score_s_f64(S, M, A, B, wA, wB, tq, stream);
+    return rc;
+  }
+  return rank1_run(Z, A, B, wA, wB, nullptr, info, n_squarings, ws, ws_bytes, stream, S, M, tq, true, armed_words);
+}
+
+}
diff --git a/cmtf_pls_amd/csrc/runtime.hip b/cmtf_pls_amd/csrc/runtime.hip
--- a/cmtf_pls_amd/csrc/runtime.hip
+++ b/cmtf_pls_amd/csrc/runtime.hip
@@ -1,4 +1,7 @@
 #include <string.h>
+
+#include <chrono>
+#include <new>
 
 #include "common.hpp"
 
@@ -37,4 +40,78 @@
   if (e != hipSuccess) { cmtfpls::set_error(hipGetErrorString(e)); return CMTFPLS_EHIP; }
   return CMTFPLS_OK;
 }
+
+int cmtfpls_mailbox_create(int n_words, void** mailbox) {
+  using cmtfpls::Mailbox;
+  if (n_words <= 0 || n_words > 4096 || !mailbox) { cmtfpls::set_error("mailbox_create: bad argument"); return CMTFPLS_EINVAL; }
+  *mailbox = nullptr;
+  Mailbox* mb = new (std::nothrow) Mailbox{nullptr, nullptr, nullptr, n_words};
+  if (!mb) { cmtfpls::set_error("mailbox_create: out of memory"); return CMTFPLS_EHIP; }
+  const size_t bytes = (size_t)(1 + n_words) * sizeof(unsigned long long);
+  hipError_t e = hipHostMalloc(reinterpret_cast<void**>(&mb->host), bytes, hipHostMallocMapped | hipHostMallocCoherent);
+  if (e == hipSuccess) {
+    memset(mb->host, 0, bytes);
+    e = hipHostGetDevicePointer(reinterpret_cast<void**>(&mb->dev), mb->host, 0);
+  }
+  if (e == hipSuccess) e = hipMalloc(reinterpret_cast<void**>(&mb->counter), sizeof(unsigned long long));
+  if (e == hipSuccess) e = hipMemset(mb->counter, 0, sizeof(unsigned long long));
+  if (e != hipSuccess) {
+    cmtfpls::set_error(hipGetErrorString(e));
+    (void)hipGetLastError();
+    if (mb->counter) (void)hipFree(mb->counter);
+    if (mb->host) (void)hipHostFree(mb->host);
+    delete mb;
+    return CMTFPLS_EHIP;
+  }
+  *mailbox = mb;
+  return CMTFPLS_OK;
 }
+
+int cmtfpls_mailbox_destroy(void* mailbox) {
+  cmtfpls::Mailbox* mb = static_cast<cmtfpls::Mailbox*>(mailbox);
+  if (!mb) return CMTFPLS_OK;
+  (void)hipFree(mb->counter);
+  (void)hipHostFree(mb->host);
+  delete mb;
+  return CMTFPLS_OK;
+}
+
+void* cmtfpls_mailbox_host(void* mailbox) { return mailbox ? static_cast<cmtfpls::Mailbox*>(mailbox)->host : nullptr; }
+
+int cmtfpls_host_wait(const void* words, unsigned long long want, double* out, int n, double timeout_s, void* stream, int query_stream) {
+  if (!words || n < 0 || (n > 0 && !out) || !(timeout_s >= 0.0)) { cmtfpls::set_error("host_wait: bad argument"); return CMTFPLS_EINVAL; }
+  const unsigned long long* w = static_cast<const unsigned long long*>(words);
+  const auto reached = [&]() { return __atomic_load_n(w, __ATOMIC_ACQUIRE) >= want; };
+  const auto deliver = [&]() {
+    if (n > 0) memcpy(out, w + 1, (size_t)n * sizeof(double));
+    return CMTFPLS_OK;
+  };
+  using clock = std::chrono::steady_clock;
+  const clock::time_point t0 = clock::now();
+  const clock::duration limit = std::chrono::duration_cast<clock::duration>(std::chrono::duration<double>(timeout_s));
+  clock::time_point next_query = t0 + std::chrono::microseconds(40);
+  for (;;) {
+    for (int spin = 0; spin < 64; ++spin) {
+      if (reached()) return deliver();
+      __builtin_ia32_pause();
+    }
+    const clock::time_point now = clock::now();
+    if (query_stream && now >= next_query) {
+      const hipError_t e = hipStreamQuery((hipStream_t)stream);
+      (void)hipGetLastError();
+      if (e != hipErrorNotReady) {
+        if (e == hipSuccess && reached()) return deliver();
+        if (e == hipSuccess) cmtfpls::set_error("host_wait: the stream drained without the sequence number");
+        else { cmtfpls::set_error(hipGetErrorString(e)); }
+        return CMTFPLS_EHIP;
+      }
+      next_query = now + std::chrono::microseconds(40);
+    }
+    if (now - t0 >= limit) {
+      if (reached()) return deliver();
+      cmtfpls::set_error("host_wait: timed out");
+      return CMTFPLS_ETIMEOUT;
+    }
+  }
+}
+}
diff --git a/cmtf_pls_amd/csrc/small.hip b/cmtf_pls_amd/csrc/small.hip
--- a/cmtf_pls_amd/csrc/small.hip
+++ b/cmtf_pls_amd/csrc/small.hip
@@ -1,3 +1,5 @@
+#include <atomic>
+
 #include "common.hpp"
 
 namespace cmtfpls {
@@ -189,7 +191,8 @@
 __global__ __launch_bounds__(1024) void q_update_kernel(const double* __restrict__ qpart, int nblk, int M,
                                                        double* __restrict__ q, int normalize,
                                                        const double* __restrict__ G, const double* __restrict__ q_prev,
-                                                       double* __restrict__ du2) {
+                                                       double* du2, int n_status, unsigned long long* mbox,
+                                                       unsigned long long* counter) {
   __shared__ double part[64][17];
   __shared__ double qs[64];
   __shared__ double dq[64];
@@ -244,6 +247,15 @@
     }
     sacc = block_sum(sacc, red);
     if (tid == 0) du2[0] = sacc;
+  }
+  if (mbox && tid == 0) {
+    for (int i = 0; i <= n_status; ++i)
+      __hip_atomic_store(mbox + 1 + i, (unsigned long long)__double_as_longlong(du2[i]), __ATOMIC_RELAXED, __HIP_MEMORY_SCOPE_SYSTEM);
+    const unsigned long long seq = counter[0] + 1;
+    counter[0] = seq;
+    __builtin_amdgcn_fence(__ATOMIC_RELEASE, "");
+    asm volatile("s_waitcnt vmcnt(0)" ::: "memory");
+    __hip_atomic_store(mbox, seq, __ATOMIC_RELAXED, __HIP_MEMORY_SCOPE_SYSTEM);
   }
 }
 
@@ -263,14 +275,28 @@
   }
 }
 
-__global__ __launch_bounds__(256) void s_contract_kernel(const double* __restrict__ S, int M, int64_t P, const double* __restrict__ q,
-                                                        double* __restrict__ Z) {
+__device__ __forceinline__ void s_contract_column(const double* __restrict__ S, int M, int64_t P, const double* __restrict__ q,
+                                                  double* __restrict__ Z) {
   const int64_t c = (int64_t)blockIdx.x * 256 + threadIdx.x;
   if (c >= P) return;
   double acc = 0.0;
 #pragma unroll 8
   for (int m = 0; m < M; ++m) acc = fma(q[m], S[(int64_t)m * P + c], acc);
   Z[c] = acc;
+}
+__global__ __launch_bounds__(256) void s_contract_kernel(const double* __restrict__ S, int M, int64_t P, const double* __restrict__ q,
+                                                        double* __restrict__ Z) {
+  s_contract_column(S, M, P, q, Z);
+}
+__global__ __launch_bounds__(256) void s_contract_preset_kernel(const double* __restrict__ S, int M, int64_t P,
+                                                               const double* __restrict__ q, double* __restrict__ Z, int cblocks,
+                                                               unsigned long long* __restrict__ region, int64_t words) {
+  if ((int)blockIdx.x < cblocks) {
+    s_contract_column(S, M, P, q, Z);
+    return;
+  }
+  const int64_t pb = (int64_t)blockIdx.x - cblocks, npb = (int64_t)gridDim.x - cblocks;
+  for (int64_t i = pb * 256 + threadIdx.x; i < words; i += npb * 256) region[i] = kChainEmpty;
 }
 
 __global__ __launch_bounds__(256) void axpy_scalar_kernel(double* __restrict__ y, int64_t n, const double* __restrict__ a,
@@ -378,12 +404,28 @@
   return check_launch("normalize");
 }
 
+static int q_update_launch(const double* qpart, int nblk, int M, double* q, int normalize, const double* G, const double* q_prev,
+                           double* du2, int n_status, const Mailbox* mb, void* stream) {
+  if (!q || M <= 0 || (qpart && nblk <= 0) || (G && (!q_prev || !du2))) { set_error("q_update: bad argument"); return CMTFPLS_EINVAL; }
+  if (M > 64) { set_error("q_update: more than 64 responses; use gram_tn + normalize + rowdot"); return CMTFPLS_EUNSUPPORTED; }
+  if (mb && (!du2 || n_status < 0 || n_status + 1 > mb->n_words || !mb->dev || !mb->counter)) {
+    set_error("q_update: the mailbox form needs du2 (the status block) and a mailbox of at least 1 + n_status words");
+    return CMTFPLS_EINVAL;
+  }
+  hipLaunchKernelGGL(q_update_kernel, dim3(1), dim3(1024), 0, (hipStream_t)stream, qpart, nblk, M, q, normalize, G, q_prev, du2,
+                     mb ? n_status : 0, mb ? mb->dev : (unsigned long long*)nullptr, mb ? mb->counter : (unsigned long long*)nullptr);
+  return check_launch("q_update");
+}
+
 int cmtfpls_q_update_f64(const double* qpart, int nblk, int M, double* q, int normalize, const double* G, const double* q_prev,
                          double* du2, void* stream) {
-  if (!q || M <= 0 || (qpart && nblk <= 0) || (G && (!q_prev || !du2))) { set_error("q_update: bad argument"); return CMTFPLS_EINVAL; }
-  if (M > 64) { set_error("q_update: more than 64 responses; use gram_tn + normalize + rowdot"); return CMTFPLS_EUNSUPPORTED; }
-  hipLaunchKernelGGL(q_update_kernel, dim3(1), dim3(1024), 0, (hipStream_t)stream, qpart, nblk, M, q, normalize, G, q_prev, du2);
-  return check_launch("q_update");
+  return q_update_launch(qpart, nblk, M, q, normalize, G, q_prev, du2, 0, nullptr, stream);
+}
+
+int cmtfpls_q_update_mailbox_f64(const double* qpart, int nblk, int M, double* q, int normalize, const double* G, const double* q_prev,
+                                 double* du2, int n_status, void* mailbox, void* stream) {
+  if (!mailbox) { set_error("q_update_mailbox: no mailbox"); return CMTFPLS_EINVAL; }
+  return q_update_launch(qpart, nblk, M, q, normalize, G, q_prev, du2, n_status, static_cast<const Mailbox*>(mailbox), stream);
 }
 
 int cmtfpls_s_downdate_f64(double* S, int M, int A, int B, const double* ya, const double* wA, const double* wB,
@@ -411,27 +453,55 @@
   return check_launch("kr_axpy");
 }
 
+static std::atomic<int> g_preset_merge{1};
+void cmtfpls_xcov_preset_merge_enable(int on) { g_preset_merge.store(on ? 1 : 0, std::memory_order_relaxed); }
+int cmtfpls_xcov_preset_merge_enabled(void) { return g_preset_merge.load(std::memory_order_relaxed); }
+
+static int xcov_iterate_run(const double* S, int M, int A, int B, const double* q_cur, double* Z, double* wA, double* wB, double* info,
+                            int n_squarings, double* q_new, const double* G, double* du2, int first, void* ws_rank1,
+                            size_t ws_rank1_bytes, int n_status, const Mailbox* mb, void* stream) {
+  if (!S || !q_cur || !Z || !wA || !wB || !q_new || !G || !du2 || M <= 0 || A <= 0 || B <= 0) {
+    set_error("xcov_iterate: bad argument");
+    return CMTFPLS_EINVAL;
+  }
+  if (M > 64) { set_error("xcov_iterate: more than 64 responses"); return CMTFPLS_EUNSUPPORTED; }
+  const int64_t P = (int64_t)A * B;
+  int rc = CMTFPLS_OK;
+  int64_t armed = 0;
+  if (first) {
+    const unsigned cblocks = (unsigned)((P + 255) / 256);
+    unsigned long long* region = nullptr;
+    if (g_preset_merge.load(std::memory_order_relaxed)) armed = rank1_chain_region(A, B, n_squarings, ws_rank1, ws_rank1_bytes, &region);
+    if (armed > 0)
+      hipLaunchKernelGGL(s_contract_preset_kernel, dim3(cblocks + (unsigned)((armed + 2047) / 2048)), dim3(256), 0, (hipStream_t)stream,
+                         S, M, P, q_cur, Z, (int)cblocks, region, armed);
+    else
+      hipLaunchKernelGGL(s_contract_kernel, dim3(cblocks), dim3(256), 0, (hipStream_t)stream, S, M, P, q_cur, Z);
+    rc = check_launch("xcov_iterate: s_contract");
+  }
+  if (rc == CMTFPLS_OK) rc = rank1_score_armed(Z, A, B, wA, wB, info, n_squarings, S, M, q_new, ws_rank1, ws_rank1_bytes, stream, armed);
+  if (rc == CMTFPLS_OK) rc = q_update_launch(nullptr, 0, M, q_new, 1, G, q_cur, du2, n_status, mb, stream);
+  return rc;
+}
+
 int cmtfpls_xcov_iterate_f64(const double* S, int M, int A, int B, const double* q_cur, double* Z, double* wA, double* wB,
                              double* info, int n_squarings, double* q_new, const double* G, double* du2, int first,
                              void* ws_contract, size_t ws_contract_bytes, void* ws_rank1, size_t ws_rank1_bytes, void* stream) {
-  if (!S || !q_cur || !Z || !wA || !wB || !q_new || !G || !du2 || M <= 0 || A <= 0 || B <= 0) {
-    set_error("xcov_iterate: bad argument");
-    return CMTFPLS_EINVAL;
-  }
-  if (M > 64) { set_error("xcov_iterate: more than 64 responses"); return CMTFPLS_EUNSUPPORTED; }
-  const int64_t P = (int64_t)A * B;
-  int rc = CMTFPLS_OK;
-  if (first) {
-    hipLaunchKernelGGL(s_contract_kernel, dim3((unsigned)((P + 255) / 256)), dim3(256), 0, (hipStream_t)stream, S, M, P, q_cur, Z);
-    rc = check_launch("xcov_iterate: s_contract");
-  }
-  if (rc == CMTFPLS_OK) rc = cmtfpls_rank1_score_f64(Z, A, B, wA, wB, info, n_squarings, S, M, q_new, ws_rank1, ws_rank1_bytes, stream);
-  if (rc == CMTFPLS_OK) rc = cmtfpls_q_update_f64(nullptr, 0, M, q_new, 1, G, q_cur, du2, stream);
-  return rc;
-}
-
-int cmtfpls_xcov_iterate_blocks_f64(const cmtfpls_xcov_block* blocks, int nb, int M, const double* q_cur, double* tq, double* q_new,
-                                    const double* G, double* du2, int first, void* ws_rank1, size_t ws_rank1_bytes, void* stream) {
+  (void)ws_contract; (void)ws_contract_bytes;
+  return xcov_iterate_run(S, M, A, B, q_cur, Z, wA, wB, info, n_squarings, q_new, G, du2, first, ws_rank1, ws_rank1_bytes, 0, nullptr, stream);
+}
+
+int cmtfpls_xcov_iterate_mailbox_f64(const double* S, int M, int A, int B, const double* q_cur, double* Z, double* wA, double* wB,
+                                     double* info, int n_squarings, double* q_new, const double* G, double* du2, int first,
+                                     void* ws_rank1, size_t ws_rank1_bytes, int n_status, void* mailbox, void* stream) {
+  if (!mailbox) { set_error("xcov_iterate_mailbox: no mailbox"); return CMTFPLS_EINVAL; }
+  return xcov_iterate_run(S, M, A, B, q_cur, Z, wA, wB, info, n_squarings, q_new, G, du2, first, ws_rank1, ws_rank1_bytes, n_status,
+                          static_cast<const Mailbox*>(mailbox), stream);
+}
+
+static int xcov_iterate_blocks_run(const cmtfpls_xcov_block* blocks, int nb, int M, const double* q_cur, double* tq, double* q_new,
+                                   const double* G, double* du2, int first, void* ws_rank1, size_t ws_rank1_bytes, int n_status,
+                                   const Mailbox* mb, void* stream) {
   if (!blocks || nb <= 0 || !q_cur || !tq || !q_new || !G || !du2 || M <= 0) { set_error("xcov_iterate_blocks: bad argument"); return CMTFPLS_EINVAL; }
   if (M > 64) { set_error("xcov_iterate_blocks: more than 64 responses"); return CMTFPLS_EUNSUPPORTED; }
   hipStream_t st = (hipStream_t)stream;
@@ -466,8 +536,21 @@
     }
     if (rc == CMTFPLS_OK) rc = cmtfpls_score_s_f64(k.S2 ? k.S2 : k.S, M, k.A, k.B, k.wA, k.wB, tq + (int64_t)b * M, stream);
   }
-  if (rc == CMTFPLS_OK) rc = cmtfpls_q_update_f64(tq, nb, M, q_new, 1, G, q_cur, du2, stream);
+  if (rc == CMTFPLS_OK) rc = q_update_launch(tq, nb, M, q_new, 1, G, q_cur, du2, n_status, mb, stream);
   return rc;
+}
+
+int cmtfpls_xcov_iterate_blocks_f64(const cmtfpls_xcov_block* blocks, int nb, int M, const double* q_cur, double* tq, double* q_new,
+                                    const double* G, double* du2, int first, void* ws_rank1, size_t ws_rank1_bytes, void* stream) {
+  return xcov_iterate_blocks_run(blocks, nb, M, q_cur, tq, q_new, G, du2, first, ws_rank1, ws_rank1_bytes, 0, nullptr, stream);
+}
+
+int cmtfpls_xcov_iterate_blocks_mailbox_f64(const cmtfpls_xcov_block* blocks, int nb, int M, const double* q_cur, double* tq,
+                                            double* q_new, const double* G, double* du2, int first, void* ws_rank1,
+                                            size_t ws_rank1_bytes, int n_status, void* mailbox, void* stream) {
+  if (!mailbox) { set_error("xcov_iterate_blocks_mailbox: no mailbox"); return CMTFPLS_EINVAL; }
+  return xcov_iterate_blocks_run(blocks, nb, M, q_cur, tq, q_new, G, du2, first, ws_rank1, ws_rank1_bytes, n_status,
+                                 static_cast<const Mailbox*>(mailbox), stream);
 }
 
 int cmtfpls_colscale_f64(double* Z, int64_t P, const double* colcnt, double n_samples, void* stream) {
diff --git a/cmtf_pls_amd/fitrun.py b/cmtf_pls_amd/fitrun.py
--- a/cmtf_pls_amd/fitrun.py
+++ b/cmtf_pls_amd/fitrun.py
@@ -125,6 +125,9 @@
         self.status_host = None
         if self.status.is_cuda:
             self.status_host = torch.empty(self.status.shape, dtype=torch.float64, pin_memory=True)
+        self._mbox = None
+        self._mbox_ok = bool(eng.opt.status_mailbox and hasattr(be, "mailbox_acquire") and not comm.sharded and M <= 64)
+        self.status_transport = None
         self.sq_max = int(getattr(be, "rank1_squarings", 30))
         self.sq_budget = [self.sq_max] * len(self.blocks)
         side = int(getattr(be, "rank1_chain_side", 0))
@@ -349,7 +352,32 @@
         if note not in self.notes:
             self.notes.append(note)
 
-    def _read_status(self) -> np.ndarray:
+    def _mailbox(self, n_words: int):
+        if not self._mbox_ok:
+            return None
+        mb = self.eng.be.mailbox_acquire(n_words)
+        if mb is None:
+            self._mbox_ok = False
+            self.notes.append("status mailbox could not be set up: convergence status through copy + event")
+        return mb
+
+    def _release_mailboxes(self) -> None:
+        be = self.eng.be
+        pipe = getattr(self, "_pipe", None) or {}
+        for mb in [self._mbox] + list(pipe.get("mbox") or []):
+            if mb is not None:
+                be.mailbox_release(mb)
+        self._mbox = None
+        if pipe.get("mbox"):
+            pipe["mbox"] = None
+            pipe["plans"].clear()
+
+    def _read_status(self, mailbox=None) -> np.ndarray:
+        if mailbox is not None:
+            mailbox.count += 1
+            self.status_transport = "mailbox"
+            return self.eng.be.mailbox_wait(mailbox, mailbox.count)
+        self.status_transport = self.status_transport or "copy + event"
         if self.status_host is None:
             return self.status.cpu().numpy()
         self.status_host.copy_(self.status, non_blocking=True)
@@ -506,9 +534,16 @@
             if sharded:
                 be.q_update(q_new, self.qpart, normalize=False, nparts=nparts)
 
+        if self._mbox is None and not sharded:
+            self._mbox = self._mailbox(self.status.numel())
+        mbox = None if sharded else self._mbox
+
         def seg_y_update():
             if sharded:
                 be.q_update(q_new, None, normalize=True, G=self.Gy, q_prev=q_cur, du2=self.status[0:1])
+            elif mbox is not None:
+                be.q_update(q_new, self.qpart, normalize=True, G=self.Gy, q_prev=q_cur, du2=self.status[0:1], nparts=nparts,
+                            mailbox=mbox, n_status=self.status.numel() - 1)
             else:
                 be.q_update(q_new, self.qpart, normalize=True, G=self.Gy, q_prev=q_cur, du2=self.status[0:1], nparts=nparts)
 
@@ -547,7 +582,7 @@
                     self._run(("floadings", par, budgets), seg_loadings_scores)
                     comm.allreduce(q_new)
                     self._run(("fyupdate", par), seg_y_update)
-            host = self._read_status()
+            host = self._read_status(mbox)
             local, peer = self._update_budgets(host), self._peer_failed(host, first)
             if not (local or peer):
                 break
@@ -694,6 +729,7 @@
             self.eng.comm.allreduce(self.dot_log)
             parts.append(self.dot_log.reshape(-1))
         host = torch.cat(parts).cpu().numpy()
+        self._release_mailboxes()
         R = self.R
         self.coef[...] = host[: R * R].reshape(R, R)
         ssq = host[R * R: R * R + R * (nb + 1)].reshape(R, nb + 1).copy()
@@ -723,6 +759,7 @@
             "graphs": bool(self.use_graphs and self._graphs), "graph_error": self._graph_error,
             "collectives_in_graph": self._collectives_captured is True,
             "backend": getattr(eng.be, "name", type(eng.be).__name__),
+            "status_transport": self.status_transport,
         }
         if self.algorithm == "direct":
             rep["y_side"] = "fused into the sweeps" if self._fused else "separate launches"
diff --git a/cmtf_pls_amd/fitrun_xcov.py b/cmtf_pls_amd/fitrun_xcov.py
--- a/cmtf_pls_amd/fitrun_xcov.py
+++ b/cmtf_pls_amd/fitrun_xcov.py
@@ -37,11 +37,19 @@
 
         par = self._parity
         q_cur, q_new = self.qx[par], self.qx[par ^ 1]
+        if composite and self._mbox is None:
+            self._mbox = self._mailbox(self.status.numel())
+        mbox = self._mbox if composite else None
 
         def seg(first: bool):
             if composite:
-                be.xcov_iterate(self.S[0], blk0.A, blk0.B, q_cur, self.Zs[0], self.wA[0], self.wB[0], self.status[1:3],
-                                self.sq_budget[0], q_new, self.Gy, self.status[0:1], first)
+                if mbox is not None:
+                    be.xcov_iterate(self.S[0], blk0.A, blk0.B, q_cur, self.Zs[0], self.wA[0], self.wB[0], self.status[1:3],
+                                    self.sq_budget[0], q_new, self.Gy, self.status[0:1], first, mailbox=mbox,
+                                    n_status=self.status.numel() - 1)
+                else:
+                    be.xcov_iterate(self.S[0], blk0.A, blk0.B, q_cur, self.Zs[0], self.wA[0], self.wB[0], self.status[1:3],
+                                    self.sq_budget[0], q_new, self.Gy, self.status[0:1], first)
                 return
             if first:
                 for b, blk in enumerate(self.blocks):
@@ -61,7 +69,7 @@
         first = True
         while True:
             self._run(("xcov", it > 0, tuple(self.sq_budget), first, par if composite else -1), lambda: seg(first))
-            host = self._read_status()
+            host = self._read_status(mbox)
             if not self._update_budgets(host):
                 break
             first = False
@@ -102,10 +110,20 @@
                 "Z": [list(self.Zs), second["Z"]], "wA": [list(self.wA), second["wA"]], "wB": [list(self.wB), second["wB"]],
                 "status": [be.zeros(1 + 2 * nb), be.zeros(1 + 2 * nb)],
                 "plans": {}, "slots": {},
+                "mbox": None,
             }
             for st in pp["status"]:
                 st[1::2] = 1.0
+            if single or hasattr(be, "xcov_blocks_plan"):
+                two = [self._mailbox(1 + 2 * nb), self._mailbox(1 + 2 * nb)]
+                if all(mb is not None for mb in two):
+                    pp["mbox"] = two
+                else:
+                    for mb in two:
+                        if mb is not None:
+                            be.mailbox_release(mb)
         plans = pp["plans"]
+        mboxes = pp["mbox"]
 
         def make_plan(it: int):
             s = it & 1
@@ -113,22 +131,41 @@
             if single:
                 blk0 = self.blocks[0]
                 if hasattr(be, "xcov_iterate_plan"):
+                    extra = {"mailbox": mboxes[s]} if mboxes else {}
                     one = be.xcov_iterate_plan(self.S[0], blk0.A, blk0.B, q_cur, pp["Z"][s][0], pp["wA"][s][0], pp["wB"][s][0], st,
-                                               q_new, self.Gy)
+                                               q_new, self.Gy, **extra)
                     return lambda nsq, first: one(nsq[0], first)
+                if mboxes:
+                    return lambda nsq, first: be.xcov_iterate(self.S[0], blk0.A, blk0.B, q_cur, pp["Z"][s][0], pp["wA"][s][0],
+                                                              pp["wB"][s][0], st[1:3], nsq[0], q_new, self.Gy, st[0:1], first,
+                                                              mailbox=mboxes[s], n_status=2)
                 return lambda nsq, first: be.xcov_iterate(self.S[0], blk0.A, blk0.B, q_cur, pp["Z"][s][0], pp["wA"][s][0],
                                                           pp["wB"][s][0], st[1:3], nsq[0], q_new, self.Gy, st[0:1], first)
             descr = [dict(S=self.S[b], S2=self.S2[b] if blk.has_miss else None, colcnt=blk.colcnt if blk.has_miss else None,
                           n_samples=self.n_total, order=len(blk.shape), A=blk.A, B=blk.B,
                           Z=pp["Z"][s][b], wA=pp["wA"][s][b], wB=pp["wB"][s][b]) for b, blk in enumerate(self.blocks)]
-            return be.xcov_blocks_plan(descr, self.M, q_cur, self.Tq, q_new, self.Gy, st)
+            extra = {"mailbox": mboxes[s]} if mboxes else {}
+            return be.xcov_blocks_plan(descr, self.M, q_cur, self.Tq, q_new, self.Gy, st, **extra)
 
         def enqueue(it: int, first: bool = True):
             plan = plans.get(it % 6)
             if plan is None:
                 plan = plans[it % 6] = make_plan(it)
             plan([n if it > 0 else min(self.sq_max, n + 4) for n in self.sq_budget], first)
+            if mboxes:
+                mb = mboxes[it & 1]
+                mb.count += 1
+                return (mb, mb.count)
             return be.status_snapshot(pp["status"][it & 1], it & 1, slots=pp["slots"])
+
+        if mboxes:
+            self.status_transport = "mailbox"
+
+            def wait(tok):
+                return be.mailbox_wait(tok[0], tok[1])
+        else:
+            self.status_transport = self.status_transport or "copy + event"
+            wait = be.status_wait
 
         stats = self.pipeline_stats
         it, tok = 0, enqueue(0)
@@ -140,7 +177,7 @@
                 if it == 0 or predicted is None or predicted >= tol:
                     ahead = enqueue(it + 1)
                     stats["ahead"] += 1
-            host = be.status_wait(tok)
+            host = wait(tok)
             short = [b for b in range(nb) if not host[1 + 2 * b] > 0.5 and self.sq_budget[b] < self.sq_max]
             if any(host[2 + 2 * b] < 0 for b in range(nb)):
                 self._chain_gave_up()
diff --git a/cmtf_pls_amd/options.py b/cmtf_pls_amd/options.py
--- a/cmtf_pls_amd/options.py
+++ b/cmtf_pls_amd/options.py
@@ -18,6 +18,7 @@
     xcov_stats_with_s: bool = True
     xcov_deflate_build: bool = True
     xcov_pipeline: bool = True
+    status_mailbox: bool = True
     capture_collectives: bool = False
     project_split_rows: bool = True
     masked_folds: bool = False
diff --git a/include/cmtfpls.h b/include/cmtfpls.h
--- a/include/cmtfpls.h
+++ b/include/cmtfpls.h
@@ -13,11 +13,17 @@
 #define CMTFPLS_EWORKSPACE 2
 #define CMTFPLS_EHIP 3
 #define CMTFPLS_EUNSUPPORTED 4
+#define CMTFPLS_ETIMEOUT 5
 
 int cmtfpls_abi_version(void);
 const char* cmtfpls_last_error(void);
 int cmtfpls_clear_error(void);
 int cmtfpls_status_to_host(const void* src, void* dst_host, size_t bytes, void* event, void* stream);
+int cmtfpls_mailbox_create(int n_words, void** mailbox);
+int cmtfpls_mailbox_destroy(void* mailbox);
+void* cmtfpls_mailbox_host(void* mailbox);
+int cmtfpls_host_wait(const void* words, unsigned long long want, double* out, int n, double timeout_s, void* stream,
+                      int query_stream);
 
 size_t cmtfpls_colstats_workspace_bytes(int64_t I, int64_t P);
 int cmtfpls_colstats_f32(const float* X, int64_t I, int64_t P, double* colsum, double* colcnt,
@@ -88,6 +94,12 @@
                              double* wB, double* info, int n_squarings, double* q_new, const double* G, double* du2,
                              int first, void* ws_contract, size_t ws_contract_bytes, void* ws_rank1,
                              size_t ws_rank1_bytes, void* stream);
+int cmtfpls_xcov_iterate_mailbox_f64(const double* S, int M, int A, int B, const double* q_cur, double* Z, double* wA,
+                                     double* wB, double* info, int n_squarings, double* q_new, const double* G, double* du2,
+                                     int first, void* ws_rank1, size_t ws_rank1_bytes, int n_status, void* mailbox,
+                                     void* stream);
+void cmtfpls_xcov_preset_merge_enable(int on);
+int cmtfpls_xcov_preset_merge_enabled(void);
 typedef struct {
   const double* S;
   const double* S2;
@@ -103,6 +115,9 @@
 } cmtfpls_xcov_block;
 int cmtfpls_xcov_iterate_blocks_f64(const cmtfpls_xcov_block* blocks, int nb, int M, const double* q_cur, double* tq, double* q_new,
                                     const double* G, double* du2, int first, void* ws_rank1, size_t ws_rank1_bytes, void* stream);
+int cmtfpls_xcov_iterate_blocks_mailbox_f64(const cmtfpls_xcov_block* blocks, int nb, int M, const double* q_cur, double* tq,
+                                            double* q_new, const double* G, double* du2, int first, void* ws_rank1,
+                                            size_t ws_rank1_bytes, int n_status, void* mailbox, void* stream);
 int cmtfpls_s_downdate_f64(double* S, int M, int A, int B, const double* ya, const double* wA, const double* wB,
                            const double* q, const double* v, void* stream);
 int cmtfpls_kr_axpy_f64(double* v, int A, int B, const double* WA, const double* WB, int ld, int k, const double* coef, void* stream);
@@ -155,6 +170,8 @@
                            void* stream);
 int cmtfpls_q_update_f64(const double* qpart, int nblk, int M, double* q, int normalize, const double* G,
                          const double* q_prev, double* du2, void* stream);
+int cmtfpls_q_update_mailbox_f64(const double* qpart, int nblk, int M, double* q, int normalize, const double* G,
+                                 const double* q_prev, double* du2, int n_status, void* mailbox, void* stream);
 
 int cmtfpls_deflate_f32(float* X, int64_t I, int A, int B, const double* t, const double* wA,
                         const double* wB, double* ssq_part, void* stream);
```

Result: no change. 767.0 (median of 6 runs) (+0.9%).
